# sair-lab/AirSLAM

Hardware: AMD Instinct MI355X
Metric: stereo detect+match pairs/sec (2x PLNet @512x512 internal: points + lines, junctions on the left + LightGlue match) (higher is better)
Workload: dtype fp16

## Files before the change

airslam_amd/_lib.py:

```python
from __future__ import annotations

import ctypes as C
import os

_HERE = os.path.dirname(os.path.abspath(__file__))
LIB_PATH = os.path.join(_HERE, "libairfe.so")


class Tuning(C.Structure):
    _fields_ = [(n, C.c_int) for n in (
        "fuse_lg_block", "gemm_small_max_m", "gemm8_min_m", "gemmr_min_m", "gemmr_wgs", "qkv_pair", "block_min_m", "lgb_tokens", "sg_kenc_gemm",
        "fold_qkv", "overlap_lines", "kf_graph", "kf_spec_rows", "fuse_dec", "assign_fused", "fold_out_proj", "desc_gather_stream", "copy_wgs")] + [("reserved", C.c_int * 5)]


class Cfg(C.Structure):
    _fields_ = [
        ("device", C.c_int), ("precision", C.c_int), ("max_batch", C.c_int), ("enc_chunk", C.c_int),
        ("max_keypoints", C.c_int), ("keypoint_threshold", C.c_float), ("remove_borders", C.c_int),
        ("nms_radius", C.c_int), ("line_threshold", C.c_float), ("line_length_threshold", C.c_float),
        ("matcher", C.c_int), ("image_width", C.c_int), ("image_height", C.c_int), ("sinkhorn_iters", C.c_int),
        ("superpoint_pack", C.c_char_p), ("plnet_s1_pack", C.c_char_p), ("lightglue_pack", C.c_char_p),
        ("superglue_pack", C.c_char_p), ("matcher_precision", C.c_int), ("line_precision", C.c_int), ("check_launches", C.c_int),
        ("tuning", C.POINTER(Tuning)),
    ]


class Stage0(C.Structure):
    _fields_ = [(n, C.c_void_p) for n in (
        "juncs_pred", "lines_pred", "iskeep", "idx_junc_to_end_min", "idx_junc_to_end_max",
        "loi_features", "loi_features_thin", "loi_features_aux")]


class BowdbFilter(C.Structure):
    _fields_ = [("ratio", C.c_float), ("min_words", C.c_int), ("d_max_index", C.c_void_p), ("d_exclude", C.c_void_p), ("exclude_words", C.c_int)]


class RelocCfg(C.Structure):
    _fields_ = [("ratio", C.c_float), ("min_words", C.c_int), ("K", C.c_int), ("outlier_rejection", C.c_int), ("min_inlier", C.c_int),
                ("pose_refinement", C.c_int), ("cam", C.c_double * 5), ("thr", C.c_double * 2)]


class LoopCfg(C.Structure):
    _fields_ = [("ratio", C.c_float), ("min_words", C.c_int), ("K", C.c_int), ("outlier_rejection", C.c_int), ("distance_rate", C.c_double),
                ("min_matches", C.c_int), ("min_points", C.c_int), ("min_inliers", C.c_int), ("cam", C.c_double * 5), ("thr", C.c_double * 2)]


class SeqPolicy(C.Structure):
    _fields_ = [("min_init_stereo_feature", C.c_int), ("min_num_match", C.c_int), ("max_num_match", C.c_int), ("tracking_point_rate", C.c_float),
                ("tracking_parallax_rate", C.c_float), ("min_x_diff", C.c_double), ("max_x_diff", C.c_double), ("max_y_diff", C.c_double),
                ("image_width", C.c_int), ("image_height", C.c_int)]


class SeqFrame(C.Structure):
    _fields_ = ([(n, C.c_int) for n in ("frame_type", "candidate", "promoted", "dropped", "enough_match", "good_stereo_point", "n_left", "n_right", "n_lines_left",
                                        "n_lines_right", "n_junctions", "n_stereo", "n_matches")] + [("_pad", C.c_int)]
                + [(n, C.c_void_p) for n in ("features_left", "features_right", "lines_left", "lines_right", "junctions", "stereo_idx", "stereo_score", "matches_idx",
                                             "matches_score")])


class DebugLinearArgs(C.Structure):
    _fields_ = ([(n, C.c_int) for n in ("prec", "M", "K", "K1", "N")] + [(n, C.c_void_p) for n in ("x1", "x2", "w", "b")]
                + [("epi", C.c_int), ("act", C.c_int), ("rowidx", C.c_void_p), ("src_rows", C.c_int), ("rot_cos", C.c_void_p), ("rot_sin", C.c_void_p),
                   ("Np", C.c_int), ("H", C.c_int), ("x32", C.c_void_p), ("d2s_hc", C.c_int), ("d2s_wc", C.c_int), ("flag", C.c_void_p),
                   ("kernel", C.c_int), ("gr_wgs", C.c_int), ("out", C.c_void_p), ("out2", C.c_void_p)])


class DebugLgBlockArgs(C.Structure):
    _fields_ = ([("prec", C.c_int), ("M", C.c_int)] + [(n, C.c_void_p) for n in ("attn", "x32", "xb", "wo", "bo", "w1", "b1", "gamma", "beta", "w2", "b2")]
                + [(n, C.c_int) for n in ("relu", "tokens_per_wg", "mixed", "nqk_n")]
                + [(n, C.c_void_p) for n in ("nqk_w", "nqk_b", "nv_w", "nv_b", "rot_cos", "rot_sin")]
                + [("Np", C.c_int)] + [(n, C.c_void_p) for n in ("q", "k", "vt")] + [("rows_past", C.c_int * 5)])


class DebugWgPrimsArgs(C.Structure):
    _fields_ = [("v", C.c_void_p), ("keep", C.c_void_p), ("n", C.c_int), ("threads", C.c_int), ("keys", C.c_void_p), ("P", C.c_int), ("key_bytes", C.c_int),
                ("scan", C.c_void_p), ("pos", C.c_void_p), ("totals", C.c_void_p), ("wave", C.c_void_p), ("sorted", C.c_void_p)]


class DebugConvArgs(C.Structure):
    _fields_ = ([(n, C.c_void_p) for n in ("x", "img", "w1a", "b1a", "w", "b")] + [(n, C.c_int) for n in ("cin", "cout", "B", "H", "W", "pool", "out_pad", "relu", "wgs")]
                + [("y_words", C.c_size_t), ("y_raw", C.c_void_p)])


class DebugLgPrepareArgs(C.Structure):
    _fields_ = ([(n, C.c_int) for n in ("prec", "B", "cap", "ld", "kp_off", "normalize")] + [(n, C.c_float) for n in ("cx", "cy", "linv")]
                + [(n, C.c_void_p) for n in ("f0", "f1", "n0", "n1", "wr", "f0x", "f1x")] + [(n, C.c_int) for n in ("n0x", "n1x", "slack_rows", "rows")]
                + [(n, C.c_void_p) for n in ("x32", "xb", "rot_cos", "rot_sin", "lens")] + [("rows_past", C.c_int)])


class DebugLgAssignArgs(C.Structure):
    _fields_ = ([(n, C.c_int) for n in ("prec", "B", "n")] + [(n, C.c_void_p) for n in ("md", "x32", "w")] + [("b", C.c_float), ("lens", C.c_void_p), ("cap", C.c_int),
                ("thr", C.c_float), ("form", C.c_int)]
                + [(n, C.c_void_p) for n in ("pad", "z", "sim", "scores", "rowlse", "collse", "rowval", "rowarg", "colarg", "idx", "score", "nmatch")])


class DebugSgFrontArgs(C.Structure):
    _fields_ = ([(n, C.c_int) for n in ("prec", "split", "B", "cap", "normalize")] + [(n, C.c_void_p) for n in ("f0", "f1", "n0", "n1")] + [("rows", C.c_int)]
                + [(n, C.c_void_p) for n in ("lens", "x32", "xb", "h128", "hb")] + [("rows_past", C.c_int)])


class DebugAttentionArgs(C.Structure):
    _fields_ = ([(n, C.c_int) for n in ("prec", "S", "H", "n", "cross")] + [(n, C.c_void_p) for n in ("q", "k", "v", "lens")]
                + [("canary", C.c_int), ("raw", C.c_int), ("out", C.c_void_p), ("Np", C.c_int), ("rows_past", C.c_int)])


class DebugDetectorTailArgs(C.Structure):
    _fields_ = ([(n, C.c_int) for n in ("B", "Bs", "h", "w", "cap")] + [(n, C.c_void_p) for n in ("heat", "act", "feat", "feat1", "n", "n1", "nms_map", "keep", "cand_cnt")]
                + [("nms_map_written", C.c_int)])


class DebugLinePostArgs(C.Structure):
    _fields_ = ([(n, C.c_int) for n in ("B", "nj", "ld", "h", "w", "capL", "capJ", "from_plane")]
                + [(n, C.c_void_p) for n in ("la", "sc", "m2", "heat", "lines", "nlines", "nfound", "junc", "njunc", "jfound", "jmap")])


class DebugJunctionTailArgs(C.Structure):
    _fields_ = ([(n, C.c_int) for n in ("B", "nj", "ld", "h", "w", "capL", "capJ")]
                + [(n, C.c_void_p) for n in ("la", "sc", "m2", "heat", "act", "lines", "nlines", "nfound", "junc", "njunc", "jfound")] + [("fused", C.c_int)])


class DebugLineMidArgs(C.Structure):
    _fields_ = ([(n, C.c_int) for n in ("B", "j2l", "s1_form", "wgs")]
                + [(n, C.c_void_p) for n in ("juncs_pred", "lines_pred", "thin", "aux", "loi", "iskeep_in", "idx_min_in", "idx_max_in", "iskeep", "idx_min", "idx_max", "counts",
                                             "keep", "pairs", "rep", "head4", "prop4", "ridx", "proj", "lines_adjusted", "scores_line", "table_dirty")])


class DebugS0DecodeArgs(C.Structure):
    _fields_ = ([(n, C.c_int) for n in ("B", "mode", "ld", "off", "want_ta8", "want_loi", "want_jnms", "prec", "wgs")] + [(n, C.c_void_p) for n in ("rows", "x", "w", "b")]
                + [("stage_floats", C.c_size_t)] + [(n, C.c_void_p) for n in ("stage", "jloc", "joff", "jnms", "ta8", "loi", "head_rows")])


SIGNATURES = {
    "airfe_copy_rows_dev": (C.c_int, [C.c_void_p, C.c_int, C.c_void_p, C.c_void_p, C.c_void_p, C.c_void_p, C.c_void_p, C.c_void_p]),
    "airfe_pack_rows_dev": (C.c_int, [C.c_void_p, C.c_int, C.c_void_p, C.c_void_p, C.c_void_p, C.c_void_p, C.c_void_p, C.c_void_p, C.c_void_p]),
    "airfe_seq_default_policy": (None, [C.POINTER(SeqPolicy)]),
    "airfe_seq_add_keyframe_check": (C.c_int, [C.POINTER(SeqPolicy), C.c_void_p, C.c_int, C.c_void_p, C.c_int, C.c_void_p, C.c_int]),
    "airfe_seq_good_stereo_points": (C.c_int, [C.POINTER(SeqPolicy), C.c_void_p, C.c_void_p, C.c_void_p, C.c_int]),
    "airfe_seq_create": (C.c_int, [C.c_void_p, C.c_void_p, C.c_int, C.POINTER(SeqPolicy), C.c_int, C.c_int, C.c_void_p, C.c_void_p, C.c_void_p, C.POINTER(C.c_void_p)]),
    "airfe_seq_destroy": (None, [C.c_void_p]),
    "airfe_seq_last_error": (C.c_char_p, [C.c_void_p]),
    "airfe_seq_begin": (C.c_int, [C.c_void_p, C.c_void_p, C.c_void_p, C.c_int, C.c_int, C.c_int, C.c_size_t]),
    "airfe_seq_end": (C.c_int, [C.c_void_p, C.POINTER(SeqFrame)]),
    "airfe_seq_step": (C.c_int, [C.c_void_p, C.c_void_p, C.c_void_p, C.c_int, C.c_int, C.c_int, C.c_size_t, C.POINTER(SeqFrame)]),
    "airfe_seq_stream": (C.c_void_p, [C.c_void_p]),
    "airfe_seq_set_outlier_rejection": (C.c_int, [C.c_void_p, C.c_int]),
    "airfe_seq_wall_split": (C.c_int, [C.c_void_p, C.POINTER(C.c_double), C.POINTER(C.c_double), C.POINTER(C.c_double), C.POINTER(C.c_int), C.POINTER(C.c_int)]),
    "airfe_default_cfg": (None, [C.POINTER(Cfg)]),
    "airfe_default_tuning": (None, [C.POINTER(Tuning)]),
    "airfe_debug_fail_next_launch": (C.c_int, [C.c_void_p, C.c_int]),
    "airfe_create": (C.c_int, [C.POINTER(Cfg), C.POINTER(C.c_void_p)]),
    "airfe_destroy": (None, [C.c_void_p]),
    "airfe_last_error": (C.c_char_p, [C.c_void_p]),
    "airfe_detect_points": (C.c_int, [C.c_void_p, C.c_void_p, C.c_int, C.c_int, C.c_int, C.c_void_p, C.c_int,
                                      C.POINTER(C.c_int)]),
    "airfe_has_line_branch": (C.c_int, [C.c_void_p]),
    "airfe_detect_plnet": (C.c_int, [C.c_void_p, C.c_void_p, C.c_int, C.c_int, C.c_int, C.POINTER(Stage0), C.c_void_p,
                                     C.c_int, C.POINTER(C.c_int), C.c_void_p, C.c_int, C.POINTER(C.c_int), C.c_void_p,
                                     C.c_int, C.POINTER(C.c_int), C.c_int]),
    "airfe_stereo_keyframe": (C.c_int, [C.c_void_p, C.c_void_p, C.c_void_p, C.c_int, C.c_int, C.c_int, C.c_void_p, C.c_void_p, C.c_int,
                                        C.POINTER(C.c_int), C.POINTER(C.c_int), C.c_void_p, C.c_void_p, C.c_int, C.POINTER(C.c_int),
                                        C.POINTER(C.c_int), C.c_void_p, C.c_int, C.POINTER(C.c_int), C.c_void_p, C.c_void_p, C.c_int,
                                        C.POINTER(C.c_int)]),
    "airfe_stereo_keyframe_tracked": (C.c_int, [C.c_void_p, C.c_void_p, C.c_void_p, C.c_int, C.c_int, C.c_int, C.c_void_p, C.c_void_p, C.c_int,
                                                C.POINTER(C.c_int), C.POINTER(C.c_int), C.c_void_p, C.c_void_p, C.c_int, C.POINTER(C.c_int),
                                                C.POINTER(C.c_int), C.c_void_p, C.c_int, C.POINTER(C.c_int), C.c_void_p, C.c_void_p, C.c_int,
                                                C.POINTER(C.c_int), C.c_void_p, C.c_int, C.c_void_p, C.c_void_p, C.POINTER(C.c_int)]),
    "airfe_track_frame": (C.c_int, [C.c_void_p, C.c_void_p, C.c_int, C.c_int, C.c_int, C.c_void_p, C.c_int, C.c_void_p, C.c_int, C.POINTER(C.c_int),
                                    C.c_void_p, C.c_void_p, C.c_int, C.POINTER(C.c_int)]),
    "airfe_promote_frame": (C.c_int, [C.c_void_p, C.c_void_p, C.c_int, C.c_int, C.c_int, C.c_void_p, C.c_int, C.POINTER(C.c_int), C.c_void_p, C.c_void_p, C.c_int,
                                      C.POINTER(C.c_int)]),
    "airfe_adopt_reference": (C.c_int, [C.c_void_p]),
    "airfe_match_lightglue": (C.c_int, [C.c_void_p, C.c_void_p, C.c_int, C.c_void_p, C.c_int, C.c_void_p, C.c_void_p,
                                        C.c_int, C.POINTER(C.c_int)]),
    "airfe_match_superglue": (C.c_int, [C.c_void_p, C.c_void_p, C.c_int, C.c_void_p, C.c_int, C.c_void_p, C.c_void_p,
                                        C.c_void_p, C.c_void_p]),
    "airfe_assign_points_to_lines": (C.c_int, [C.c_void_p, C.c_void_p, C.c_int, C.c_void_p, C.c_int, C.c_void_p, C.c_void_p,
                                               C.c_void_p, C.c_int, C.c_void_p]),
    "airfe_match_lines": (C.c_int, [C.c_void_p, C.c_void_p, C.c_void_p, C.c_int, C.c_int, C.c_void_p, C.c_void_p, C.c_int, C.c_int,
                                    C.c_void_p, C.c_int, C.c_void_p]),
    "airfe_bow_load": (C.c_int, [C.c_void_p, C.c_void_p, C.c_void_p, C.c_void_p, C.c_void_p, C.c_void_p, C.c_int]),
    "airfe_bow_transform": (C.c_int, [C.c_void_p, C.c_void_p, C.c_int, C.c_void_p, C.c_void_p]),
    "airfe_bow_transform_dev": (C.c_int, [C.c_void_p, C.c_void_p, C.c_int, C.c_void_p, C.c_void_p, C.c_void_p]),
    "airfe_bow_vector": (C.c_int, [C.c_void_p, C.c_void_p, C.c_int, C.c_void_p, C.c_void_p, C.POINTER(C.c_int), C.c_void_p]),
    "airfe_bow_vector_batch_dev": (C.c_int, [C.c_void_p, C.c_void_p, C.c_void_p, C.c_int, C.c_int] + [C.c_void_p] * 5),
    "airfe_bowdb_create": (C.c_int, [C.c_void_p, C.c_int, C.c_int, C.c_int, C.POINTER(C.c_void_p)]),
    "airfe_bowdb_destroy": (C.c_int, [C.c_void_p]),
    "airfe_bowdb_clear": (C.c_int, [C.c_void_p]),
    "airfe_bowdb_size": (C.c_int, [C.c_void_p]),
    "airfe_bowdb_add_batch_dev": (C.c_int, [C.c_void_p] * 6 + [C.c_int, C.c_int, C.c_void_p]),
    "airfe_bowdb_add": (C.c_int, [C.c_void_p] * 6 + [C.c_int, C.c_int]),
    "airfe_bowdb_query_batch_dev": (C.c_int, [C.c_void_p] * 4 + [C.c_int, C.c_int, C.POINTER(BowdbFilter)] + [C.c_void_p] * 3 + [C.c_int] + [C.c_void_p] * 4),
    "airfe_bowdb_topk_dev": (C.c_int, [C.c_void_p] * 4 + [C.c_int, C.c_int, C.c_int, C.c_void_p, C.c_void_p, C.c_void_p]),
    "airfe_bowdb_match_candidates_batch_dev": (C.c_int, [C.c_void_p] * 4 + [C.c_int, C.c_int, C.c_void_p, C.c_int, C.c_int] + [C.c_void_p] * 3 + [C.c_int] + [C.c_void_p] * 3),
    "airfe_bowdb_attach_map": (C.c_int, [C.c_void_p, C.c_int]),
    "airfe_bowdb_set_points_dev": (C.c_int, [C.c_void_p, C.c_int, C.c_int, C.c_void_p, C.c_void_p]),
    "airfe_bowdb_set_points": (C.c_int, [C.c_void_p, C.c_int, C.c_int, C.c_void_p]),
    "airfe_bowdb_get_points": (C.c_int, [C.c_void_p, C.c_int, C.c_int, C.c_void_p]),
    "airfe_bowdb_set_covisibility": (C.c_int, [C.c_void_p, C.c_void_p, C.c_void_p, C.c_void_p, C.c_int]),
    "airfe_bowdb_get_covisibility": (C.c_int, [C.c_void_p, C.c_void_p, C.c_void_p, C.c_void_p, C.c_int, C.POINTER(C.c_int)]),
    "airfe_bowdb_set_positions": (C.c_int, [C.c_void_p, C.c_int, C.c_int, C.c_void_p]),
    "airfe_bowdb_group_dev": (C.c_int, [C.c_void_p, C.c_int] + [C.c_void_p] * 3 + [C.c_int] * 3 + [C.c_void_p] * 8),
    "airfe_relocalize_batch_dev": (C.c_int, [C.c_void_p, C.c_void_p, C.POINTER(RelocCfg), C.c_void_p, C.c_void_p, C.c_int, C.c_int] + [C.c_void_p] * 9 +
                                   [C.c_int] + [C.c_void_p] * 3),
    "airfe_bowdb_set_poses": (C.c_int, [C.c_void_p, C.c_int, C.c_int, C.c_void_p]),
    "airfe_bowdb_get_poses": (C.c_int, [C.c_void_p, C.c_int, C.c_int, C.c_void_p]),
    "airfe_bowdb_set_u_right_dev": (C.c_int, [C.c_void_p, C.c_int, C.c_int, C.c_void_p, C.c_void_p]),
    "airfe_bowdb_set_u_right": (C.c_int, [C.c_void_p, C.c_int, C.c_int, C.c_void_p]),
    "airfe_bowdb_get_u_right": (C.c_int, [C.c_void_p, C.c_int, C.c_int, C.c_void_p]),
    "airfe_bowdb_attach_point_ids": (C.c_int, [C.c_void_p, C.c_int]),
    "airfe_bowdb_set_point_ids_dev": (C.c_int, [C.c_void_p, C.c_int, C.c_int, C.c_void_p, C.c_void_p]),
    "airfe_bowdb_set_point_ids": (C.c_int, [C.c_void_p, C.c_int, C.c_int, C.c_void_p]),
    "airfe_bowdb_get_point_ids": (C.c_int, [C.c_void_p, C.c_int, C.c_int, C.c_void_p]),
    "airfe_bowdb_build_covisibility_dev": (C.c_int, [C.c_void_p, C.c_void_p, C.c_void_p]),
    "airfe_bowdb_build_covisibility": (C.c_int, [C.c_void_p, C.POINTER(C.c_int)]),
    "airfe_bowdb_attach_triangulation": (C.c_int, [C.c_void_p]),
    "airfe_bowdb_triangulate_points_dev": (C.c_int, [C.c_void_p, C.c_void_p, C.c_int] + [C.c_void_p] * 5),
    "airfe_bowdb_triangulate_points": (C.c_int, [C.c_void_p, C.c_void_p, C.c_int, C.c_void_p, C.c_void_p, C.c_void_p, C.POINTER(C.c_int)]),
    "airfe_bowdb_fill_points_dev": (C.c_int, [C.c_void_p, C.c_void_p, C.c_void_p, C.c_int, C.c_void_p, C.c_void_p]),
    "airfe_triangulate_point": (C.c_int, [C.c_void_p, C.c_void_p, C.c_void_p, C.c_int, C.c_void_p, C.POINTER(C.c_int)]),
    "airfe_bowdb_attach_merge": (C.c_int, [C.c_void_p]),
    "airfe_bowdb_merge_points_dev": (C.c_int, [C.c_void_p, C.c_void_p, C.c_int, C.c_void_p, C.c_void_p, C.c_void_p]),
    "airfe_bowdb_merge_points": (C.c_int, [C.c_void_p, C.c_void_p, C.c_int, C.c_void_p, C.c_void_p]),
    "airfe_bowdb_loop_merge_batch_dev": (C.c_int, [C.c_void_p, C.c_void_p, C.c_void_p, C.c_int] + [C.c_void_p] * 6 + [C.c_int] + [C.c_void_p] * 4),
    "airfe_junction_connections_batch_dev": (C.c_int, [C.c_void_p, C.c_void_p, C.c_void_p, C.c_int, C.c_void_p, C.c_void_p] + [C.c_int] * 4 + [C.c_void_p, C.c_int] +
                                             [C.c_void_p] * 4),
    "airfe_junction_connections": (C.c_int, [C.c_void_p, C.c_void_p, C.c_int, C.c_void_p, C.c_int, C.c_int, C.c_int, C.c_void_p, C.c_int, C.POINTER(C.c_int),
                                             C.c_void_p]),
    "airfe_bowdb_attach_junctions": (C.c_int, [C.c_void_p, C.c_int, C.c_int]),
    "airfe_bowdb_set_junctions_dev": (C.c_int, [C.c_void_p, C.c_int, C.c_int] + [C.c_void_p] * 6),
    "airfe_bowdb_set_junctions": (C.c_int, [C.c_void_p, C.c_int, C.c_int] + [C.c_void_p] * 5),
    "airfe_bowdb_get_junctions": (C.c_int, [C.c_void_p, C.c_int, C.c_int] + [C.c_void_p] * 10),
    "airfe_bowdb_junction_term_batch_dev": (C.c_int, [C.c_void_p] * 9 + [C.c_int] + [C.c_void_p] * 4),
    "airfe_bowdb_junction_extra_batch_dev": (C.c_int, [C.c_void_p, C.c_void_p, C.c_void_p, C.c_int, C.c_void_p, C.c_void_p] + [C.c_int] * 4 + [C.c_void_p] * 4),
    "airfe_bowdb_add_junction_frames_batch_dev": (C.c_int, [C.c_void_p, C.c_void_p, C.c_void_p, C.c_int, C.c_void_p, C.c_void_p] + [C.c_int] * 4 + [C.c_void_p]),
    "airfe_bowdb_query_stored_batch_dev": (C.c_int, [C.c_void_p, C.c_void_p, C.c_int, C.c_float, C.c_int, C.c_int] + [C.c_void_p] * 3 + [C.c_int] +
                                           [C.c_void_p] * 4),
    "airfe_loop_detect_batch_dev": (C.c_int, [C.c_void_p, C.c_void_p, C.POINTER(LoopCfg), C.c_void_p, C.c_int] + [C.c_void_p] * 10 + [C.c_int] +
                                    [C.c_void_p] * 3),
    "airfe_set_rectify_maps": (C.c_int, [C.c_void_p, C.c_int, C.c_void_p, C.c_void_p, C.c_int, C.c_int]),
    "airfe_rectify_detect_points": (C.c_int, [C.c_void_p, C.c_int, C.c_void_p, C.c_int, C.c_int, C.c_int, C.c_void_p, C.c_void_p, C.c_int,
                                              C.POINTER(C.c_int)]),
    "airfe_rectify_batch_dev": (C.c_int, [C.c_void_p, C.c_int, C.c_void_p, C.c_int, C.c_int, C.c_int, C.c_int, C.c_size_t, C.c_void_p,
                                          C.c_int, C.c_size_t, C.c_void_p]),
    "airfe_detect_points_batch_dev": (C.c_int, [C.c_void_p, C.c_void_p, C.c_int, C.c_int, C.c_int, C.c_int, C.c_size_t,
                                                C.c_void_p, C.c_int, C.c_void_p, C.c_void_p]),
    "airfe_match_lightglue_batch_dev": (C.c_int, [C.c_void_p, C.c_void_p, C.c_void_p, C.c_void_p, C.c_void_p, C.c_int,
                                                  C.c_int, C.c_void_p, C.c_void_p, C.c_int, C.c_void_p, C.c_void_p]),
    "airfe_match_superglue_batch_dev": (C.c_int, [C.c_void_p, C.c_void_p, C.c_void_p, C.c_void_p, C.c_void_p, C.c_int, C.c_int,
                                                  C.c_void_p, C.c_void_p, C.c_void_p, C.c_void_p, C.c_void_p]),
    "airfe_stereo_batch_dev": (C.c_int, [C.c_void_p, C.c_void_p, C.c_void_p, C.c_int, C.c_int, C.c_int, C.c_int,
                                         C.c_size_t, C.c_void_p, C.c_void_p, C.c_int, C.c_void_p, C.c_void_p, C.c_void_p,
                                         C.c_void_p, C.c_int, C.c_void_p, C.c_void_p]),
    "airfe_detect_plnet_batch_dev": (C.c_int, [C.c_void_p, C.c_void_p, C.c_int, C.c_int, C.c_int, C.c_int, C.c_size_t, C.c_void_p,
                                               C.c_int, C.c_void_p, C.c_void_p, C.c_int, C.c_void_p, C.c_void_p, C.c_int, C.c_void_p,
                                               C.c_int, C.c_void_p, C.c_void_p]),
    "airfe_stereo_plnet_batch_dev": (C.c_int, [C.c_void_p, C.c_void_p, C.c_void_p, C.c_int, C.c_int, C.c_int, C.c_int, C.c_size_t,
                                               C.c_void_p, C.c_void_p, C.c_int, C.c_void_p, C.c_void_p, C.c_void_p, C.c_int, C.c_void_p,
                                               C.c_void_p, C.c_int, C.c_void_p, C.c_void_p, C.c_void_p, C.c_void_p, C.c_int, C.c_void_p,
                                               C.c_void_p]),
    "airfe_debug_plnet_j2l": (C.c_int, [C.c_void_p, C.c_int, C.c_void_p, C.c_void_p, C.c_void_p]),
    "airfe_assign_points_to_lines_batch_dev": (C.c_int, [C.c_void_p, C.c_void_p, C.c_void_p, C.c_int, C.c_void_p, C.c_void_p, C.c_int, C.c_int,
                                                         C.c_void_p, C.c_void_p, C.c_void_p, C.c_int, C.c_void_p, C.c_void_p]),
    "airfe_match_lines_batch_dev": (C.c_int, [C.c_void_p] + [C.c_void_p] * 8 + [C.c_int, C.c_int, C.c_void_p, C.c_void_p, C.c_int, C.c_int,
                                              C.c_void_p, C.c_void_p, C.c_void_p, C.c_int, C.c_void_p, C.c_void_p]),
    "airfe_fundamental_ransac": (C.c_int, [C.c_void_p, C.c_void_p, C.c_int, C.c_void_p, C.c_int, C.c_void_p, C.c_void_p, C.c_int, C.POINTER(C.c_int)]),
    "airfe_fundamental_ransac_batch_dev": (C.c_int, [C.c_void_p, C.c_void_p, C.c_void_p, C.c_void_p, C.c_void_p, C.c_int, C.c_int, C.c_void_p, C.c_void_p,
                                                     C.c_int, C.c_void_p, C.c_void_p, C.c_void_p]),
    "airfe_set_outlier_rejection": (C.c_int, [C.c_void_p, C.c_int]),
    "airfe_pnp_ransac": (C.c_int, [C.c_void_p, C.c_void_p, C.c_void_p, C.c_int, C.c_void_p, C.c_void_p, C.c_void_p, C.c_void_p, C.POINTER(C.c_int)]),
    "airfe_pnp_ransac_batch_dev": (C.c_int, [C.c_void_p, C.c_void_p, C.c_void_p, C.c_void_p, C.c_int, C.c_int, C.c_void_p, C.c_void_p, C.c_void_p,
                                             C.c_void_p, C.c_void_p, C.c_void_p]),
    "airfe_stereo_points": (C.c_int, [C.c_void_p, C.c_void_p, C.c_void_p, C.c_int, C.c_void_p, C.c_int, C.c_void_p, C.c_int, C.c_void_p, C.c_void_p,
                                      C.c_void_p, C.POINTER(C.c_int)]),
    "airfe_stereo_points_batch_dev": (C.c_int, [C.c_void_p] * 6 + [C.c_int, C.c_int, C.c_void_p, C.c_void_p, C.c_int] + [C.c_void_p] * 5),
    "airfe_stereo_lines": (C.c_int, [C.c_void_p, C.c_void_p, C.c_void_p, C.c_int, C.c_void_p, C.c_int] + [C.c_void_p] * 8),
    "airfe_stereo_lines_batch_dev": (C.c_int, [C.c_void_p] * 6 + [C.c_int, C.c_void_p, C.c_void_p, C.c_int] + [C.c_void_p] * 7),
    "airfe_stereo_line_landmarks_batch_dev": (C.c_int, [C.c_void_p] * 6 + [C.c_int] + [C.c_void_p] * 4 + [C.c_int, C.c_void_p, C.c_void_p, C.c_int,
                                                        C.c_void_p, C.c_int] + [C.c_void_p] * 8 + [C.c_int] + [C.c_void_p] * 8),
    "airfe_track_pose_batch_dev": (C.c_int, [C.c_void_p, C.c_void_p, C.c_void_p, C.c_int, C.c_void_p, C.c_int, C.c_void_p, C.c_void_p, C.c_int, C.c_int,
                                             C.c_void_p, C.c_void_p, C.c_void_p, C.c_void_p, C.c_void_p]),
    "airfe_frame_optimize": (C.c_int, [C.c_void_p, C.c_void_p, C.c_void_p, C.c_int] + [C.c_void_p] * 7 + [C.POINTER(C.c_int)]),
    "airfe_frame_optimize_batch_dev": (C.c_int, [C.c_void_p, C.c_void_p, C.c_void_p, C.c_void_p, C.c_int, C.c_int] + [C.c_void_p] * 9),
    "airfe_track_pose_opt_batch_dev": (C.c_int, [C.c_void_p, C.c_void_p, C.c_void_p, C.c_int, C.c_void_p, C.c_int, C.c_void_p, C.c_int, C.c_void_p,
                                                 C.c_void_p, C.c_int, C.c_int] + [C.c_void_p] * 9),
    "airfe_sync": (C.c_int, [C.c_void_p]),
    "airfe_superglue_status": (C.c_int, [C.c_void_p, C.c_void_p]),
    "airfe_profile_enable": (C.c_int, [C.c_void_p, C.c_int]),
    "airfe_profile_stages": (C.c_int, []),
    "airfe_profile_stage_name": (C.c_char_p, [C.c_int]),
    "airfe_profile_read": (C.c_int, [C.c_void_p, C.c_void_p, C.c_void_p, C.c_void_p, C.c_void_p]),
    "airfe_debug_detector_maps": (C.c_int, [C.c_void_p, C.c_int, C.c_void_p, C.c_void_p, C.c_void_p]),
    "airfe_debug_lightglue_scores": (C.c_int, [C.c_void_p, C.c_void_p, C.c_int, C.c_void_p, C.c_int, C.c_void_p]),
    "airfe_debug_superglue_scores": (C.c_int, [C.c_void_p, C.c_void_p, C.c_int, C.c_void_p, C.c_int, C.c_void_p]),
    "airfe_debug_lg_filter": (C.c_int, [C.c_void_p, C.c_void_p, C.c_int, C.c_int, C.c_void_p, C.c_void_p, C.c_int, C.POINTER(C.c_int)]),
    "airfe_debug_sg_decode": (C.c_int, [C.c_void_p, C.c_void_p, C.c_int, C.c_int, C.c_void_p, C.c_void_p, C.c_void_p, C.c_void_p]),
    "airfe_debug_sg_sinkhorn": (C.c_int, [C.c_void_p, C.c_void_p, C.c_void_p, C.c_int, C.c_int, C.c_float, C.c_int, C.c_int, C.c_void_p, C.POINTER(C.c_int)]),
    "airfe_debug_detector_tail": (C.c_int, [C.c_void_p, C.POINTER(DebugDetectorTailArgs)]),
    "airfe_debug_line_post": (C.c_int, [C.c_void_p, C.POINTER(DebugLinePostArgs)]),
    "airfe_debug_junction_tail": (C.c_int, [C.c_void_p, C.POINTER(DebugJunctionTailArgs)]),
    "airfe_debug_junctions_topk": (C.c_int, [C.c_void_p, C.c_void_p, C.c_void_p, C.c_int, C.c_void_p]),
    "airfe_debug_line_mid": (C.c_int, [C.c_void_p, C.POINTER(DebugLineMidArgs)]),
    "airfe_debug_s0_decode": (C.c_int, [C.c_void_p, C.POINTER(DebugS0DecodeArgs)]),
    "airfe_debug_lg_prepare": (C.c_int, [C.c_void_p, C.POINTER(DebugLgPrepareArgs)]),
    "airfe_debug_lg_assign": (C.c_int, [C.c_void_p, C.POINTER(DebugLgAssignArgs)]),
    "airfe_debug_sg_front": (C.c_int, [C.c_void_p, C.POINTER(DebugSgFrontArgs)]),
    "airfe_debug_plnet_stage0": (C.c_int, [C.c_void_p] + [C.c_void_p] * 10),
    "airfe_debug_plnet_s1": (C.c_int, [C.c_void_p, C.POINTER(Stage0), C.c_void_p, C.c_void_p, C.c_int, C.POINTER(C.c_int)]),
    "airfe_debug_plnet_s1_last": (C.c_int, [C.c_void_p, C.c_void_p, C.c_void_p, C.c_int, C.POINTER(C.c_int)]),
    "airfe_debug_preprocess": (C.c_int, [C.c_void_p, C.c_void_p, C.c_int, C.c_int, C.c_int, C.c_void_p]),
    "airfe_debug_conv3x3": (C.c_int, [C.c_void_p, C.c_void_p, C.c_int, C.c_int, C.c_int, C.c_int, C.c_void_p, C.c_void_p,
                                      C.c_int, C.c_int, C.c_void_p]),
    "airfe_debug_conv": (C.c_int, [C.c_void_p, C.POINTER(DebugConvArgs)]),
    "airfe_debug_trace": (C.c_int, [C.c_void_p, C.c_int]),
    "airfe_debug_trace_stop": (C.c_int, [C.c_void_p, C.c_int]),
    "airfe_debug_trace_buffer": (C.c_int, [C.c_void_p, C.c_int, C.c_void_p, C.c_size_t]),
    "airfe_debug_trace_slots": (C.c_int, [C.c_void_p]),
    "airfe_debug_conv_order": (C.c_int, [C.c_int, C.POINTER(C.c_int)]),
    "airfe_debug_wg_prims": (C.c_int, [C.c_void_p, C.POINTER(DebugWgPrimsArgs)]),
    "airfe_debug_trace_slot": (C.c_int, [C.c_void_p, C.c_int, C.c_char_p, C.c_int, C.POINTER(C.c_uint), C.POINTER(C.c_uint), C.POINTER(C.c_uint)]),
    "airfe_debug_trace_read": (C.c_int, [C.c_void_p, C.c_void_p, C.c_void_p, C.c_void_p]),
    "airfe_debug_gemm": (C.c_int, [C.c_void_p, C.c_void_p, C.c_int, C.c_int, C.c_void_p, C.c_void_p, C.c_int, C.c_int,
                                   C.c_void_p]),
    "airfe_debug_linear": (C.c_int, [C.c_void_p, C.POINTER(DebugLinearArgs)]),
    "airfe_debug_qkv": (C.c_int, [C.c_void_p] + [C.c_int] * 3 + [C.c_void_p] * 3 + [C.c_int] + [C.c_void_p] * 4 + [C.c_int] * 2 + [C.c_void_p] * 3),
    "airfe_debug_lg_block": (C.c_int, [C.c_void_p, C.POINTER(DebugLgBlockArgs)]),
    "airfe_debug_ln_gelu": (C.c_int, [C.c_void_p, C.c_int, C.c_void_p, C.c_void_p, C.c_void_p, C.c_int]),
    "airfe_debug_attention_args": (C.c_int, [C.c_void_p, C.POINTER(DebugAttentionArgs)]),
    "airfe_debug_attention": (C.c_int, [C.c_void_p, C.c_void_p, C.c_void_p, C.c_void_p, C.c_void_p, C.c_int, C.c_int, C.c_int, C.c_int, C.c_void_p]),
}

_lib = None


def lib() -> C.CDLL:
    global _lib
    if _lib is None:
        if not os.path.exists(LIB_PATH):
            raise RuntimeError(
                f"{LIB_PATH} is missing: build it with `python -m airslam_amd.build` "
                "(hipcc, gfx950).  airslam_amd has no CPU fallback.")
        try:
            import torch
        except Exception:
            pass
        l = C.CDLL(LIB_PATH)
        for name, (res, args) in SIGNATURES.items():
            fn = getattr(l, name)
            fn.restype = res
            fn.argtypes = args
        _lib = l
    return _lib
```

airslam_amd/api.py:

```python
from __future__ import annotations

import ctypes as C
import os
import tempfile
from typing import Dict, Optional

import numpy as np

from . import _lib, weights as W

FEAT = 259


def _pack_arg(x, tmpfiles) -> Optional[bytes]:
    if x is None:
        return None
    if isinstance(x, (str, bytes, os.PathLike)):
        return os.fsencode(x)
    f = tempfile.NamedTemporaryFile(suffix=".airfe", delete=False)
    f.close()
    W.save_pack(f.name, x)
    tmpfiles.append(f.name)
    return f.name.encode()


class AirfeError(RuntimeError):
    pass


def conv_tile_order(order: int) -> int:
    prev = C.c_int()
    if _lib.lib().airfe_debug_conv_order(int(order), C.byref(prev)) != 0:
        raise AirfeError((_lib.lib().airfe_last_error(None) or b"airfe_debug_conv_order failed").decode())
    return prev.value


class Context:

    def __init__(self, superpoint=None, lightglue=None, superglue=None, plnet_s1=None, tuning=None, **cfg):
        self._l = _lib.lib()
        c = _lib.Cfg()
        self._l.airfe_default_cfg(C.byref(c))
        t = None
        if tuning and "conv_order" in tuning:
            tuning = dict(tuning)
            conv_tile_order(int(tuning.pop("conv_order")))
        if tuning:
            t = _lib.Tuning()
            self._l.airfe_default_tuning(C.byref(t))
            for k, v in tuning.items():
                if k == "reserved" or not hasattr(t, k):
                    raise TypeError(f"unknown airfe_tuning field {k!r}")
                setattr(t, k, int(v))
            c.tuning = C.pointer(t)
        for k, v in cfg.items():
            if not hasattr(c, k):
                raise TypeError(f"unknown airfe_cfg field {k!r}")
            setattr(c, k, v)
        tmp = []
        try:
            c.superpoint_pack = _pack_arg(superpoint, tmp)
            c.lightglue_pack = _pack_arg(lightglue, tmp)
            c.superglue_pack = _pack_arg(superglue, tmp)
            c.plnet_s1_pack = _pack_arg(plnet_s1, tmp)
            h = C.c_void_p()
            rc = self._l.airfe_create(C.byref(c), C.byref(h))
            if rc != 0:
                raise AirfeError((self._l.airfe_last_error(None) or b"airfe_create failed").decode())
        finally:
            for t in tmp:
                os.unlink(t)
        self._h = h
        c.tuning = None
        self.cfg = c
        self.max_keypoints = c.max_keypoints
        self.np_rows = (c.max_keypoints + 15) // 16 * 16

    def close(self):
        if getattr(self, "_h", None):
            self._l.airfe_destroy(self._h)
            self._h = None

    def __del__(self):
        try:
            self.close()
        except Exception:
            pass

    def _chk(self, rc, what):
        if rc != 0:
            raise AirfeError(f"{what}: {(self._l.airfe_last_error(self._h) or b'').decode()}")

    @staticmethod
    def _image(img, wrong_type=None):
        img = np.asarray(img)
        if img.ndim != 2 or img.dtype != np.uint8:
            raise wrong_type if wrong_type is not None else AirfeError("empty image")
        if img.size == 0:
            raise AirfeError("empty image")
        if img.strides[1] != 1 or img.strides[0] < img.shape[1]:
            img = np.ascontiguousarray(img)
        return img

    def detect_points(self, gray: np.ndarray) -> np.ndarray:
        gray = self._image(gray, TypeError("expected a 2-D uint8 image"))
        cap = self.np_rows
        feat = np.empty((cap, FEAT), dtype=np.float32)
        n = C.c_int(0)
        self._chk(self._l.airfe_detect_points(self._h, gray.ctypes.data, gray.shape[0], gray.shape[1], gray.strides[0],
                                              feat.ctypes.data, cap, C.byref(n)), "airfe_detect_points")
        return feat[:n.value].copy()

    def bow_load(self, voc: dict):
        d = np.ascontiguousarray(voc["desc"], np.float32); fc = np.ascontiguousarray(voc["first_child"], np.int32)
        nc = np.ascontiguousarray(voc["n_children"], np.int32); wi = np.ascontiguousarray(voc["word_id"], np.int32)
        w = np.ascontiguousarray(voc["weight"], np.float64)
        self._chk(self._l.airfe_bow_load(self._h, d.ctypes.data, fc.ctypes.data, nc.ctypes.data, wi.ctypes.data, w.ctypes.data, d.shape[0]),
                  "airfe_bow_load")

    def bow_transform(self, feat_rows: np.ndarray):
        f = np.ascontiguousarray(feat_rows, np.float32).reshape(-1, FEAT)
        wid = np.empty((f.shape[0],), np.uint32); w = np.empty((f.shape[0],), np.float64)
        self._chk(self._l.airfe_bow_transform(self._h, f.ctypes.data, f.shape[0], wid.ctypes.data, w.ctypes.data), "airfe_bow_transform")
        return wid, w

    def set_rectify_maps(self, side: int, mapx: np.ndarray, mapy: np.ndarray):
        mx = np.ascontiguousarray(mapx, np.float32); my = np.ascontiguousarray(mapy, np.float32)
        if mx.shape != my.shape or mx.ndim != 2:
            raise TypeError("maps must be two 2-D arrays of one shape")
        self._chk(self._l.airfe_set_rectify_maps(self._h, side, mx.ctypes.data, my.ctypes.data, mx.shape[0], mx.shape[1]), "airfe_set_rectify_maps")

    def rectify_detect(self, side: int, raw: np.ndarray, detect: bool = True):
        raw = self._image(raw)
        rect = np.empty(raw.shape, np.uint8)
        cap = self.np_rows
        feat = np.empty((cap, FEAT), np.float32) if detect else None
        n = C.c_int(0)
        self._chk(self._l.airfe_rectify_detect_points(self._h, side, raw.ctypes.data, raw.shape[0], raw.shape[1], raw.strides[0],
                                                      rect.ctypes.data, feat.ctypes.data if detect else None, cap, C.byref(n)),
                  "airfe_rectify_detect_points")
        return rect, (feat[:n.value].copy() if detect else None)

    def match_lightglue(self, f0: np.ndarray, f1: np.ndarray):
        f0 = np.ascontiguousarray(f0, dtype=np.float32)
        f1 = np.ascontiguousarray(f1, dtype=np.float32)
        cap = self.np_rows
        idx = np.empty((cap, 2), dtype=np.int32)
        sc = np.empty((cap,), dtype=np.float32)
        n = C.c_int(0)
        self._chk(self._l.airfe_match_lightglue(self._h, f0.ctypes.data, f0.shape[0], f1.ctypes.data, f1.shape[0],
                                                idx.ctypes.data, sc.ctypes.data, cap, C.byref(n)), "airfe_match_lightglue")
        return idx[:n.value].copy(), sc[:n.value].copy()

    def lightglue_scores(self, f0: np.ndarray, f1: np.ndarray) -> np.ndarray:
        f0 = np.ascontiguousarray(f0, dtype=np.float32)
        f1 = np.ascontiguousarray(f1, dtype=np.float32)
        out = np.empty((f0.shape[0], f1.shape[0]), dtype=np.float32)
        self._chk(self._l.airfe_debug_lightglue_scores(self._h, f0.ctypes.data, f0.shape[0], f1.ctypes.data, f1.shape[0],
                                                       out.ctypes.data), "airfe_debug_lightglue_scores")
        return out

    @staticmethod
    def _stage0(s0):
        st = _lib.Stage0()
        keep = []
        for name, _ in _lib.Stage0._fields_:
            a = np.ascontiguousarray(s0[name], dtype=np.float32)
            keep.append(a)
            setattr(st, name, a.ctypes.data)
        return st, keep

    def detect_plnet(self, gray: np.ndarray, stage0=None, want_junctions: bool = False, cap_lines: int = 45056,
                     cap_junc: int = 2048):
        gray = self._image(gray)
        cap = self.np_rows
        feat = np.empty((cap, FEAT), np.float32)
        lines = np.empty((cap_lines, 4), np.float64)
        junc = np.empty((cap_junc, FEAT), np.float32)
        n, nl, nj = C.c_int(0), C.c_int(0), C.c_int(0)
        st, keep = (self._stage0(stage0) if stage0 is not None else (None, None))
        self._chk(self._l.airfe_detect_plnet(self._h, gray.ctypes.data, gray.shape[0], gray.shape[1], gray.strides[0],
                                             C.byref(st) if st is not None else None, feat.ctypes.data, cap, C.byref(n),
                                             lines.ctypes.data, cap_lines, C.byref(nl), junc.ctypes.data, cap_junc,
                                             C.byref(nj), int(want_junctions)), "airfe_detect_plnet")
        return feat[:n.value].copy(), lines[:nl.value].copy(), junc[:nj.value].copy()

    def stereo_keyframe(self, left: np.ndarray, right: np.ndarray, match: bool = True, want_junctions: bool = True, cap_lines: int = 4096,
                        cap_junc: int = 2048, track: bool = False, ref_feat=None, outlier_rejection: bool = False):
        if outlier_rejection and not track:
            raise AirfeError("stereo_keyframe: outlier_rejection applies to the temporal match: pass track=True")
        if ref_feat is not None and not track:
            raise AirfeError("stereo_keyframe: ref_feat is the temporal match's reference: pass track=True")
        if track and not match:
            raise AirfeError("stereo_keyframe: track=True needs match=True (the temporal pair rides in the stereo match's forward)")
        imgs = [self._image(g) for g in (left, right)]
        if imgs[0].shape != imgs[1].shape:
            raise AirfeError("stereo_keyframe: left and right images differ in size")
        if imgs[0].strides[0] != imgs[1].strides[0]:
            imgs = [np.ascontiguousarray(g) for g in imgs]
# ... 312 lines not shown
                                  thin=thin.ctypes.data, aux=aux.ctypes.data, loi=loi.ctypes.data, **{k: v.ctypes.data for k, v in out.items()})
        ins = [None if x is None else f(x) for x in (iskeep, idx_min, idx_max)]
        for name, x in zip(("iskeep_in", "idx_min_in", "idx_max_in"), ins):
            if x is not None:
                assert x.shape == (b, n)
                setattr(a, name, x.ctypes.data)
        self._chk(self._l.airfe_debug_line_mid(self._h, C.byref(a)), "airfe_debug_line_mid")
        return out

    S0_STAGE = {"lines_pred": (600, 3 * 16384 * 4), "thin": (600 + 7 * 3 * 16384, 4 * 16384), "aux": (600 + 7 * 3 * 16384 + 4 * 16384, 4 * 16384)}
    S0_STAGE_FLOATS = (600 + 7 * 3 * 16384 + 8 * 16384 + 63) // 64 * 64

    def debug_s0_decode(self, rows=None, ld=160, off=128, ta8=True, loi=False, jnms=True, x=None, w=None, b=None, prec=1, wgs=0, two_pass=False):
        f = lambda t: np.ascontiguousarray(t, np.float32)
        npx, sf = 128 * 128, self.S0_STAGE_FLOATS
        a = _lib.DebugS0DecodeArgs(want_ta8=int(bool(ta8)), want_loi=int(bool(loi)), want_jnms=int(bool(jnms)), prec=int(prec), wgs=int(wgs), stage_floats=sf)
        if rows is not None:
            assert x is None and not two_pass
            rows = f(rows)
            bb = rows.shape[0]
            assert rows.shape == (bb, npx, ld)
            a.mode, a.ld, a.off, a.rows = 0, int(ld), int(off), rows.ctypes.data
        else:
            x, w, b = f(x), f(w), f(b)
            bb = x.shape[0] // npx
            assert x.shape == (bb * npx, 128) and w.shape == (17, 128) and b.shape == (17,)
            a.mode, a.x, a.w, a.b = (2 if two_pass else 1), x.ctypes.data, w.ctypes.data, b.ctypes.data
        poison = lambda *shape: np.full(shape, -1, np.int32).view(np.float32)
        out = {"stage": poison(bb, sf), "jloc": poison(bb, 128, 128), "joff": poison(bb, 2, 128, 128), "jnms": poison(bb, 128, 128), "ta8": poison(bb, npx, 8),
               "loi": poison(128, 128, 128)}
        if two_pass:
            out["head_rows"] = poison(bb, npx, 32)
        a.B = bb
        for k, v in out.items():
            setattr(a, k, v.ctypes.data)
        self._chk(self._l.airfe_debug_s0_decode(self._h, C.byref(a)), "airfe_debug_s0_decode")
        for k, (o, n) in self.S0_STAGE.items():
            v = out["stage"][:, o:o + n]
            out[k] = v.reshape(bb, 3 * npx, 4) if k == "lines_pred" else v.reshape(bb, 4, 128, 128)
        return out

    def debug_junctions_topk(self, jloc, joff):
        jloc, joff = np.ascontiguousarray(jloc, np.float32), np.ascontiguousarray(joff, np.float32)
        b = jloc.shape[0]
        assert jloc.shape == (b, 128, 128) and joff.shape == (b, 2, 128, 128)
        out = np.full((b, 300, 2), np.nan, np.float32)
        self._chk(self._l.airfe_debug_junctions_topk(self._h, jloc.ctypes.data, joff.ctypes.data, b, out.ctypes.data), "airfe_debug_junctions_topk")
        return out

    def debug_preprocess(self, gray):
        gray = np.ascontiguousarray(gray, np.uint8)
        out = np.empty((512, 512), np.float32)
        self._chk(self._l.airfe_debug_preprocess(self._h, gray.ctypes.data, gray.shape[0], gray.shape[1], gray.strides[0],
                                                 out.ctypes.data), "airfe_debug_preprocess")
        return out

    def debug_conv3x3(self, x, w, b, pool=False):
        x = np.ascontiguousarray(x, np.float32); w = np.ascontiguousarray(w, np.float32); b = np.ascontiguousarray(b, np.float32)
        bb, cin, hh, ww = x.shape
        cout = w.shape[0]
        ho, wo = (hh // 2, ww // 2) if pool else (hh, ww)
        y = np.empty((bb, cout, ho, wo), np.float32)
        self._chk(self._l.airfe_debug_conv3x3(self._h, x.ctypes.data, bb, cin, hh, ww, w.ctypes.data, b.ctypes.data, cout,
                                              int(pool), y.ctypes.data), "airfe_debug_conv3x3")
        return y

    def debug_conv(self, w, b, prec, x=None, img=None, w1a=None, b1a=None, pool=False, out_pad=1, relu=True, wgs=256):
        f32 = lambda t: None if t is None else np.ascontiguousarray(t, np.float32)
        x, img, w1a, b1a, w, b = map(f32, (x, img, w1a, b1a, w, b))
        src = x if x is not None else img
        bb, hh, ww = src.shape[0], src.shape[-2], src.shape[-1]
        cout, cin = w.shape[0], w.shape[1]
        p = int(out_pad)
        ho, wo = (hh // 2, ww // 2) if pool else (hh, ww)
        guard = (wo + 2 * p) * cout
        words = bb * (ho + 2 * p) * guard
        raw = np.zeros(words + 2 * guard, np.uint16)
        ptr = lambda t: None if t is None else t.ctypes.data
        a = _lib.DebugConvArgs(x=ptr(x), img=ptr(img), w1a=ptr(w1a), b1a=ptr(b1a), w=ptr(w), b=ptr(b), cin=cin, cout=cout, B=bb, H=hh, W=ww, pool=int(pool), out_pad=p,
                               relu=int(relu), wgs=int(wgs), y_words=raw.size, y_raw=ptr(raw))
        self._chk(self._l.airfe_debug_conv(self._h, C.byref(a)), "airfe_debug_conv")
        buf = raw[guard:guard + words].reshape(bb, ho + 2 * p, wo + 2 * p, cout)
        inner = np.ascontiguousarray(buf[:, p:p + ho, p:p + wo, :])
        y = inner.view(np.float16).astype(np.float32) if prec == 1 else (inner.astype(np.uint32) << 16).view(np.float32)
        return {"raw": buf, "guard_lo": raw[:guard], "guard_hi": raw[guard + words:], "y": np.ascontiguousarray(y.transpose(0, 3, 1, 2))}

    def debug_gemm(self, x, w, b, relu=False):
        x = np.ascontiguousarray(x, np.float32); w = np.ascontiguousarray(w, np.float32); b = np.ascontiguousarray(b, np.float32)
        m, k = x.shape
        n = w.shape[0]
        y = np.empty((m, n), np.float32)
        self._chk(self._l.airfe_debug_gemm(self._h, x.ctypes.data, m, k, w.ctypes.data, b.ctypes.data, n, int(relu),
                                           y.ctypes.data), "airfe_debug_gemm")
        return y

    DEBUG_KERNELS = {"dispatch": 0, "small": 1, "tiled": 2, "gemm8": 3, "gemmr": 4, "gemmr_gather": 5, "gemmr_gather128": 6}

    def debug_linear(self, x1, w, b, prec, epi=0, act=0, x2=None, rowidx=None, rot=None, Np=0, x32=None, d2s=None, kernel="dispatch", gr_wgs=0):
        f32 = lambda t: None if t is None else np.ascontiguousarray(t, np.float32)
        x1, w, b, x2, x32 = f32(x1), f32(w), f32(b), f32(x2), (None if x32 is None else np.array(x32, np.float32, copy=True))
        n, k = w.shape
        m = len(rowidx) if rowidx is not None else x1.shape[0]
        a = _lib.DebugLinearArgs(prec=prec, M=m, K=k, K1=x1.shape[1], N=n, x1=x1.ctypes.data, w=w.ctypes.data, b=b.ctypes.data, epi=epi, act=act, Np=Np, H=4,
                                 kernel=self.DEBUG_KERNELS[kernel], gr_wgs=gr_wgs)
        keep = []
        if x2 is not None:
            a.x2 = x2.ctypes.data
        if rowidx is not None:
            ri = np.ascontiguousarray(rowidx, np.int32)
            keep.append(ri)
            a.rowidx, a.src_rows = ri.ctypes.data, x1.shape[0]
        if rot is not None:
            rc, rs = f32(rot[0]), f32(rot[1])
            keep += [rc, rs]
            a.rot_cos, a.rot_sin = rc.ctypes.data, rs.ctypes.data
        if x32 is not None:
            a.x32 = x32.ctypes.data
        flag = np.zeros(1, np.int32)
        out2 = None
        if epi == 5:
            hc, wc = d2s
            a.d2s_hc, a.d2s_wc, a.flag = hc, wc, flag.ctypes.data
            out = np.empty((m // (hc * wc), 8 * hc, 8 * wc), np.float32)
        elif epi in (3, 4):
            s = m // Np
            out = np.empty((s, 4, Np, 64) if epi == 3 else (s, 4, 64, Np), np.float32)
            if epi == 3 and n == 512:
                out2 = np.empty_like(out)
                a.out2 = out2.ctypes.data
        else:
            out = np.empty((m, n), np.float32)
        a.out = out.ctypes.data
        self._chk(self._l.airfe_debug_linear(self._h, C.byref(a)), "airfe_debug_linear")
        if epi == 5:
            return out, int(flag[0])
        if epi == 2:
            return out, x32
        return (out, out2) if out2 is not None else out

    def debug_qkv(self, x, wqk, bqk, wv, bv, prec, Np, rot=None, pair=True, gr_wgs=0):
        f32 = lambda t: np.ascontiguousarray(t, np.float32)
        x, wqk, bqk, wv, bv = f32(x), f32(wqk), f32(bqk), f32(wv), f32(bv)
        m, nqk, s = x.shape[0], wqk.shape[0], x.shape[0] // Np
        q = np.empty((s, 4, Np, 64), np.float32)
        k = np.empty_like(q) if nqk == 512 else None
        vt = np.empty((s, 4, 64, Np), np.float32)
        rc, rs = (f32(rot[0]), f32(rot[1])) if rot is not None else (None, None)
        ptr = lambda t: None if t is None else t.ctypes.data
        self._chk(self._l.airfe_debug_qkv(self._h, prec, m, Np, ptr(x), ptr(wqk), ptr(bqk), nqk, ptr(wv), ptr(bv), ptr(rc), ptr(rs), int(pair), gr_wgs, ptr(q),
                                          ptr(k), ptr(vt)), "airfe_debug_qkv")
        return q, k, vt

    def debug_lg_block(self, attn, x32, w1, b1, w2, b2, prec, gamma=None, beta=None, wo=None, bo=None, relu=False, tokens_per_wg=128, mixed=False,
                       nqk=None, nv=None, rot=None, Np=0):
        f32 = lambda t: None if t is None else np.ascontiguousarray(t, np.float32)
        m = attn.shape[0]
        attn, w1, b1, w2, b2, gamma, beta, wo, bo = map(f32, (attn, w1, b1, w2, b2, gamma, beta, wo, bo))
        x32 = np.array(x32, np.float32, copy=True)
        xb = np.empty_like(x32)
        ptr = lambda t: None if t is None else t.ctypes.data
        a = _lib.DebugLgBlockArgs(prec=prec, M=m, attn=ptr(attn), x32=ptr(x32), xb=ptr(xb), wo=ptr(wo), bo=ptr(bo), w1=ptr(w1), b1=ptr(b1), gamma=ptr(gamma),
                                  beta=ptr(beta), w2=ptr(w2), b2=ptr(b2), relu=int(relu), tokens_per_wg=tokens_per_wg, mixed=int(mixed), Np=Np)
        q = k = vt = None
        keep = []
        if nqk is not None:
            (qw, qb), (vw, vb) = map(lambda p: (f32(p[0]), f32(p[1])), (nqk, nv))
            keep += [qw, qb, vw, vb]
            s = m // Np
            q, vt = np.empty((s, 4, Np, 64), np.float32), np.empty((s, 4, 64, Np), np.float32)
            a.nqk_n, a.nqk_w, a.nqk_b, a.nv_w, a.nv_b, a.q, a.vt = qw.shape[0], ptr(qw), ptr(qb), ptr(vw), ptr(vb), ptr(q), ptr(vt)
            if qw.shape[0] == 512:
                k = np.empty_like(q)
                a.k = ptr(k)
        if rot is not None:
            rc, rs = f32(rot[0]), f32(rot[1])
            keep += [rc, rs]
            a.rot_cos, a.rot_sin = ptr(rc), ptr(rs)
        self._chk(self._l.airfe_debug_lg_block(self._h, C.byref(a)), "airfe_debug_lg_block")
        return {"x32": x32, "xb": xb, "q": q, "k": k, "vt": vt, "rows_past": list(a.rows_past)}

    def debug_ln_gelu(self, h, gamma, beta, prec):
        h = np.array(h, np.float32, copy=True)
        gamma, beta = np.ascontiguousarray(gamma, np.float32), np.ascontiguousarray(beta, np.float32)
        self._chk(self._l.airfe_debug_ln_gelu(self._h, prec, h.ctypes.data, gamma.ctypes.data, beta.ctypes.data, h.shape[0]), "airfe_debug_ln_gelu")
        return h

    def debug_attention(self, q, k, v, lens, cross=False, prec=None, raw=False):
        q = np.ascontiguousarray(q, np.float32); k = np.ascontiguousarray(k, np.float32); v = np.ascontiguousarray(v, np.float32)
        lens = np.ascontiguousarray(lens, np.int32)
        s, h, n, d = q.shape
        assert d == 64 and k.shape == q.shape and v.shape == q.shape and lens.shape == (s,)
        if prec is None:
            assert not raw, "raw rows come from airfe_debug_attention_args: give prec"
            out = np.empty((s, n, h * 64), np.float32)
            self._chk(self._l.airfe_debug_attention(self._h, q.ctypes.data, k.ctypes.data, v.ctypes.data, lens.ctypes.data, s, h, n, int(cross), out.ctypes.data),
                      "airfe_debug_attention")
            return out
        out = np.empty((s, (n + 15) // 16 * 16 if raw else n, h * 64), np.float32)
        a = _lib.DebugAttentionArgs(prec=int(prec), S=s, H=h, n=n, cross=int(cross), q=q.ctypes.data, k=k.ctypes.data, v=v.ctypes.data, lens=lens.ctypes.data,
                                    canary=1, raw=int(raw), out=out.ctypes.data)
        self._chk(self._l.airfe_debug_attention_args(self._h, C.byref(a)), "airfe_debug_attention_args")
        return (out, a.rows_past) if raw else out

    def detect_batch_dev(self, gray_t, feat_t, n_t, stream=None):
        b, h, w = gray_t.shape
        self._chk(self._l.airfe_detect_points_batch_dev(self._h, gray_t.data_ptr(), b, h, w, gray_t.stride(1),
                                                        gray_t.stride(0), feat_t.data_ptr(), feat_t.shape[1],
                                                        n_t.data_ptr(), self._stream(stream)), "airfe_detect_points_batch_dev")

    def fundamental_ransac(self, f0: np.ndarray, f1: np.ndarray, idx: np.ndarray, score: np.ndarray):
        f0 = np.ascontiguousarray(f0, dtype=np.float32).reshape(-1, FEAT)
        f1 = np.ascontiguousarray(f1, dtype=np.float32).reshape(-1, FEAT)
        idx = np.array(idx, dtype=np.int32, copy=True).reshape(-1, 2)
        score = np.array(score, dtype=np.float32, copy=True).reshape(-1)
        if len(score) != len(idx):
            raise AirfeError("fundamental_ransac: idx and score differ in length")
        k = C.c_int(0)
        self._chk(self._l.airfe_fundamental_ransac(self._h, f0.ctypes.data, len(f0), f1.ctypes.data, len(f1), idx.ctypes.data, score.ctypes.data, len(idx),
                                                   C.byref(k)), "airfe_fundamental_ransac")
        return idx[:k.value], score[:k.value]

    def fundamental_ransac_batch_dev(self, f0_t, f1_t, idx_t, score_t, nm_t, F_t=None, stream=None):
        self._chk(self._l.airfe_fundamental_ransac_batch_dev(self._h, f0_t.data_ptr(), None, f1_t.data_ptr(), None, f0_t.shape[0], f0_t.shape[1],
                                                             idx_t.data_ptr(), score_t.data_ptr(), idx_t.shape[1], nm_t.data_ptr(),
                                                             None if F_t is None else F_t.data_ptr(), self._stream(stream)),
                  "airfe_fundamental_ransac_batch_dev")

    def pnp_ransac(self, obj: np.ndarray, img: np.ndarray, K):
        obj = np.ascontiguousarray(obj, np.float64).reshape(-1, 3)
        img = np.ascontiguousarray(img, np.float64).reshape(-1, 2)
        if len(obj) != len(img):
            raise AirfeError("pnp_ransac: obj and img differ in length")
        k = np.ascontiguousarray(K, np.float64).reshape(4)
        Twc, Rt = np.zeros(16), np.zeros(12)
        mask = np.zeros(max(len(obj), 1), np.uint8)
        cnt = C.c_int(0)
        self._chk(self._l.airfe_pnp_ransac(self._h, obj.ctypes.data, img.ctypes.data, len(obj), k.ctypes.data, Twc.ctypes.data, Rt.ctypes.data,
                                           mask.ctypes.data, C.byref(cnt)), "airfe_pnp_ransac")
        return dict(Twc=Twc.reshape(4, 4), Rt=Rt, inlier=mask[:len(obj)], count=cnt.value)

    def pnp_ransac_batch_dev(self, obj_t, img_t, n_t, K, Twc_t, inlier_t, count_t, Rt_t=None, stream=None):
        k = np.ascontiguousarray(K, np.float64).reshape(4)
        self._chk(self._l.airfe_pnp_ransac_batch_dev(self._h, obj_t.data_ptr(), img_t.data_ptr(), n_t.data_ptr(), obj_t.shape[0], obj_t.shape[1],
                                                     k.ctypes.data, Twc_t.data_ptr(), None if Rt_t is None else Rt_t.data_ptr(), inlier_t.data_ptr(),
                                                     count_t.data_ptr(), self._stream(stream)), "airfe_pnp_ransac_batch_dev")

    def stereo_points(self, cam, featL: np.ndarray, featR: np.ndarray, idx: np.ndarray):
        cam = np.ascontiguousarray(cam, np.float64).reshape(8)
        featL = np.ascontiguousarray(featL, np.float32).reshape(-1, FEAT)
        featR = np.ascontiguousarray(featR, np.float32).reshape(-1, FEAT)
        idx = np.ascontiguousarray(idx, np.int32).reshape(-1, 2)
        nL = len(featL)
        u, d, xyz = np.empty(max(nL, 1)), np.empty(max(nL, 1)), np.empty((max(nL, 1), 3))
        good = C.c_int(0)
        self._chk(self._l.airfe_stereo_points(self._h, cam.ctypes.data, featL.ctypes.data, nL, featR.ctypes.data, len(featR), idx.ctypes.data, len(idx),
                                              u.ctypes.data, d.ctypes.data, xyz.ctypes.data, C.byref(good)), "airfe_stereo_points")
        return dict(u_right=u[:nL], depth=d[:nL], xyz=xyz[:nL], good=good.value)

    def stereo_points_batch_dev(self, cam, featL_t, nL_t, featR_t, nR_t, idx_t, nm_t, u_right_t, depth_t, xyz_t, good_t, stream=None):
        cam = np.ascontiguousarray(cam, np.float64).reshape(8)
        self._chk(self._l.airfe_stereo_points_batch_dev(self._h, cam.ctypes.data, featL_t.data_ptr(), nL_t.data_ptr(), featR_t.data_ptr(), nR_t.data_ptr(),
                                                        featL_t.shape[0], featL_t.shape[1], idx_t.data_ptr(), nm_t.data_ptr(), idx_t.shape[1],
                                                        u_right_t.data_ptr(), depth_t.data_ptr(), xyz_t.data_ptr(), good_t.data_ptr(), self._stream(stream)),
                  "airfe_stereo_points_batch_dev")

    def stereo_lines(self, cam, lines_left: np.ndarray, lines_right: np.ndarray, line_matches: np.ndarray, Twc=None):
        cam = np.ascontiguousarray(cam, np.float64).reshape(8)
        ll = np.ascontiguousarray(lines_left, np.float64).reshape(-1, 4)
        lr = np.ascontiguousarray(lines_right, np.float64).reshape(-1, 4)
        lm = np.ascontiguousarray(line_matches, np.int32).reshape(-1)
        if len(lm) != len(ll):
            raise ValueError("stereo_lines: one match per left line")
        twc = None if Twc is None else np.ascontiguousarray(Twc, np.float64).reshape(16)
        n = len(ll)
        m = max(n, 1)
        sel, valid, status = np.empty((m, 4)), np.empty(m, np.uint8), np.empty(m, np.int32)
        ends, plk, count = np.empty((m, 6)), np.empty((m, 6)), np.empty(3, np.int32)
        self._chk(self._l.airfe_stereo_lines(self._h, cam.ctypes.data, ll.ctypes.data, n, lr.ctypes.data if len(lr) else None, len(lr), lm.ctypes.data,
                                             None if twc is None else twc.ctypes.data, sel.ctypes.data, valid.ctypes.data, status.ctypes.data,
                                             ends.ctypes.data, plk.ctypes.data, count.ctypes.data), "airfe_stereo_lines")
        return dict(lines_right_sel=sel[:n], right_valid=valid[:n], status=status[:n], endpoints=ends[:n], plucker=plk[:n], count=count)

    def stereo_lines_batch_dev(self, cam, lines_left_t, nlines_left_t, lines_right_t, nlines_right_t, line_matches_t, Twc_t, lines_right_sel_t,
                               right_valid_t, status_t, endpoints_t, plucker_t, count_t, stream=None):
        cam = np.ascontiguousarray(cam, np.float64).reshape(8)
        self._chk(self._l.airfe_stereo_lines_batch_dev(
            self._h, cam.ctypes.data, lines_left_t.data_ptr(), nlines_left_t.data_ptr(), lines_right_t.data_ptr(), nlines_right_t.data_ptr(),
            lines_left_t.shape[1], line_matches_t.data_ptr(), None if Twc_t is None else Twc_t.data_ptr(), lines_left_t.shape[0],
            lines_right_sel_t.data_ptr(), right_valid_t.data_ptr(), status_t.data_ptr(), endpoints_t.data_ptr(), plucker_t.data_ptr(), count_t.data_ptr(),
            self._stream(stream)), "airfe_stereo_lines_batch_dev")

    def stereo_line_landmarks_batch_dev(self, cam, lines_left_t, nlines_left_t, lines_right_t, nlines_right_t, featL_t, nL_t, featR_t, nR_t, idx_t, nm_t,
                                        Twc_t, relL, relR, line_matches_t, lines_right_sel_t, right_valid_t, status_t, endpoints_t, plucker_t, count_t,
                                        stream=None):
        cam = np.ascontiguousarray(cam, np.float64).reshape(8)
        tot = [None if r[3] is None else r[3].data_ptr() for r in (relL, relR)]
        self._chk(self._l.airfe_stereo_line_landmarks_batch_dev(
            self._h, cam.ctypes.data, lines_left_t.data_ptr(), nlines_left_t.data_ptr(), lines_right_t.data_ptr(), nlines_right_t.data_ptr(),
            lines_left_t.shape[1], featL_t.data_ptr(), nL_t.data_ptr(), featR_t.data_ptr(), nR_t.data_ptr(), featL_t.shape[1], idx_t.data_ptr(),
            nm_t.data_ptr(), idx_t.shape[1], None if Twc_t is None else Twc_t.data_ptr(), lines_left_t.shape[0], relL[0].data_ptr(), relL[1].data_ptr(),
            relL[2].data_ptr(), tot[0], relR[0].data_ptr(), relR[1].data_ptr(), relR[2].data_ptr(), tot[1], relL[1].shape[1],
            line_matches_t.data_ptr(), lines_right_sel_t.data_ptr(), right_valid_t.data_ptr(), status_t.data_ptr(), endpoints_t.data_ptr(),
            plucker_t.data_ptr(), count_t.data_ptr(), self._stream(stream)), "airfe_stereo_line_landmarks_batch_dev")

    def track_pose_batch_dev(self, K, xyz_t, feat_t, tidx_t, ntrack_t, Twc_t, mask_t, count_t, Rt_t=None, stream=None):
        k = np.ascontiguousarray(K, np.float64).reshape(4)
        self._chk(self._l.airfe_track_pose_batch_dev(self._h, k.ctypes.data, xyz_t.data_ptr(), xyz_t.shape[1], feat_t.data_ptr(), feat_t.shape[1],
                                                     tidx_t.data_ptr(), ntrack_t.data_ptr(), tidx_t.shape[1], tidx_t.shape[0], Twc_t.data_ptr(),
                                                     None if Rt_t is None else Rt_t.data_ptr(), mask_t.data_ptr(), count_t.data_ptr(),
                                                     self._stream(stream)), "airfe_track_pose_batch_dev")

    @staticmethod
    def _tcb(Tcb):
        if Tcb is None:
            return None, None
        t = np.ascontiguousarray(Tcb, np.float64)
        if t.size == 16:
            t = np.ascontiguousarray(np.concatenate([t.reshape(4, 4)[:3, :3].reshape(9), t.reshape(4, 4)[:3, 3]]))
        t = t.reshape(12)
        return t, t.ctypes.data

    def frame_optimize(self, X: np.ndarray, obs: np.ndarray, cam, thr, Twc0, Tcb=None):
        X = np.ascontiguousarray(X, np.float64).reshape(-1, 3)
        obs = np.ascontiguousarray(obs, np.float64).reshape(-1, 3)
        if len(X) != len(obs):
            raise AirfeError("frame_optimize: X and obs differ in length")
        cam = np.ascontiguousarray(cam, np.float64).reshape(5)
        thr = np.ascontiguousarray(thr, np.float64).reshape(2)
        T0 = np.ascontiguousarray(Twc0, np.float64).reshape(16)
        keep, tcb = self._tcb(Tcb)
        Twc, Rt = np.zeros(16), np.zeros(12)
        mask = np.zeros(max(len(X), 1), np.uint8)
# ... 573 lines not shown
```

airslam_amd/csrc/airfe_debug.hip:

```cpp
#include "airfe_host.h"
#include "wg_prims.h"

#include <limits.h>
#include <memory>

struct HookStage {
  enum { OWN_TEXT = 1, SATURATION = 2, DEVICE_WIDE = 4 };
  HookStage(airfe_ctx* c_, const std::string& who_, int pack_prec = 0) : c(c_), who(who_), st(c_->stream) { mem.pack_prec = pack_prec; }
  HookStage(const HookStage&) = delete;
  ~HookStage() {
    if (queued) (void)hipStreamSynchronize(st);
    for (void* p : mem.allocs) (void)hipFree(p);
  }
  int status() const { return rc; }
  hipStream_t stream() { queued = true; return st; }
  int refuse(const std::string& m) { return rc ? rc : rc = fail(c, who + ": " + m); }
  void step(int r) { queued = true; if (r) rc = 1; }
  template <class T> T* fresh(size_t n, int byte) {
    T* p = raw<T>(n);
    fill(p, byte, std::max<size_t>(n, 1) * sizeof(T));
    return p;
  }
  template <class T> T* up(std::vector<T> v) { T* p = raw<T>(v.size()); put(p, std::move(v)); return p; }
  template <class T> T* up(const T* src, size_t n) { return up(std::vector<T>(src, src + n)); }
// ... 84 lines not shown
  __shared__ int wsum[THREADS / 64];
  __shared__ K key[32768 / sizeof(K)];
  const int t = threadIdx.x;
  const int x0 = t < n ? v[t] : 0;
  const int ws = wave_sum(x0), wx = wave_max(x0), wn = wave_min(x0);
  if ((t & 63) == 0) { wave[3 * (t >> 6)] = ws; wave[3 * (t >> 6) + 1] = wx; wave[3 * (t >> 6) + 2] = wn; }
  int sbase = 0, cbase = 0, s = 0, mx = INT_MIN, mn = INT_MAX;
  for (int i0 = 0; i0 < n; i0 += THREADS) {
    const int i = i0 + t;
    const int x = i < n ? v[i] : 0;
    int stot, ctot;
    const int ex = sbase + block_excl_scan<THREADS>(x, wsum, &stot);
    const int p = cbase + block_compact<THREADS>(i < n && keep[i], wsum, &ctot);
    if (i < n) { scan[i] = ex; pos[i] = p; s += x; mx = max(mx, x); mn = min(mn, x); }
    sbase += stot;
    cbase += ctot;
  }
  s = block_sum<THREADS>(s, wsum);
  mx = block_max<THREADS>(mx, wsum);
  mn = block_min<THREADS>(mn, wsum);
  if (t == 0) { totals[0] = sbase; totals[1] = cbase; totals[2] = s; totals[3] = mx; totals[4] = mn; }
  for (int i = t; i < P; i += THREADS) key[i] = keys[i];
  block_sort_asc<THREADS>(key, P);
  for (int i = t; i < P; i += THREADS) sorted[i] = key[i];
}
template <int THREADS>
static void launch_wg_prims(const airfe_debug_wg_prims_args* a, const int* v, const uint8_t* keep, const void* keys, int* out, void* sorted, hipStream_t st) {
  int *scan = out, *pos = out + a->n, *totals = out + 2 * a->n, *wave = totals + 5;
  if (a->key_bytes == 4)
    hipLaunchKernelGGL((wg_prims_kernel<THREADS, unsigned>), dim3(1), dim3(THREADS), 0, st, v, keep, a->n, static_cast<const unsigned*>(keys), a->P, scan, pos, totals,
                       wave, static_cast<unsigned*>(sorted));
  else
    hipLaunchKernelGGL((wg_prims_kernel<THREADS, unsigned long long>), dim3(1), dim3(THREADS), 0, st, v, keep, a->n, static_cast<const unsigned long long*>(keys), a->P,
                       scan, pos, totals, wave, static_cast<unsigned long long*>(sorted));
}

extern "C" {

int airfe_debug_preprocess(airfe_ctx* c, const uint8_t* gray, int h, int w, int stride, float* out) try {
  if (c && enter_device(c)) return 1;
  if (!c || !c->has_sp) return fail(c, "debug_preprocess: detector not loaded");
  const size_t bytes = (size_t)h * stride;
  const int R = AIRFE_INTERNAL_SIZE;
  HookStage s(c, "debug_preprocess");
  s.step(upload_image(c, gray, h, w, stride) || ensure_tables(c, h, w));
  if (s.status()) return 1;
  launch_preprocess(c->st_img.p, 1, h, w, stride, bytes, c->xtab, c->ytab, c->lut, c->img32, R, R, s.stream());
  s.wait();
  s.get2d(out, (size_t)R * 4, c->img32 + (R + 2) + 1, (size_t)(R + 2) * 4, (size_t)R * 4, R);
  return s.status();
} AIRFE_CATCH(c)

int airfe_debug_conv3x3(airfe_ctx* c, const float* x, int B, int cin, int H, int W, const float* w, const float* b, int cout,
                        int pool, float* y) try {
  AIRFE_ENTER(c);
  if ((cin != 64 && cin != 128) || cout % 64 || W % 16 || H % 16) return fail(c, "debug_conv3x3: unsupported shape");
  const int prec = c->prec;
  const int Ho = pool ? H / 2 : H, Wo = pool ? W / 2 : W;
  const size_t ywords = (size_t)B * (Ho + 2) * (Wo + 2) * cout;
  HookStage s(c, "debug_conv3x3");
  ConvArgs a;
  a.X = s.up(dbg_conv_x(x, B, cin, H, W, prec)); a.Wp = s.up(dbg_conv_slabs(w, cin, cout, prec));
  a.bias = s.up(b, (size_t)cout); a.Y = s.fresh<uint16_t>(ywords, 0);
  a.B = B; a.H = H; a.W = W; a.CIN = cin; a.COUT = cout;
  a.pool = pool; a.out_pad = 1; a.relu = 1;
  if (s.status()) return 1;
  launch_conv3x3(prec, a, s.stream());
  s.wait();
  const std::vector<uint16_t> yo = s.get<uint16_t>(a.Y, ywords);
  for (int bb = 0; bb < B; ++bb)
    for (int co = 0; co < cout; ++co)
      for (int yy = 0; yy < Ho; ++yy)
        for (int xx = 0; xx < Wo; ++xx)
          y[(((size_t)bb * cout + co) * Ho + yy) * Wo + xx] = back2(yo[(((size_t)bb * (Ho + 2) + yy + 1) * (Wo + 2) + xx + 1) * cout + co], prec);
  return s.status();
} AIRFE_CATCH(c)

int airfe_debug_fail_next_launch(airfe_ctx* c, int stage) try {
  AIRFE_ENTER(c);
  if (stage < -1 || stage >= ST_COUNT) return fail(c, "debug_fail_next_launch: no such stage");
  c->fail_stage = stage;
  return 0;
} AIRFE_CATCH(c)

int airfe_debug_gemm(airfe_ctx* c, const float* x, int M, int K, const float* w, const float* b, int N, int relu, float* y) try {
  AIRFE_ENTER(c);
  if (K != 128 && K != 256 && K != 512) return fail(c, "debug_gemm: K must be 128, 256 or 512");
  const int prec = c->prec, Mp = (M + 127) / 128 * 128, Np8 = (N + 7) / 8 * 8;
  HookStage s(c, "debug_gemm", prec);
  LinW lw;
  s.linear(w, b, K, N, lw);
  GemmArgs g;
  g.X1 = s.up(dbg_rows2(x, M, K, Mp, prec)); g.ld1 = K; g.K1 = K; g.Wp = lw.w; g.bias = lw.b; g.M = Mp; g.N = N; g.cb_total = lw.cbt;
  g.epi = EPI_STORE_F32; g.act = relu ? ACT_RELU : ACT_NONE; g.out = s.fresh<float>((size_t)Mp * Np8, 0); g.ldo = Np8;
  dbg_gemm_dispatch(c, g, 0);
  if (s.status()) return 1;
  launch_gemm(prec, K, false, g, s.stream());
  s.wait(HookStage::OWN_TEXT);
  const std::vector<float> yo = s.get<float>(g.out, (size_t)Mp * Np8);
  for (int m = 0; m < M; ++m)
    for (int n = 0; n < N; ++n) y[(size_t)m * N + n] = yo[(size_t)m * Np8 + n];
  return s.status();
} AIRFE_CATCH(c)

int airfe_debug_conv(airfe_ctx* c, airfe_debug_conv_args* a) try {
  AIRFE_ENTER(c);
  if (!a || !a->w || !a->b || !a->y_raw) return fail(c, "debug_conv: null argument");
  const bool fused = a->img != nullptr;
  if (fused == (a->x != nullptr)) return fail(c, "debug_conv: exactly one of x (plain form) and img (fused conv1a -> conv1b) must be given");
  const int cin = a->cin, cout = a->cout, B = a->B, H = a->H, W = a->W, pool = a->pool, opad = a->out_pad, prec = c->prec;
  if (prec != 0 && prec != 1) return fail(c, "debug_conv: the context's precision must be fp16 or bf16");
  if (a->wgs < 1 || a->wgs > 256) return fail(c, "debug_conv: wgs must lie in 1 .. 256");
  if (cin != 64 && cin != 128) return fail(c, "debug_conv: cin must be 64 or 128");
  if (cout < 64 || cout % 64 || (cin == 128 && cout % 128)) return fail(c, "debug_conv: cout must be a multiple of 64 (of 128 when cin is 128)");
  if (B < 1 || H < 16 || W < 16 || H % 16 || W % 16) return fail(c, "debug_conv: B >= 1, H and W multiples of 16");
  if ((pool != 0 && pool != 1) || (opad != 0 && opad != 1) || (a->relu != 0 && a->relu != 1)) return fail(c, "debug_conv: pool, out_pad and relu are 0 or 1");
  if (pool && !opad) return fail(c, "debug_conv: a pooled layer always feeds another conv (out_pad = 1); pool with out_pad = 0 is no form of the arena");
  if (fused && (cin != 64 || cout != 64 || !pool || !opad || !a->relu || !a->w1a || !a->b1a))
    return fail(c, "debug_conv: the fused form is conv1a -> conv1b: cin = cout = 64, pool = 1, out_pad = 1, relu = 1, w1a and b1a given");
  const int Ho = pool ? H / 2 : H, Wo = pool ? W / 2 : W;
  const size_t guard = (size_t)(Wo + 2 * opad) * cout, words = (size_t)B * (Ho + 2 * opad) * guard, total = words + 2 * guard;
  if (a->y_words != total) return fail(c, "debug_conv: y_words must be (B (Ho + 2 out_pad) + 2) (Wo + 2 out_pad) cout");
  HookStage s(c, "debug_conv");
  ConvArgs g;
  if (fused) {
    std::vector<float> im((size_t)B * (H + 2) * (W + 2), 0.f);
    for (int bb = 0; bb < B; ++bb)
      for (int yy = 0; yy < H; ++yy) memcpy(&im[((size_t)bb * (H + 2) + yy + 1) * (W + 2) + 1], a->img + ((size_t)bb * H + yy) * W, (size_t)W * sizeof(float));
    g.img = s.up(std::move(im));
    g.w1a = s.up(a->w1a, (size_t)64 * 9);
    g.b1a = s.up(a->b1a, (size_t)64);
  } else {
    g.X = s.up(dbg_conv_x(a->x, B, cin, H, W, prec));
  }
  g.Wp = s.up(dbg_conv_slabs(a->w, cin, cout, prec));
  g.bias = s.up(a->b, (size_t)cout);
  uint16_t* dy = s.fresh<uint16_t>(total, 0xFF);
  if (s.status()) return 1;
  g.Y = dy + guard;
  g.B = B; g.H = H; g.W = W; g.CIN = cin; g.COUT = cout; g.pool = pool; g.out_pad = opad; g.relu = a->relu; g.wgs = a->wgs;
  if (fused) launch_conv64r(prec, g, s.stream());
  else launch_conv3x3(prec, g, s.stream());
  s.wait(HookStage::OWN_TEXT);
  s.get(a->y_raw, dy, total * 2);
  return s.status();
} AIRFE_CATCH(c)

int airfe_debug_conv_order(int order, int* previous) try {
  if (order < -1 || order > CONV_ORDER_DEFAULT) return fail(nullptr, "debug_conv_order: order must lie in -1 .. 3");
  const int before = conv_tile_order_switch(order);
  if (previous) *previous = before;
  return 0;
} AIRFE_CATCH(nullptr)

int airfe_debug_linear(airfe_ctx* c, const airfe_debug_linear_args* a) try {
  AIRFE_ENTER(c);
  if (!a || !a->x1 || !a->w || !a->b || !a->out) return fail(c, "debug_linear: null argument");
  const int prec = a->prec, M = a->M, K = a->K, N = a->N, epi = a->epi, kern = a->kernel, K1 = a->x2 ? a->K1 : K;
  if ((prec != 0 && prec != 1) || M < 1 || N < 1 || (K != 128 && K != 256 && K != 512) || K1 < 32 || K1 % 32 || K1 > K || (a->x2 && K1 == K) ||
      epi < EPI_STORE || epi > EPI_SOFTMAX_D2S || kern < AIRFE_DEBUG_KERNEL_DISPATCH || kern > AIRFE_DEBUG_KERNEL_GEMMR_GATHER128 || (a->act != ACT_NONE && a->act != ACT_RELU))
    return fail(c, "debug_linear: bad argument");
  const bool trans = epi == EPI_HEADS_T, heads = epi == EPI_HEADS || trans, d2s = epi == EPI_SOFTMAX_D2S;
  if (heads && ((a->H != 4 && a->H != 0) || a->Np < 16 || a->Np % 16 || M % a->Np || (epi == EPI_HEADS ? (N != 256 && N != 512) || (N == 512 && !a->out2) : N != 256)))
    return fail(c, "debug_linear: head layouts need H = 4, M = S * Np with Np a multiple of 16, N = 256 (or 512 with out2 for EPI_HEADS)");
  if ((a->rot_cos || a->rot_sin) && (epi != EPI_HEADS || !a->rot_cos || !a->rot_sin)) return fail(c, "debug_linear: rotary is an EPI_HEADS form");
  if (epi == EPI_RESID && (!a->x32 || N % 64)) return fail(c, "debug_linear: EPI_RESID needs x32 and N a multiple of 64");
  if (d2s && (K != 256 || N != 65 || a->x2 || a->rowidx || a->act || a->d2s_hc < 1 || a->d2s_wc < 1 || M % (a->d2s_hc * a->d2s_wc) || M % 16 ||
              (kern != AIRFE_DEBUG_KERNEL_DISPATCH && kern != AIRFE_DEBUG_KERNEL_GEMM8)))
    return fail(c, "debug_linear: EPI_SOFTMAX_D2S is launch_gemm8's head kernel: K = 256, N = 65, dense rows, M = B * hc * wc, M % 16 == 0");
  if (a->rowidx) {
    if (kern != AIRFE_DEBUG_KERNEL_GEMM8 && kern != AIRFE_DEBUG_KERNEL_GEMMR_GATHER && kern != AIRFE_DEBUG_KERNEL_GEMMR_GATHER128)
      return fail(c, "debug_linear: a row gather runs in gemm8, gemmr_gather or gemmr_gather128 only");
    if (a->src_rows < 1) return fail(c, "debug_linear: rowidx needs src_rows");
    for (int r = 0; r < M; ++r)
      if (a->rowidx[r] < 0 || a->rowidx[r] >= a->src_rows) return fail(c, "debug_linear: rowidx entry outside 0 .. src_rows - 1");
  }
  static const int row_tile[7] = {128, 32, 128, 256, 32, 32, 64};
  const int Mp = d2s ? M : (M + row_tile[kern] - 1) / row_tile[kern] * row_tile[kern];
  const int xrows = a->rowidx ? a->src_rows : Mp;
  const int ldo = (epi == EPI_STORE || epi == EPI_STORE_F32) ? (N + 7) / 8 * 8 : N;
  const int Sg = heads ? (Mp + a->Np - 1) / a->Np : 0, S = heads ? M / a->Np : 0;
  const bool f32 = epi == EPI_STORE_F32 || d2s, two = epi == EPI_HEADS && N == 512;
  const size_t out_elems = d2s ? (size_t)M * 64 : heads ? (size_t)Sg * 4 * a->Np * 64 : (size_t)Mp * ldo, out_bytes = out_elems * (f32 ? 4 : 2);
  HookStage s(c, "debug_linear", prec);
  LinW lw;
  s.linear(a->w, a->b, K, N, lw);
  GemmArgs g;
  g.X1 = s.up(dbg_rows2(a->x1, a->rowidx ? a->src_rows : M, K1, xrows, prec)); g.ld1 = K1; g.K1 = K1;
  if (a->x2) { g.X2 = s.up(dbg_rows2(a->x2, M, K - K1, Mp, prec)); g.ld2 = K - K1; }
  g.Wp = lw.w; g.bias = lw.b; g.M = Mp; g.N = N; g.cb_total = lw.cbt; g.epi = epi; g.act = a->act; g.ldo = ldo; g.Np = a->Np; g.H = 4;
  dbg_gemm_dispatch(c, g, a->gr_wgs);
  if (a->rot_cos) { g.rot_cos = s.up(dbg_rows4(a->rot_cos, M, 32, Mp)); g.rot_sin = s.up(dbg_rows4(a->rot_sin, M, 32, Mp)); }
  if (a->rowidx) { std::vector<int> ri(Mp, 0); memcpy(ri.data(), a->rowidx, (size_t)M * sizeof(int)); g.rowidx = s.up(std::move(ri)); }
  g.out = s.fresh<uint8_t>(out_bytes, 0xFF);
  if (two) g.out2 = s.fresh<uint8_t>(out_bytes, 0xFF);
  if (epi == EPI_RESID) g.x32 = s.up(dbg_rows4(a->x32, M, N, Mp));
  if (d2s) { g.d2s_hc = a->d2s_hc; g.d2s_wc = a->d2s_wc; g.flag = s.fresh<int>(1, 0); }
  if (s.status()) return 1;
  const char* refused = nullptr;
  hipStream_t st = s.stream();
  switch (kern) {
    case AIRFE_DEBUG_KERNEL_DISPATCH:
      if (d2s) launch_gemm8(prec, K, false, g, st);
      else launch_gemm(prec, K, trans, g, st);
      break;
    case AIRFE_DEBUG_KERNEL_SMALL:
      if (d2s || a->rowidx) refused = "gemm_small";
      else { g.small_max = 1 << 30; g.g8_min = 1 << 30; g.gr_min = 1 << 30; launch_gemm(prec, K, trans, g, st); }
      break;
    case AIRFE_DEBUG_KERNEL_TILED:
      if (d2s || a->rowidx || K1 % 64) refused = "gemm_kernel";
      else { g.small_max = -1; g.g8_min = 1 << 30; g.gr_min = 1 << 30; launch_gemm(prec, K, trans, g, st); }
      break;
    case AIRFE_DEBUG_KERNEL_GEMM8:
      if (K1 % 64) refused = "gemm8";
      else launch_gemm8(prec, K, trans, g, st);
      break;
    case AIRFE_DEBUG_KERNEL_GEMMR:
      if (a->rowidx || !gemmr_applicable(K, trans, g)) refused = "gemmr";
      else launch_gemmr(prec, trans, g, st);
      break;
    case AIRFE_DEBUG_KERNEL_GEMMR_GATHER:
      if (!gemmr_gather_applicable(K, g)) refused = "gemmr_gather";
      else launch_gemmr_gather(prec, g, st);
      break;
    default:
      if (!gemmr_gather128_applicable(g)) refused = "gemmr_gather128";
      else launch_gemmr_gather128(prec, g, st);
      break;
  }
  if (refused) return s.refuse(std::string(refused) + " does not apply to this form");
  s.wait(HookStage::OWN_TEXT);
  if (f32) {
    const std::vector<float> ho = s.get<float>(g.out, out_elems);
    for (int m = 0; m < (d2s ? 1 : M); ++m) memcpy(a->out + (size_t)m * N, ho.data() + (size_t)m * ldo, (d2s ? out_elems : (size_t)N) * 4);
    if (d2s && a->flag) s.get(a->flag, g.flag, sizeof(int));
  } else if (heads) {
    const size_t n = (size_t)S * 4 * a->Np * 64;
    dbg_back2(s.get<uint16_t>(g.out, out_elems), n, prec, a->out);
    if (two) dbg_back2(s.get<uint16_t>(g.out2, out_elems), n, prec, a->out2);
  } else {
    const std::vector<uint16_t> ho = s.get<uint16_t>(g.out, out_elems);
    for (int m = 0; m < M; ++m)
      for (int n = 0; n < N; ++n) a->out[(size_t)m * N + n] = back2(ho[(size_t)m * ldo + n], prec);
    if (epi == EPI_RESID) s.get(a->x32, g.x32, (size_t)M * N * 4);
  }
  return s.status();
} AIRFE_CATCH(c)

int airfe_debug_qkv(airfe_ctx* c, int prec, int M, int Np, const float* x, const float* wqk, const float* bqk, int nqk, const float* wv, const float* bv,
                    const float* rot_cos, const float* rot_sin, int pair, int gr_wgs, float* q, float* k, float* vt) try {
  AIRFE_ENTER(c);
  if ((prec != 0 && prec != 1) || M < 1 || Np < 16 || Np % 16 || M % Np || (nqk != 256 && nqk != 512) || !x || !wqk || !bqk || !wv || !bv || !q || !vt ||
      (nqk == 512 && !k) || (!rot_cos) != (!rot_sin))
    return fail(c, "debug_qkv: bad argument");
  const int Mp = (M + 127) / 128 * 128, Sg = (Mp + Np - 1) / Np, S = M / Np;
  const size_t elems = (size_t)Sg * 4 * Np * 64, n = (size_t)S * 4 * Np * 64;
  HookStage s(c, "debug_qkv", prec);
  LinW lqk, lv;
  s.linear(wqk, bqk, 256, nqk, lqk);
  s.linear(wv, bv, 256, 256, lv);
  GemmArgs ga, gb;
  ga.X1 = gb.X1 = s.up(dbg_rows2(x, M, 256, Mp, prec));
  ga.ld1 = gb.ld1 = 256; ga.K1 = gb.K1 = 256; ga.M = gb.M = Mp; ga.Np = gb.Np = Np; ga.H = gb.H = 4;
  ga.Wp = lqk.w; ga.bias = lqk.b; ga.N = nqk; ga.cb_total = lqk.cbt; ga.epi = EPI_HEADS; ga.ldo = nqk;
  gb.Wp = lv.w; gb.bias = lv.b; gb.N = 256; gb.cb_total = lv.cbt; gb.epi = EPI_HEADS_T; gb.ldo = 256;
  ga.out = s.fresh<uint16_t>(elems, 0xFF);
  if (nqk == 512) ga.out2 = s.fresh<uint16_t>(elems, 0xFF);
  gb.out = s.fresh<uint16_t>(elems, 0xFF);
  if (rot_cos) { ga.rot_cos = s.up(dbg_rows4(rot_cos, M, 32, Mp)); ga.rot_sin = s.up(dbg_rows4(rot_sin, M, 32, Mp)); }
  dbg_gemm_dispatch(c, ga, gr_wgs);
  dbg_gemm_dispatch(c, gb, gr_wgs);
  if (s.status()) return 1;
  if (pair) {
    if (!gemmr_pair_applicable(ga, gb)) return s.refuse("gemmr_pair does not apply to this form");
    launch_gemmr_pair(prec, ga, gb, s.stream());
  } else {
    launch_gemm(prec, 256, false, ga, s.stream());
    launch_gemm(prec, 256, true, gb, s.stream());
  }
  s.wait(HookStage::OWN_TEXT);
  dbg_back2(s.get<uint16_t>(ga.out, elems), n, prec, q);
  if (nqk == 512) dbg_back2(s.get<uint16_t>(ga.out2, elems), n, prec, k);
  dbg_back2(s.get<uint16_t>(gb.out, elems), n, prec, vt);
  return s.status();
} AIRFE_CATCH(c)

int airfe_debug_lg_block(airfe_ctx* c, airfe_debug_lg_block_args* a) try {
  AIRFE_ENTER(c);
  if (!a || !a->attn || !a->x32 || !a->xb || !a->w1 || !a->b1 || !a->w2 || !a->b2 || (!a->relu && (!a->gamma || !a->beta)) || (!a->wo) != (!a->bo))
    return fail(c, "debug_lg_block: null argument");
  const int prec = a->prec, M = a->M, T = a->tokens_per_wg, nq = a->nqk_n, Np = a->Np;
  if ((prec != 0 && prec != 1) || M < 1 || (T != 32 && T != 64 && T != 112 && T != 128) || (nq != 0 && nq != 256 && nq != 512) || (a->relu && nq))
    return fail(c, "debug_lg_block: bad argument");
  if (a->mixed) {
    const int tiles = (M + 15) / 16, W = c->n_cu;
    if (a->wo || T != 112 || W <= 0 || tiles <= 7 * W || tiles > 13 * W) return fail(c, "debug_lg_block: the mixed split does not apply to this form");
  }
  if (nq && (!a->nqk_w || !a->nqk_b || !a->nv_w || !a->nv_b || !a->q || !a->vt || (nq == 512) != (a->rot_cos && a->rot_sin) || (nq == 512 && !a->k) || Np < 16 ||
             Np % 16 || M % Np))
    return fail(c, "debug_lg_block: the next projection needs its weights and outputs, rotary exactly when nqk_n = 512, and M = S * Np (Np a multiple of 16)");
  const int cap = M + 256;
  const int Sg = nq ? (cap + Np - 1) / Np : 0, S = nq ? M / Np : 0;
  const size_t helems = (size_t)Sg * 4 * Np * 64;
  HookStage s(c, "debug_lg_block", prec);
  LinW lo, l1, l2, lq, lv;
  if (a->wo) s.linear(a->wo, a->bo, 256, 256, lo);
  s.linear(a->w1, a->b1, 512, 512, l1);
  s.linear(a->w2, a->b2, 512, 256, l2);
  if (nq) { s.linear(a->nqk_w, a->nqk_b, 256, nq, lq); s.linear(a->nv_w, a->nv_b, 256, 256, lv); }
  const bool fr = lg_blockf_frag_weights();
  const std::vector<float> x32h = dbg_rows4(a->x32, M, 256, cap);
  std::vector<uint16_t> xbh((size_t)cap * 256);
  for (size_t i = 0; i < xbh.size(); ++i) xbh[i] = cvt2(x32h[i], prec);
  std::vector<float> gb(1024, 0.f);
  if (!a->relu) { memcpy(gb.data(), a->gamma, 512 * 4); memcpy(gb.data() + 512, a->beta, 512 * 4); }
  LgBlockFArgs g;
  g.attn = s.up(dbg_rows2(a->attn, M, 256, cap, prec));
  g.xb = s.up(xbh);
  g.x32 = s.up(x32h);
  const float* dgb = s.up(std::move(gb));
  g.gamma = dgb; g.beta = dgb ? dgb + 512 : nullptr;
  g.wo = a->wo ? (fr ? lo.wf : lo.w) : nullptr; g.bo = a->wo ? lo.b : nullptr;
  g.w1 = fr ? l1.wf : l1.w; g.b1 = l1.b; g.w2 = fr ? l2.wf : l2.w; g.b2 = l2.b;
  g.M = M; g.tokens_per_wg = T; g.mixed = a->mixed; g.n_cu = c->n_cu; g.relu = a->relu;
  if (nq) {
    g.nqk_w = fr ? lq.wf : lq.w; g.nqk_b = lq.b; g.nqk_n = nq; g.nv_w = fr ? lv.wf : lv.w; g.nv_b = lv.b; g.Np = Np; g.H = 4;
    if (nq == 512) { g.rot_cos = s.up(dbg_rows4(a->rot_cos, M, 32, cap)); g.rot_sin = s.up(dbg_rows4(a->rot_sin, M, 32, cap)); }
    g.q_out = s.fresh<uint16_t>(helems, 0xFF);
    if (nq == 512) g.k_out = s.fresh<uint16_t>(helems, 0xFF);
    g.vt_out = s.fresh<uint16_t>(helems, 0xFF);
  }
  if (s.status()) return 1;
  launch_lg_blockf(prec, g, s.stream());
  s.wait(HookStage::OWN_TEXT);
  const std::vector<float> x32o = s.get<float>(g.x32, (size_t)cap * 256);
  const std::vector<uint16_t> xbo = s.get<uint16_t>(g.xb, (size_t)cap * 256);
  memcpy(a->x32, x32o.data(), (size_t)M * 256 * 4);
  dbg_back2(xbo, (size_t)M * 256, prec, a->xb);
  for (int i = 0; i < 5; ++i) a->rows_past[i] = 0;
  for (int r = M; r < cap; ++r)
    for (int f = 0; f < 256; ++f) {
      const size_t e = (size_t)r * 256 + f;
      if (memcmp(&x32o[e], &x32h[e], 4)) a->rows_past[0] = r - M + 1;
      if (xbo[e] != xbh[e]) a->rows_past[1] = r - M + 1;
    }
  uint16_t* dev[3] = {g.q_out, g.k_out, g.vt_out};
  float* host[3] = {a->q, a->k, a->vt};
  for (int j = 0; j < 3 && nq; ++j) {
    if (!dev[j]) continue;
    const std::vector<uint16_t> ho = s.get<uint16_t>(dev[j], helems);
    dbg_back2(ho, (size_t)S * 4 * Np * 64, prec, host[j]);
    for (size_t e = (size_t)S * 4 * Np * 64; e < helems; ++e) {
      if (ho[e] == 0xFFFF) continue;
      const size_t sq = e / ((size_t)4 * Np * 64), w = e % ((size_t)Np * 64);
      const int row = (int)(sq * Np + (j == 2 ? w % Np : w / 64));
      a->rows_past[2 + j] = std::max(a->rows_past[2 + j], row - M + 1);
    }
  }
  return s.status();
} AIRFE_CATCH(c)

int airfe_debug_ln_gelu(airfe_ctx* c, int prec, float* h, const float* gamma, const float* beta, int M) try {
  AIRFE_ENTER(c);
  if ((prec != 0 && prec != 1) || M < 1 || !h || !gamma || !beta) return fail(c, "debug_ln_gelu: bad argument");
  HookStage s(c, "debug_ln_gelu");
  std::vector<float> gb(1024);
  memcpy(gb.data(), gamma, 512 * 4);
  memcpy(gb.data() + 512, beta, 512 * 4);
  uint16_t* dh = s.up(dbg_rows2(h, M, 512, M, prec));
  const float* dgb = s.up(std::move(gb));
  if (s.status()) return 1;
  launch_ln_gelu(prec, dh, dgb, dgb + 512, M, s.stream());
  s.wait(HookStage::OWN_TEXT);
  dbg_back2(s.get<uint16_t>(dh, (size_t)M * 512), (size_t)M * 512, prec, h);
  return s.status();
} AIRFE_CATCH(c)
}

static int dbg_attention_run(airfe_ctx* c, airfe_debug_attn_args* a, const char* who) {
  const std::string w = std::string(who) + ": ";
  const int S = a->S, H = a->H, n = a->n, cross = a->cross, prec = a->prec;
  if (prec != 0 && prec != 1) return fail(c, w + "prec must be 0 (bf16) or 1 (fp16)");
  if (S < 1 || H < 1 || n < 1 || (S * H) % 8 != 0 || (cross && (S & 1))) return fail(c, w + "S * H must be a multiple of 8 (cross: S even)");
  if (!a->q || !a->k || !a->v || !a->lens || !a->out) return fail(c, w + "null argument");
  for (int s = 0; s < S; ++s)
    if (a->lens[s] < 0 || a->lens[s] > n) return fail(c, w + "lens[s] must lie in 0 .. n");
  const int Np = (n + 15) / 16 * 16;
  a->Np = Np; a->rows_past = 0;
  const size_t rows = (size_t)S * H * Np + 128;
  std::vector<uint16_t> hq(rows * 64, 0), hk(rows * 64, 0), hvt(rows * 64, 0);
  for (int s = 0; s < S; ++s)
    for (int h = 0; h < H; ++h)
      for (int i = 0; i < n; ++i)
        for (int d = 0; d < 64; ++d) {
          const size_t src = (((size_t)s * H + h) * n + i) * 64 + d;
          hq[(((size_t)s * H + h) * Np + i) * 64 + d] = cvt2(a->q[src], prec);
          hk[(((size_t)s * H + h) * Np + i) * 64 + d] = cvt2(a->k[src], prec);
          hvt[(((size_t)s * H + h) * 64 + d) * Np + i] = cvt2(a->v[src], prec);
        }
  HookStage s(c, who);
  const uint16_t *dq = s.up(std::move(hq)), *dk = s.up(std::move(hk)), *dv = s.up(std::move(hvt));
  const size_t out_n = (size_t)S * Np * H * 64, slack_n = (size_t)128 * H * 64;
  uint16_t* dout = s.fresh<uint16_t>(out_n + slack_n, a->canary ? 0xFF : 0);
  const int* dl = s.up(a->lens, (size_t)S);
  if (s.status()) return 1;
  launch_attention32(prec, dq, dk, dv, dout, dl, S, H, Np, cross, s.stream());
  s.wait(HookStage::OWN_TEXT);
  const std::vector<uint16_t> ho = s.get<uint16_t>(dout, out_n + slack_n);
  const int rows_out = a->raw ? Np : n;
  for (int q = 0; q < S; ++q)
    for (int i = 0; i < rows_out; ++i)
      for (int f = 0; f < H * 64; ++f) a->out[((size_t)q * rows_out + i) * H * 64 + f] = back2(ho[((size_t)q * Np + i) * H * 64 + f], prec);
  for (int r = 0; r < 128 && a->canary; ++r) {
    bool changed = false;
    for (int f = 0; f < H * 64 && !changed; ++f) changed = ho[out_n + (size_t)r * H * 64 + f] != 0xFFFFu;
    a->rows_past += changed;
  }
  return s.status();
}

extern "C" {
int airfe_debug_attention(airfe_ctx* c, const float* q, const float* k, const float* v, const int* lens, int S, int H, int n, int cross, float* out) try {
  AIRFE_ENTER(c);
  if (c->mprec == 2) return fail(c, "debug_attention drives the 2-byte kernel (matcher_precision fp16 / bf16)");
  airfe_debug_attn_args a = {};
  a.prec = c->mprec; a.S = S; a.H = H; a.n = n; a.cross = cross;
  a.q = q; a.k = k; a.v = v; a.lens = lens; a.out = out;
  return dbg_attention_run(c, &a, "debug_attention");
} AIRFE_CATCH(c)

int airfe_debug_attention_args(airfe_ctx* c, airfe_debug_attn_args* a) try {
  AIRFE_ENTER(c);
  if (!a) return fail(c, "debug_attention_args: null argument");
  return dbg_attention_run(c, a, "debug_attention_args");
} AIRFE_CATCH(c)

int airfe_debug_lg_prepare(airfe_ctx* c, airfe_debug_lg_prepare_args* a) try {
  AIRFE_ENTER(c);
  if (!c->has_arena) return fail(c, "debug_lg_prepare: no matcher loaded");
  if (!a || !a->f0 || !a->f1 || !a->n0 || !a->n1 || !a->wr || !a->x32 || !a->xb || !a->rot_cos || !a->rot_sin || !a->lens || (!a->f0x) != (!a->f1x))
    return fail(c, "debug_lg_prepare: null argument");
  const int Np = c->Np, B = a->B, Bt = a->f0x ? 2 : B;
  if ((a->prec != 0 && a->prec != 1) || B < 1 || B > c->Pmax || (a->f0x && (B != 1 || c->Pmax < 2)) || a->cap < 1 || a->cap > Np || a->kp_off < 0 ||
      a->ld < a->kp_off + 258 || a->slack_rows < 0)
    return fail(c, "debug_lg_prepare: bad argument (prec 0 / 1, 1 <= B <= max_batch, a second pair with B = 1 only, 1 <= cap <= Np, ld >= kp_off + 258)");
  for (int b = 0; b < B; ++b)
    if (a->n0[b] < 0 || a->n0[b] > a->cap || a->n1[b] < 0 || a->n1[b] > a->cap) return fail(c, "debug_lg_prepare: every n0, n1 must lie in 0 .. cap");
  if (a->f0x && (a->n0x < 0 || a->n0x > Np || a->n1x < 0 || a->n1x > Np)) return fail(c, "debug_lg_prepare: the second pair's lengths must lie in 0 .. Np");
  const size_t rows = (size_t)2 * Bt * Np + (size_t)a->slack_rows, R = c->arena_rows;
  if (rows > R || (size_t)a->rows != rows) return fail(c, "debug_lg_prepare: rows must be 2 Bt Np + slack_rows and fit the arena");
  HookStage s(c, "debug_lg_prepare");
  const size_t fl = (size_t)B * a->cap * a->ld;
  std::vector<int> hn(2 * B + 2);
  for (int b = 0; b < B; ++b) { hn[b] = a->n0[b]; hn[B + b] = a->n1[b]; }
  hn[2 * B] = a->n0x; hn[2 * B + 1] = a->n1x;
  const int* dn = s.up(std::move(hn));
  LgPrepArgs pa;
  pa.f0 = s.up(a->f0, fl); pa.f1 = s.up(a->f1, fl); pa.wr = s.up(a->wr, (size_t)64);
  if (a->f0x) {
    std::vector<float> x0(a->f0x, a->f0x + (size_t)a->n0x * a->ld), x1(a->f1x, a->f1x + (size_t)a->n1x * a->ld);
    x0.resize(x0.size() + a->ld, 0.f); x1.resize(x1.size() + a->ld, 0.f);
    pa.f0x = s.up(std::move(x0)); pa.f1x = s.up(std::move(x1));
  }
  const DevSpan arena[4] = {{c->x32, R * 256 * 4}, {c->xb, R * 256 * 2}, {c->rot_cos, R * 32 * 4}, {c->rot_sin, R * 32 * 4}};
  for (const DevSpan& e : arena) s.fill(e.p, 0xFF, e.bytes);
  s.fill(c->lens, 0xFF, (size_t)2 * c->Pmax * 4);
  if (s.status()) return 1;
  pa.n0 = dn; pa.n1 = dn + B; pa.ld = a->ld; pa.kp_off = a->kp_off; pa.normalize = a->normalize;
  pa.cx = a->cx; pa.cy = a->cy; pa.linv = a->linv; pa.B = B; pa.cap = a->cap; pa.Np = Np;
  pa.x32 = c->x32; pa.xb = c->xb; pa.rot_cos = c->rot_cos; pa.rot_sin = c->rot_sin; pa.lens = c->lens;
  if (a->f0x) { pa.n0x = dn + 2 * B; pa.n1x = dn + 2 * B + 1; }
  pa.slack_rows = a->slack_rows;
  launch_lg_prepare(a->prec, pa, s.stream());
  s.wait();
  const std::vector<float> hx = s.get<float>(c->x32, R * 256);
  const std::vector<uint16_t> hb = s.get<uint16_t>(c->xb, R * 256);
  s.get(a->rot_cos, c->rot_cos, rows * 32 * 4);
  s.get(a->rot_sin, c->rot_sin, rows * 32 * 4);
  s.get(a->lens, c->lens, (size_t)2 * Bt * 4);
  if (s.status()) return 1;
  memcpy(a->x32, hx.data(), rows * 256 * 4);
  dbg_back2(hb, rows * 256, a->prec, a->xb);
  int past = 0;
  for (size_t r = rows; r < R; ++r) {
    bool touched = false;
    for (int k = 0; k < 256 && !touched; ++k) {
      uint32_t u;
      memcpy(&u, &hx[r * 256 + k], 4);
      touched = u != 0xFFFFFFFFu || hb[r * 256 + k] != 0xFFFFu;
    }
    past += touched;
  }
  a->rows_past = past;
  for (const DevSpan& e : arena) s.fill(e.p, 0, e.bytes);
  return s.wait();
} AIRFE_CATCH(c)

int airfe_debug_lg_assign(airfe_ctx* c, airfe_debug_lg_assign_args* a) try {
  AIRFE_ENTER(c);
  if (!c->has_arena) return fail(c, "debug_lg_assign: no matcher loaded");
  if (!a || !a->md || !a->x32 || !a->w || !a->lens || !a->z || !a->sim || !a->scores || !a->rowlse || !a->collse || !a->rowval || !a->rowarg || !a->colarg ||
      !a->idx || !a->score || !a->nmatch)
    return fail(c, "debug_lg_assign: null argument");
  const int Np = c->Np, B = a->B, n = a->n, S = 2 * B, cap = a->cap, prec = a->prec;
// ... 624 lines not shown
```

airslam_amd/csrc/kernels.h:

```cpp
#pragma once
#include <hip/hip_runtime.h>
#include <stdint.h>

struct MergeTables;
struct MergeLoop;

namespace airfe {

enum Epi {
  EPI_STORE = 0,
  EPI_STORE_F32 = 1,
  EPI_RESID = 2,
  EPI_HEADS = 3,
  EPI_HEADS_T = 4,
  EPI_SOFTMAX_D2S = 5
};
enum Act { ACT_NONE = 0, ACT_RELU = 1 };

struct GemmArgs {
  const uint16_t* X1 = nullptr;
  const uint16_t* X2 = nullptr;
  int ld1 = 0, ld2 = 0, K1 = 0;
  const uint16_t* Wp = nullptr;
  const float* bias = nullptr;
  int M = 0;
  int N = 0;
  int cb_total = 0;
  int epi = EPI_STORE;
  int act = ACT_NONE;
  void* out = nullptr;
  void* out2 = nullptr;
  int ldo = 0;
  float* x32 = nullptr;
  const float* rot_cos = nullptr;
  const float* rot_sin = nullptr;
  int Np = 0, H = 4;
  int small_max = 4096, g8_min = 16000;
  int gr_min = 8192;
  int gr_wgs = 256;
  const int* rowidx = nullptr;
  int d2s_hc = 0, d2s_wc = 0;
  int* flag = nullptr;
};

void launch_gemm(int prec, int K, bool trans, const GemmArgs& a, hipStream_t st);
void launch_gemm8(int prec, int K, bool trans, const GemmArgs& a, hipStream_t st);
bool gemmr_applicable(int K, bool trans, const GemmArgs& a);
void launch_gemmr(int prec, bool trans, const GemmArgs& a, hipStream_t st);
bool gemmr_gather_applicable(int K, const GemmArgs& a);
void launch_gemmr_gather(int prec, const GemmArgs& a, hipStream_t st);
bool gemmr_gather128_applicable(const GemmArgs& a);
void launch_gemmr_gather128(int prec, const GemmArgs& a, hipStream_t st);
bool gemmr_pair_applicable(const GemmArgs& a, const GemmArgs& b);
void launch_gemmr_pair(int prec, const GemmArgs& a, const GemmArgs& b, hipStream_t st);

struct LgBlockFArgs {
  const uint16_t* attn;
  uint16_t* xb;
  float* x32;
  const uint16_t *wo, *w1, *w2;
  const float *bo, *b1, *gamma, *beta, *b2;
  int M;
  int tokens_per_wg = 128;
  int mixed = 0, n_cu = 0;
  int relu = 0;
  const uint16_t *nqk_w = nullptr, *nv_w = nullptr;
  const float *nqk_b = nullptr, *nv_b = nullptr, *rot_cos = nullptr, *rot_sin = nullptr;
  int nqk_n = 0, Np = 0, H = 4;
  uint16_t *q_out = nullptr, *k_out = nullptr, *vt_out = nullptr;
};
void launch_lg_blockf(int prec, const LgBlockFArgs& a, hipStream_t st);
bool lg_blockf_frag_weights();

struct ConvArgs {
  const uint16_t* X = nullptr;
  const uint16_t* Wp = nullptr;
  const float* bias = nullptr;
  uint16_t* Y = nullptr;
  int B = 0, H = 0, W = 0, CIN = 0, COUT = 0;
  int pool = 0;
  int out_pad = 1;
  int relu = 1;
  int wgs = 256;
  const float* img = nullptr;
  const float* w1a = nullptr;
  const float* b1a = nullptr;
};
void launch_conv3x3(int prec, const ConvArgs& a, hipStream_t st);
void launch_conv64r(int prec, const ConvArgs& a, hipStream_t st);
void launch_conv128r(int prec, const ConvArgs& a, hipStream_t st);
constexpr int CONV_ORDER_64R = 1, CONV_ORDER_128R = 2, CONV_ORDER_DEFAULT = CONV_ORDER_64R | CONV_ORDER_128R;
int conv_tile_order_switch();
int conv_tile_order_switch(int v);

void launch_preprocess(const uint8_t* src, int B, int h, int w, int stride, size_t img_stride,
                       const int* xtab , const int* ytab , const float* lut ,
                       float* out, int RH, int RW, hipStream_t st, const uint8_t* src1 = nullptr, int n0 = 0);

void launch_remap_linear(const uint8_t* src, int B, int h, int w, int stride, size_t img_stride, const float* mapx, const float* mapy,
                         uint8_t* dst, int dstride, size_t dimg_stride, hipStream_t st);

void launch_softmax_d2s(const float* logits, int ldl, float* heat, int B, int HC, int WC, hipStream_t st);
void launch_l2norm256(float* d, int rows, hipStream_t st);
void launch_simple_nms(const float* heat, float* out, float* tmp, int B, int H, int W, int radius, hipStream_t st);
void launch_nms512_candidates(const float* heat, float* out, void* planes, int B, float thr, int border, unsigned long long* cand,
                              int* cand_cnt, int cand_cap, hipStream_t st);
void launch_candidates(const float* heat, int B, int H, int W, float thr, int border, unsigned long long* cand,
                       int* cand_cnt, int cand_cap, hipStream_t st);
void launch_candidates_nms3(const float* heat, int B, int H, int W, float thr, unsigned long long* cand, int* cand_cnt, int cand_cap, hipStream_t st);
struct SelectExtra {
  float* feat1 = nullptr; int* n_out1 = nullptr; int Bs = 0;
  int* desc_idx = nullptr; int HC = 0, WC = 0;
  int sort_all = 0;
};
void launch_select_list(const unsigned long long* cand, const int* cand_cnt, int cand_cap, int B, int W, int topk, int cap,
                        float* feat, int* n_out, hipStream_t st, const SelectExtra* ex = nullptr);
void launch_sample_desc(const float* desc, int B, int HC, int WC, float* feat, const int* n, int cap,
                        float w_scale, float h_scale, int normalise, hipStream_t st, int compact = 0, int* flag = nullptr,
                        float* feat1 = nullptr, const int* n1 = nullptr, int Bs = 0);
struct DescSample {
  float* feat = nullptr; float* feat1 = nullptr;
  const int* n = nullptr; const int* n1 = nullptr;
  int Bs = 0, B = 0, cap = 0, HC = 0, WC = 0;
  float w_scale = 1.f, h_scale = 1.f;
  int* flag = nullptr;
  float sx = 0.f, bx = 0.f, sy = 0.f, by = 0.f;
  int junc = 0;
};
bool gemmr_gather_sample_applicable(const GemmArgs& a);
void launch_gemmr_gather_sample(int prec, const GemmArgs& a, const DescSample& ds, hipStream_t st);
bool gemmr_gather_sample_junc_applicable(const GemmArgs& a, const DescSample& ds);
void launch_gemmr_gather_sample_junc(int prec, const GemmArgs& a, const DescSample& ds, hipStream_t st);

struct LgPrepArgs {
  const float* f0; const float* f1;
  const int* n0; const int* n1;
  int ld, kp_off;
  int normalize;
  float cx, cy, linv;
  const float* wr;
  int B, cap, Np;
  float* x32; uint16_t* xb;
  float* rot_cos; float* rot_sin;
  int* lens;
  const float *f0x = nullptr, *f1x = nullptr; const int *n0x = nullptr, *n1x = nullptr;
  int slack_rows = 0;
};
void launch_lg_prepare(int prec, const LgPrepArgs& a, hipStream_t st);
void launch_attention32(int prec, const uint16_t* Q, const uint16_t* K, const uint16_t* Vt, uint16_t* O, const int* lens,
                        int S, int H, int Np, int cross, hipStream_t st);
void launch_ln_gelu(int prec, uint16_t* h, const float* gamma, const float* beta, int M, hipStream_t st);
void launch_rowdot256(const float* x32, const float* w, float b, float* z, int M, hipStream_t st);
void launch_sim(int prec, const uint16_t* md, float* sim, int B, int Np, hipStream_t st);
void launch_lg_assign(const float* sim, const float* z, const int* lens, int B, int Np, int cap, float thr,
                      float* rowlse, float* collse, float* scores_out, int* rowarg, float* rowval, int* colarg,
                      int32_t* idx, float* score, int* nmatch, hipStream_t st);

void launch_trace_hash(const void* p, unsigned unit_words, unsigned units, unsigned long long* out, hipStream_t st);
void launch_trace_digest(const unsigned long long* tab, const unsigned* off, int slots, unsigned long long* dig, hipStream_t st);
size_t lg_assign_part_floats(int B, int Np);
void launch_lg_assign_fused(int prec, const uint16_t* md, const float* z, const int* lens, int B, int Np, int cap, float thr, float* part, float* argpart,
                            float* rowlse, float* collse, float* sim_out, float* scores_out, int* rowarg, float* rowval, int* colarg, int32_t* idx,
                            float* score, int* nmatch, hipStream_t st);
void launch_lg_filter_scores(const float* scores, const int* lens, int B, int Np, int cap, float thr, int* rowarg, float* rowval,
                             int* colarg, int32_t* idx, float* score, int* nmatch, hipStream_t st);

constexpr int LINE_CNT_LD = 64;
constexpr int WF_WGS = 48;
void launch_wireframe(const float* iskeep, const float* imin, const float* imax, int n, int jn, int* table, int* keep,
                      int* pairs, int* rep, int cap, int line_cap, int* counts, bool counted, const float* juncs, const float* lines_pred, float* head4,
                      float* prop4, int B, size_t stage_stride, hipStream_t st);
constexpr int S1_WPAD = 128;
void launch_s1_junc_rows(const float* juncs, int jn, int* ridx, int B, size_t stage_stride, hipStream_t st);
void launch_s1_junc_proj(const float* juncs, const float* head, size_t head_img, int ps, const float* lrows, int jn, const float* w0t,
                         float* proj, int B, size_t stage_stride, hipStream_t st);
void launch_plnet_s1(const float* juncs, const float* lines_pred, const int* keep, const int* pairs, const int* rep,
                     const int* counts, const float* loi, size_t loi_img, const float* proj, const float* ta8, const float* thin,
                     const float* aux, const float* const* w, float* lines_adjusted, float* scores_line, int keep_cap, int line_cap, int B,
                     size_t stage_stride, hipStream_t st, int wgs = 0);
void launch_plnet_s1h(const int* pairs, const int* counts, const float* proj, const float* ta8, const uint16_t* const* wsplit, const float* const* w,
                      const float* lines_adjusted, const float* prop4, float* scores_line, int line_cap, int B, hipStream_t st, int wgs = 0);
void launch_s1h_junc_proj(const float* juncs, const float* lrows, int jn, const uint16_t* wa, const uint16_t* wb, float* proj, int B, size_t stage_stride,
                          hipStream_t st);
void launch_line_filter(const float* la, const float* sc, const int* counts, int border, float line_thr, float len_thr,
                        float w_scale, float h_scale, int R, unsigned char* jmap, int nj, double* lines_out, int capL, int* nlines, int* nfound,
                        int line_cap, int B, hipStream_t st);
void launch_zero16(void* p, size_t bytes, hipStream_t st);
void launch_junction_scan(const unsigned char* jmap, const float* heat, int R, int border, float* feat, int cap, int* n_kept, int* n_found,
                          int* wg_counts, int B, hipStream_t st, const unsigned long long* mask = nullptr);
void launch_line_filter_junc(const float* la, const float* sc, const int* counts, int border, float line_thr, float len_thr, float w_scale, float h_scale,
                             double* lines_out, int capL, int* nlines, int* nfound, int line_cap, int B, int nj, const float* heat, const unsigned long long* mask,
                             float* feat, int capJ, int* n_kept, int* n_jfound, hipStream_t st);

struct GemmF32Args {
  const float* X1 = nullptr; int ld1 = 0, K1 = 0;
  const float* X2 = nullptr; int ld2 = 0;
  const float* W = nullptr;
  const float* bias = nullptr;
  float* Y = nullptr; int ldy = 0;
  int M = 0, N = 0, K = 0;
  float scale = 1.f;
  int relu = 0, accumulate = 0;
};
void launch_conv1a_f32(const float* img, const float* w, const float* bias, float* out, int B, int H, int W, hipStream_t st);
void launch_conv3x3_f32(const float* X, const float* Wt, const float* bias, float* Y, int B, int H, int W, int CIN, int COUT, int opad,
                        hipStream_t st);
void launch_maxpool2_f32(const float* X, float* Y, int B, int H, int W, int C, hipStream_t st);
void launch_gemm_f32(const GemmF32Args& a, hipStream_t st);
void launch_rotary_f32(float* qk, int ld, const float* rc, const float* rs, int M, hipStream_t st);
void launch_attention_f32(const float* Q, int ldq, const float* K, int ldk, const float* V, int ldv, float* O, const int* lens, int S, int H,
                          int Np, int cross, float scale, hipStream_t st);
void launch_ln_gelu_f32(float* h, const float* gamma, const float* beta, int M, hipStream_t st);

void launch_s0_decode(const float* head, int ld, int off, float* lines_pred, float* jloc, float* jnms, float* joff, float* thin, float* aux,
                      float* loi, float* ta8, int B, size_t stage_stride, hipStream_t st);
void launch_s0_head_decode(int prec, const uint16_t* X, const uint16_t* Wp, const float* bias, float* lines_pred, float* jloc, float* jnms,
                           float* joff, float* ta8, int B, size_t stage_stride, hipStream_t st, int wgs = 0);
void launch_s0_juncs(const float* sel, const int* n_sel, const float* joff, float* juncs, int jn, int sel_cap, int B, size_t stage_stride,
                     hipStream_t st);
bool launch_s0_j2l(const float* lines_pred, const float* juncs, int jn, int n, float thr, float* iskeep, float* imin, float* imax, int* counts,
                   int B, size_t stage_stride, int exact_all, hipStream_t st);

void launch_sg_prepare(int prec, const float* f0, const float* f1, const int* n0, const int* n1, int ld, int normalize,
                       float cx, float cy, float linv, const float* const* w, int B, int cap, int Np, float* x32,
// ... 311 lines not shown
```

airslam_amd/csrc/kernels_lgblockf.hip:

```cpp
#include "common.h"
#include "kernels.h"
#ifdef LF_TIMING
__device__ unsigned long long lf_dbg[32];
#define LF_T(i) { const long long now_ = wall_clock64(); if (L.wave == 0 && L.lane == 0) atomicAdd(&lf_dbg[L.tb + i], (unsigned long long)(now_ - tp_)); tp_ = now_; }
extern "C" void airfe_dbg_lf(unsigned long long* out, int reset) {
  if (reset) { unsigned long long z[32] = {}; (void)hipMemcpyToSymbol(HIP_SYMBOL(lf_dbg), z, sizeof(z)); }
  else (void)hipMemcpyFromSymbol(out, HIP_SYMBOL(lf_dbg), 32 * sizeof(unsigned long long));
}
#else
#define LF_T(i)
#endif
#ifdef LF_TIMING2
__device__ unsigned long long lf2_dbg[16];
extern "C" void airfe_dbg_lf2(unsigned long long* out, int reset) {
  if (reset) { unsigned long long z[16] = {}; (void)hipMemcpyToSymbol(HIP_SYMBOL(lf2_dbg), z, sizeof(z)); }
  else (void)hipMemcpyFromSymbol(out, HIP_SYMBOL(lf2_dbg), 16 * sizeof(unsigned long long));
}
#define LF2_NOW(v) { __builtin_amdgcn_sched_barrier(0); v = __builtin_readcyclecounter(); __builtin_amdgcn_sched_barrier(0); }
#endif

namespace airfe {

constexpr int LF_R0 = 0, LF_R1 = 65536, LF_ST = 131072;
constexpr int LF_LDS = LF_ST + 8 * 128 * 8;
// ... 118 lines not shown
      }
    };
    constexpr int AHEAD = (NT == 4 ? 4 : 8) / (NMT > 2 ? 2 : 1);
#pragma unroll
    for (int d = 1; d <= AHEAD; ++d)
      if (d <= nslab) fetch(d, ring[d - 1]);
    __builtin_amdgcn_sched_barrier(0);
#pragma unroll
    for (int s = 0; s < 8; ++s) {
      if (s < nslab) {
        hook(s);
        __builtin_amdgcn_sched_barrier(0);
#pragma unroll
        for (int h = 0; h < 2; ++h) {
          const int boff = (((s * 8 + h * 4 + g) ^ l15) << 4);
          typename P::vec8 bf[NMT];
#pragma unroll
          for (int j = 0; j < NMT; ++j) bf[j] = lds_frag<P>(brow, boff + j * 16 * pitch);
#pragma unroll
          for (int t = 0; t < NT; ++t)
#pragma unroll
            for (int j = 0; j < NMT; ++j) {
              if constexpr (SWAP) acc[t][j] = P::mfma(bf[j], cur[t][h], acc[t][j]);
              else acc[t][j] = P::mfma(cur[t][h], bf[j], acc[t][j]);
            }
        }
#pragma unroll
        for (int t = 0; t < NT; ++t) {
          cur[t][0] = ring[s % AHEAD][t][0];
          cur[t][1] = ring[s % AHEAD][t][1];
        }
        if (s + 1 + AHEAD <= nslab) fetch(s + 1 + AHEAD, ring[s % AHEAD]);
        __builtin_amdgcn_sched_barrier(0);
      }
    }
    return;
  }
  typename P::vec8 nxt[NT][2];
#ifdef LF_NOLDS
  typename P::vec8 bf0[4];
#pragma unroll
  for (int j = 0; j < 4; ++j) bf0[j] = lds_frag<P>(brow, ((g ^ l15) << 4) + j * 16 * pitch);
#endif
#ifdef LF_TIMING2
  [[maybe_unused]] unsigned long long q0 = 0, q1 = 0, q2 = 0, q3 = 0, q4 = 0, q5 = 0, q6 = 0;
  [[maybe_unused]] unsigned long long a_pref = 0, a_vm = 0, a_rd = 0, a_lgkm = 0, a_mma = 0, a_mov = 0, a_trips = 0;
#endif
#pragma unroll 1
  for (int s = 0; s < nslab; ++s) {
#ifdef LF_TIMING2
    if constexpr (TIMED) LF2_NOW(q0)
#endif
    const bool last = s + 1 == nslab;
    const char* p0 = last ? n0 : w0 + (s + 1) * LF_SS;
    const char* p1 = last ? n1 : w1 + (s + 1) * LF_SS;
#ifdef LF_NOWEIGHTS
    if (true) {
      (void)p0; (void)p1;
#pragma unroll
      for (int t = 0; t < NT; ++t) {
        nxt[t][0] = cur[t][0];
        nxt[t][1] = cur[t][1];
      }
    } else
#endif
    if constexpr (TS == TSN) {
#pragma unroll
      for (int t = 0; t < NT; ++t) {
        nxt[t][0] = lf_ldg<P>(p0 + t * TS);
        nxt[t][1] = lf_ldg<P>(p1 + t * TS);
      }
    } else {
      const int ts = last ? TSN : TS;
#pragma unroll
      for (int t = 0; t < NT; ++t) {
        nxt[t][0] = lf_ldg<P>(p0 + t * ts);
        nxt[t][1] = lf_ldg<P>(p1 + t * ts);
      }
    }
    hook(s);
    __builtin_amdgcn_sched_barrier(0);
#ifdef LF_TIMING2
    if constexpr (TIMED) {
      LF2_NOW(q1)
      asm volatile("s_waitcnt vmcnt(%0)" ::"n"(2 * NT) : "memory");
      LF2_NOW(q2)
      a_pref += q1 - q0; a_vm += q2 - q1;
    }
#endif
#pragma unroll
    for (int h = 0; h < 2; ++h) {
      const int boff = (((s * 8 + h * 4 + g) ^ l15) << 4);
#pragma unroll
      for (int mb = 0; mb < NMT; mb += 4) {
#ifdef LF_TIMING2
        if constexpr (TIMED) LF2_NOW(q3)
#endif
        typename P::vec8 bf[4];
#ifdef LF_NOLDS
        (void)boff;
#pragma unroll
        for (int j = 0; j < 4; ++j) bf[j] = bf0[j];
#else
#pragma unroll
        for (int j = 0; j < 4; ++j)
          if (mb + j < NMT) bf[j] = lds_frag<P>(brow, boff + (mb + j) * 16 * pitch);
#endif
#ifdef LF_TIMING2
        if constexpr (TIMED) {
          LF2_NOW(q4)
          asm volatile("s_waitcnt lgkmcnt(0)" ::: "memory");
          LF2_NOW(q5)
        }
#endif
#pragma unroll
        for (int t = 0; t < NT; ++t)
#pragma unroll
          for (int j = 0; j < 4; ++j)
            if (mb + j < NMT) {
              if constexpr (SWAP) acc[t][mb + j] = P::mfma(bf[j], cur[t][h], acc[t][mb + j]);
              else acc[t][mb + j] = P::mfma(cur[t][h], bf[j], acc[t][mb + j]);
            }
#ifdef LF_TIMING2
        if constexpr (TIMED) {
          LF2_NOW(q6)
          a_rd += q4 - q3; a_lgkm += q5 - q4; a_mma += q6 - q5;
        }
#endif
      }
    }
#pragma unroll
    for (int t = 0; t < NT; ++t) {
      cur[t][0] = nxt[t][0];
      cur[t][1] = nxt[t][1];
    }
#ifdef LF_TIMING2
    if constexpr (TIMED) {
      LF2_NOW(q1)
      a_mov += q1 - q6; a_trips += 1;
    }
#endif
  }
#ifdef LF_TIMING2
  if constexpr (TIMED) {
    if ((threadIdx.x & 63) == 0) {
      atomicAdd(&lf2_dbg[0], a_pref); atomicAdd(&lf2_dbg[1], a_vm); atomicAdd(&lf2_dbg[2], a_rd); atomicAdd(&lf2_dbg[3], a_lgkm); atomicAdd(&lf2_dbg[4], a_mma);
      atomicAdd(&lf2_dbg[5], a_mov); atomicAdd(&lf2_dbg[6], a_trips); atomicAdd(&lf2_dbg[7], (unsigned long long)(2 * ((NMT + 3) / 4)) * a_trips);
      atomicAdd(&lf2_dbg[8], (unsigned long long)(2 * NT * NMT) * a_trips);
    }
  }
#endif
}

struct LfLane {
  int lane, wave, l15, g, wf, cb, tp, fo0, fo1;
#ifdef LF_TIMING
  int tb;
#endif
  const char *wob, *w1b, *w2b;
};

template <class P, int NMT, bool RELU, int FOLD, bool FOLDO>
__device__ __forceinline__ void lf_pass(const LgBlockFArgs& a, char* smem, const LfLane& L, int row0) {
  const int lane = L.lane, wave = L.wave, l15 = L.l15, g = L.g, wf = L.wf, cb = L.cb, tp = L.tp, fo0 = L.fo0, fo1 = L.fo1;
#ifdef LF_TIMING
  long long tp_ = wall_clock64();
  if (wave == 0 && lane == 0) atomicAdd(&lf_dbg[L.tb + 15], 1ull);
#endif
  typename P::vec8 c2[2][2], c4[4][2];
  [[maybe_unused]] f32x4 bo2[2];
  f32x4 b14[4];
  if constexpr (FOLDO) {
    lf_first<P, 4, LF_TS512>(c4, L.w1b + 4 * LF_SS + fo0, L.w1b + 4 * LF_SS + fo1);
  } else {
    lf_first<P, 2, LF_TS256>(c2, L.wob + fo0, L.wob + fo1);
#pragma unroll
    for (int u = 0; u < 2; ++u) bo2[u] = *reinterpret_cast<const f32x4*>(a.bo + cb * 64 + tp * 32 + g * 8 + u * 4);
  }
#pragma unroll
  for (int t = 0; t < 4; ++t) b14[t] = *reinterpret_cast<const f32x4*>(a.b1 + wf * 64 + (t >> 1) * 32 + g * 8 + (t & 1) * 4);
  asm volatile("s_waitcnt vmcnt(0)" ::: "memory");
  __syncthreads();
  LF_T(0)

  if constexpr (!FOLDO) {
    {
    f32x4 acc[2][NMT];
#pragma unroll
    for (int u = 0; u < 2; ++u)
#pragma unroll
      for (int m = 0; m < NMT; ++m) acc[u][m] = bo2[u];
    lf_mma<P, 2, NMT, LF_TS256, LF_TS256>(acc, c2, L.wob + fo0, L.wob + fo1, 4, L.wob + fo0, L.wob + fo1, smem + LF_R0, 512, l15, g);
    lf_first<P, 4, LF_TS512>(c4, L.w1b + 4 * LF_SS + fo0, L.w1b + 4 * LF_SS + fo1);
    const int piece = cb * 8 + tp * 4 + g;
#pragma unroll
    for (int m = 0; m < NMT; ++m) {
      float v[8];
#pragma unroll
      for (int e = 0; e < 4; ++e) {
        v[e] = acc[0][m][e];
        v[4 + e] = acc[1][m][e];
      }
      *reinterpret_cast<uint4*>(smem + LF_R1 + (m * 16 + l15) * 512 + ((piece ^ l15) << 4)) = pack8<P>(v);
    }
    }
    __syncthreads();
  }
  LF_T(1)

  f32x4 h[4][NMT];
#pragma unroll
  for (int t = 0; t < 4; ++t)
#pragma unroll
    for (int m = 0; m < NMT; ++m) h[t][m] = b14[t];
  if constexpr (FOLDO) {
    lf_mma<P, 4, NMT, LF_TS512, LF_TS512>(h, c4, L.w1b + 4 * LF_SS + fo0, L.w1b + 4 * LF_SS + fo1, 4, L.w1b + fo0, L.w1b + fo1, smem + LF_R1, 512, l15, g);
    LF_T(2)
    LF_T(3)
  } else {
    auto xhook = [&](int s) { if (s == 3) lf_stage_rows(a.xb, row0, NMT, LF_R0, wave, lane); };
    lf_mma<P, 4, NMT, LF_TS512, LF_TS512, decltype(xhook)>(h, c4, L.w1b + 4 * LF_SS + fo0, L.w1b + 4 * LF_SS + fo1, 4, L.w1b + fo0, L.w1b + fo1, smem + LF_R1, 512, l15, g,
                                                             xhook);
    LF_T(2)
    asm volatile("s_waitcnt vmcnt(0)" ::: "memory");
    __syncthreads();
    LF_T(3)
  }
#ifdef LF_TIMING2
  lf_mma<P, 4, NMT, LF_TS512, LF_TS512, LfNoHook, false, true>(h, c4, L.w1b + fo0, L.w1b + fo1, 4, L.w1b + fo0, L.w1b + fo1, smem + LF_R0, 512, l15, g);
#else
  lf_mma<P, 4, NMT, LF_TS512, LF_TS512>(h, c4, L.w1b + fo0, L.w1b + fo1, 4, L.w1b + fo0, L.w1b + fo1, smem + LF_R0, 512, l15, g);
#endif

  [[maybe_unused]] f32x4 gam[2][2], bet[2][2];
  if constexpr (!RELU) {
#pragma unroll
    for (int q = 0; q < 2; ++q)
#pragma unroll
      for (int u = 0; u < 2; ++u) {
        gam[q][u] = *reinterpret_cast<const f32x4*>(a.gamma + wf * 64 + q * 32 + g * 8 + u * 4);
        bet[q][u] = *reinterpret_cast<const f32x4*>(a.beta + wf * 64 + q * 32 + g * 8 + u * 4);
      }
  }
  if constexpr (!RELU) {
    float2* st = reinterpret_cast<float2*>(smem + LF_ST);
#pragma unroll
    for (int m = 0; m < NMT; ++m) {
      float s1 = 0.f, s2 = 0.f;
#pragma unroll
      for (int t = 0; t < 4; ++t)
#pragma unroll
        for (int e = 0; e < 4; ++e) s1 += h[t][m][e];
      s1 = rows_sum(s1);
      const float mw = s1 * (1.0f / 64.0f);
#pragma unroll
      for (int t = 0; t < 4; ++t)
#pragma unroll
        for (int e = 0; e < 4; ++e) {
          const float d = h[t][m][e] - mw;
          s2 = fmaf(d, d, s2);
        }
      s2 = rows_sum(s2);
      if (g == 0) st[wf * 128 + m * 16 + l15] = make_float2(s1, s2);
    }
  }
  LF_T(4)
  __syncthreads();
  LF_T(5)
  const int co = cb * 64 + tp * 32 + g * 8;
  float* xr0 = a.x32 + (size_t)(row0 + l15) * 256 + co;
  float4 r0[NMT], r1[NMT];
  constexpr bool EARLY_W2 = NMT < 8;
  if constexpr (EARLY_W2) lf_first<P, 2, LF_TS512>(c2, L.w2b + fo0, L.w2b + fo1);
  f32x4 b22[2];
#pragma unroll
  for (int u = 0; u < 2; ++u) b22[u] = *reinterpret_cast<const f32x4*>(a.b2 + co + u * 4);
  __builtin_amdgcn_sched_barrier(0);
  {
    const float2* st = reinterpret_cast<const float2*>(smem + LF_ST);
    [[maybe_unused]] float nmr[NMT], rstd[NMT];
#pragma unroll
    for (int m = 0; m < (RELU ? 0 : NMT); ++m) {
      float s1 = 0.f, s2 = 0.f;
#pragma unroll
      for (int w = 0; w < 8; ++w) s1 += st[w * 128 + m * 16 + l15].x;
      const float mean = s1 * (1.0f / 512.0f);
#pragma unroll
      for (int w = 0; w < 8; ++w) {
        const float2 p = st[w * 128 + m * 16 + l15];
        const float dm = p.x * (1.0f / 64.0f) - mean;
        s2 += fmaf(64.0f * dm, dm, p.y);
      }
      const float var = s2 * (1.0f / 512.0f);
      rstd[m] = 1.0f / sqrtf(var + 1e-5f);
      nmr[m] = -mean * rstd[m];
    }
#pragma unroll
    for (int q = 0; q < 2; ++q) {
      const int piece = wf * 8 + q * 4 + g;
      if constexpr (RELU) {
#pragma unroll
        for (int m = 0; m < NMT; ++m) {
          float v[8];
#pragma unroll
          for (int e = 0; e < 4; ++e) {
            v[e] = fmaxf(h[2 * q][m][e], 0.f);
            v[4 + e] = fmaxf(h[2 * q + 1][m][e], 0.f);
          }
          *reinterpret_cast<uint4*>(smem + (m * 16 + l15) * 1024 + ((piece ^ l15) << 4)) = pack8<P>(v);
        }
      } else {
      const f32x4 g0 = gam[q][0], g1 = gam[q][1], be0 = bet[q][0], be1 = bet[q][1];
#pragma unroll
      for (int m = 0; m < NMT; ++m) {
        const f32x2 rs = {rstd[m], rstd[m]}, nm = {nmr[m], nmr[m]};
        float v[8];
#if LF_GELU_X4
        f32x2 y[4];
#pragma unroll
        for (int e = 0; e < 4; e += 2) {
          y[e >> 1] = (f32x2{h[2 * q][m][e], h[2 * q][m][e + 1]} * rs + nm) * f32x2{g0[e], g0[e + 1]} + f32x2{be0[e], be0[e + 1]};
          y[2 + (e >> 1)] = (f32x2{h[2 * q + 1][m][e], h[2 * q + 1][m][e + 1]} * rs + nm) * f32x2{g1[e], g1[e + 1]} + f32x2{be1[e], be1[e + 1]};
        }
        lf_gelu2x4(y);
#pragma unroll
        for (int e = 0; e < 4; e += 2) {
          v[e] = y[e >> 1].x; v[e + 1] = y[e >> 1].y;
          v[4 + e] = y[2 + (e >> 1)].x; v[5 + e] = y[2 + (e >> 1)].y;
        }
#else
#pragma unroll
        for (int e = 0; e < 4; e += 2) {
          const f32x2 y0 = (f32x2{h[2 * q][m][e], h[2 * q][m][e + 1]} * rs + nm) * f32x2{g0[e], g0[e + 1]} + f32x2{be0[e], be0[e + 1]};
          const f32x2 y1 = (f32x2{h[2 * q + 1][m][e], h[2 * q + 1][m][e + 1]} * rs + nm) * f32x2{g1[e], g1[e + 1]} + f32x2{be1[e], be1[e + 1]};
          const f32x2 o0 = lf_gelu2(y0), o1 = lf_gelu2(y1);
          v[e] = o0.x; v[e + 1] = o0.y;
          v[4 + e] = o1.x; v[5 + e] = o1.y;
        }
#endif
        *reinterpret_cast<uint4*>(smem + (m * 16 + l15) * 1024 + ((piece ^ l15) << 4)) = pack8<P>(v);
      }
      }
      if (q == 0) {
#pragma unroll
        for (int m = 0; m < NMT; ++m) {
          r0[m] = *reinterpret_cast<const float4*>(xr0 + (size_t)m * 16 * 256);
          r1[m] = *reinterpret_cast<const float4*>(xr0 + (size_t)m * 16 * 256 + 4);
        }
        __builtin_amdgcn_sched_barrier(0);
      }
    }
  }
  if constexpr (!EARLY_W2) lf_first<P, 2, LF_TS512>(c2, L.w2b + fo0, L.w2b + fo1);
  LF_T(6)
  __syncthreads();
  LF_T(7)

  constexpr bool KEEP_X = FOLD != 0 && NMT < 8;
  [[maybe_unused]] uint4 xpk[KEEP_X ? NMT : 1];
  {
    f32x4 acc[2][NMT];
#pragma unroll
    for (int u = 0; u < 2; ++u)
#pragma unroll
      for (int m = 0; m < NMT; ++m) acc[u][m] = b22[u];
    const char* nq = FOLD ? reinterpret_cast<const char*>(a.nqk_w) + lf_woff(256, cb, 2 * tp) : L.w2b;
    lf_mma<P, 2, NMT, LF_TS512, (FOLD ? LF_TS256 : LF_TS512)>(acc, c2, L.w2b + fo0, L.w2b + fo1, 8, nq + fo0, nq + fo1, smem, 1024, l15, g);
#pragma unroll
    for (int m = 0; m < NMT; ++m) {
      const size_t row = (size_t)(row0 + m * 16 + l15);
      float* xr = xr0 + (size_t)m * 16 * 256;
      float v[8] = {acc[0][m][0] + r0[m].x, acc[0][m][1] + r0[m].y, acc[0][m][2] + r0[m].z, acc[0][m][3] + r0[m].w,
                    acc[1][m][0] + r1[m].x, acc[1][m][1] + r1[m].y, acc[1][m][2] + r1[m].z, acc[1][m][3] + r1[m].w};
      *reinterpret_cast<float4*>(xr) = make_float4(v[0], v[1], v[2], v[3]);
      *reinterpret_cast<float4*>(xr + 4) = make_float4(v[4], v[5], v[6], v[7]);
      const uint4 xp = pack8<P>(v);
      if constexpr (KEEP_X) xpk[m] = xp;
      *reinterpret_cast<uint4*>(a.xb + row * 256 + co) = xp;
    }
  }
  LF_T(8)
  if constexpr (FOLD != 0) {
    __syncthreads();
    {
      const int piece = cb * 8 + tp * 4 + g;
#pragma unroll
      for (int m = 0; m < NMT; ++m) {
        uint4 xp;
        if constexpr (KEEP_X) xp = xpk[m];
        else xp = *reinterpret_cast<const uint4*>(a.xb + (size_t)(row0 + m * 16 + l15) * 256 + co);
        *reinterpret_cast<uint4*>(smem + LF_R0 + (m * 16 + l15) * 512 + ((piece ^ l15) << 4)) = xp;
      }
    }
    __syncthreads();
    LF_T(9)
    const int H = a.H, Np = a.Np;
    constexpr int NQ = FOLD == 2 ? 2 : 1;
    const char* vbase = reinterpret_cast<const char*>(a.nv_w) + lf_woff(256, cb, 2 * tp);
#pragma unroll
    for (int qu = 0; qu < NQ; ++qu) {
      const int cbq = cb + 4 * qu;
      const char* wq = reinterpret_cast<const char*>(a.nqk_w) + lf_woff(256, cbq, 2 * tp);
      const char* nx = (qu + 1 < NQ) ? reinterpret_cast<const char*>(a.nqk_w) + lf_woff(256, cbq + 4, 2 * tp) : vbase;
      const int cq = cbq * 64 + tp * 32 + g * 8;
      f32x4 bq[2];
#pragma unroll
      for (int u = 0; u < 2; ++u) bq[u] = *reinterpret_cast<const f32x4*>(a.nqk_b + cq + u * 4);
      f32x4 acc[2][NMT];
#pragma unroll
      for (int u = 0; u < 2; ++u)
#pragma unroll
        for (int m = 0; m < NMT; ++m) acc[u][m] = f32x4{0.f, 0.f, 0.f, 0.f};
      lf_mma<P, 2, NMT, LF_TS256, LF_TS256>(acc, c2, wq + fo0, wq + fo1, 4, nx + fo0, nx + fo1, smem + LF_R0, 512, l15, g);
      const int sel = cq >> 8, hh = (cq & 255) >> 6, d = cq & 63;
      uint16_t* ob = sel ? a.k_out : a.q_out;
#pragma unroll
      for (int m = 0; m < NMT; ++m) {
        const int row = row0 + m * 16 + l15;
        float v[8];
#pragma unroll
        for (int e = 0; e < 4; ++e) {
          v[e] = acc[0][m][e] + bq[0][e];
          v[4 + e] = acc[1][m][e] + bq[1][e];
        }
        if constexpr (FOLD == 2) {
          const f32x4 cs = *reinterpret_cast<const f32x4*>(a.rot_cos + (size_t)row * 32 + tp * 16 + g * 4);
          const f32x4 sn = *reinterpret_cast<const f32x4*>(a.rot_sin + (size_t)row * 32 + tp * 16 + g * 4);
          rotate_pairs(v, cs, sn);
        }
        const int sq = row / Np, nn = row - sq * Np;
        *reinterpret_cast<uint4*>(ob + (((size_t)sq * H + hh) * Np + nn) * 64 + d) = pack8<P>(v);
      }
    }
    LF_T(10)
    {
      float bt[2];
#pragma unroll
      for (int u = 0; u < 2; ++u) bt[u] = a.nv_b[cb * 64 + slab_row_to_feature((2 * tp + u) * 16 + l15)];
      f32x4 acc[2][NMT];
#pragma unroll
      for (int u = 0; u < 2; ++u)
#pragma unroll
        for (int m = 0; m < NMT; ++m) acc[u][m] = f32x4{0.f, 0.f, 0.f, 0.f};
      lf_mma<P, 2, NMT, LF_TS256, LF_TS256, LfNoHook, true>(acc, c2, vbase + fo0, vbase + fo1, 4, vbase + fo0, vbase + fo1, smem + LF_R0, 512, l15, g);
#pragma unroll
      for (int u = 0; u < 2; ++u) {
        const int cv = cb * 64 + slab_row_to_feature((2 * tp + u) * 16 + l15);
        const int hh = cv >> 6, d = cv & 63;
#pragma unroll
        for (int m = 0; m < NMT; ++m) {
          const int rw = row0 + m * 16 + g * 4;
          const int sq = rw / Np, nn = rw - sq * Np;
          *reinterpret_cast<uint2*>(a.vt_out + (((size_t)sq * H + hh) * 64 + d) * Np + nn) =
                pack4<P>(acc[u][m][0] + bt[u], acc[u][m][1] + bt[u], acc[u][m][2] + bt[u], acc[u][m][3] + bt[u]);
        }
      }
    }
    LF_T(11)
  }
}

__device__ __forceinline__ void lf_lane_init(const LgBlockFArgs& a, LfLane& L) {
  const int tid = threadIdx.x;
  L.lane = tid & 63;
  L.wave = __builtin_amdgcn_readfirstlane(tid >> 6);
  L.l15 = L.lane & 15;
  L.g = L.lane >> 4;
  if (LF_FRAG) {
    L.fo0 = L.lane * 16;
    L.fo1 = L.lane * 16 + 1024;
  } else {
    const int sw = (L.l15 >> 1) & 7;
    L.fo0 = L.l15 * 128 + ((L.g ^ sw) << 4);
    L.fo1 = L.l15 * 128 + (((4 + L.g) ^ sw) << 4);
  }
  L.wf = (L.wave + (blockIdx.x >> 3)) & 7;
  L.cb = L.wf >> 1;
  L.tp = L.wf & 1;
  L.wob = reinterpret_cast<const char*>(a.wo) + lf_woff(256, L.cb, 2 * L.tp);
  L.w1b = reinterpret_cast<const char*>(a.w1) + lf_woff(512, L.wf, 0);
  L.w2b = reinterpret_cast<const char*>(a.w2) + lf_woff(512, L.cb, 2 * L.tp);
}

template <class P, int NMT, bool RELU, int FOLD, bool FOLDO>
__global__ __launch_bounds__(512, 1) void lg_blockf_kernel(LgBlockFArgs a) {
  extern __shared__ __attribute__((aligned(16))) char smem[];
  LfLane L;
  lf_lane_init(a, L);
  const int row0 = blockIdx.x * (16 * NMT);
  lf_stage_rows(a.attn, row0, NMT, FOLDO ? LF_R1 : LF_R0, L.wave, L.lane);
  if constexpr (FOLDO) lf_stage_rows(a.xb, row0, NMT, LF_R0, L.wave, L.lane);
#ifdef LF_TIMING
  L.tb = 0;
#endif
  lf_pass<P, NMT, RELU, FOLD, FOLDO>(a, smem, L, row0);
#ifdef LF_TWICE
  __syncthreads();
  L.tb = 16;
  lf_stage_rows(a.attn, row0, NMT, FOLDO ? LF_R1 : LF_R0, L.wave, L.lane);
  if constexpr (FOLDO) lf_stage_rows(a.xb, row0, NMT, LF_R0, L.wave, L.lane);
  lf_pass<P, NMT, RELU, FOLD, FOLDO>(a, smem, L, row0);
#endif
}

template <class P, bool RELU, int FOLD>
__global__ __launch_bounds__(512, 1) void lg_blockf_mixed_kernel(LgBlockFArgs a, int n7) {
  extern __shared__ __attribute__((aligned(16))) char smem[];
  LfLane L;
  lf_lane_init(a, L);
#ifdef LF_TIMING
  L.tb = 0;
#endif
  if ((int)blockIdx.x < n7) {
    const int row0 = blockIdx.x * 112;
    lf_stage_rows(a.attn, row0, 7, LF_R1, L.wave, L.lane);
    lf_stage_rows(a.xb, row0, 7, LF_R0, L.wave, L.lane);
    lf_pass<P, 7, RELU, FOLD, true>(a, smem, L, row0);
  } else {
    const int row0 = n7 * 112 + ((int)blockIdx.x - n7) * 96;
    lf_stage_rows(a.attn, row0, 6, LF_R1, L.wave, L.lane);
    lf_stage_rows(a.xb, row0, 6, LF_R0, L.wave, L.lane);
    lf_pass<P, 6, RELU, FOLD, true>(a, smem, L, row0);
  }
}

template <class P, bool RELU, int FOLD>
static bool launch_mixed(const LgBlockFArgs& a, hipStream_t st) {
  const int tiles = (a.M + 15) / 16, W = a.n_cu;
  if (!a.mixed || a.wo || W <= 0 || tiles <= 7 * W || tiles > 13 * W) return false;
  const int n7 = W, n6 = (tiles - 7 * W + 5) / 6;
  static PerDeviceOnce attr_once;
  auto kfn = lg_blockf_mixed_kernel<P, RELU, FOLD>;
  if (auto once_token = attr_once.first()) {
    (void)hipFuncSetAttribute(reinterpret_cast<const void*>(kfn), hipFuncAttributeMaxDynamicSharedMemorySize, LF_LDS);
  }
  hipLaunchKernelGGL(kfn, dim3((unsigned)(n7 + n6)), dim3(512), LF_LDS, st, a, n7);
  return true;
}

template <class P, int NMT, bool RELU, int FOLD, bool FOLDO>
static void launch_fo(const LgBlockFArgs& a, hipStream_t st) {
  static PerDeviceOnce attr_once;
  auto kfn = lg_blockf_kernel<P, NMT, RELU, FOLD, FOLDO>;
  if (auto once_token = attr_once.first()) {
    (void)hipFuncSetAttribute(reinterpret_cast<const void*>(kfn), hipFuncAttributeMaxDynamicSharedMemorySize, LF_LDS);
  }
  hipLaunchKernelGGL(kfn, dim3((unsigned)((a.M + 16 * NMT - 1) / (16 * NMT))), dim3(512), LF_LDS, st, a);
}

template <class P, int NMT, bool RELU, int FOLD = 0>
static void launch_f(const LgBlockFArgs& a, hipStream_t st) {
  if (a.wo) launch_fo<P, NMT, RELU, FOLD, false>(a, st);
  else launch_fo<P, NMT, RELU, FOLD, true>(a, st);
}

template <class P, bool RELU, int FOLD>
static void launch_nmt(const LgBlockFArgs& a, hipStream_t st) {
  switch (a.tokens_per_wg) {
    case 32: launch_f<P, 2, RELU, FOLD>(a, st); break;
    case 64: launch_f<P, 4, RELU, FOLD>(a, st); break;
    case 112: if (!launch_mixed<P, RELU, FOLD>(a, st)) launch_f<P, 7, RELU, FOLD>(a, st); break;
    default: launch_f<P, 8, RELU, FOLD>(a, st); break;
  }
}

bool lg_blockf_frag_weights() { return LF_FRAG != 0; }

void launch_lg_blockf(int prec, const LgBlockFArgs& a, hipStream_t st) {
  if (a.relu) {
    if (prec == 1) launch_nmt<PF16, true, 0>(a, st); else launch_nmt<PBF16, true, 0>(a, st);
    return;
  }
  if (a.nqk_w) {
    if (a.nqk_n == 512) {
      if (prec == 1) launch_nmt<PF16, false, 2>(a, st); else launch_nmt<PBF16, false, 2>(a, st);
    } else {
      if (prec == 1) launch_nmt<PF16, false, 1>(a, st); else launch_nmt<PBF16, false, 1>(a, st);
    }
    return;
  }
  if (prec == 1) launch_nmt<PF16, false, 0>(a, st); else launch_nmt<PBF16, false, 0>(a, st);
}

}
```

include/airfe_debug.h:

```cpp
#ifndef AIRFE_DEBUG_H_
#define AIRFE_DEBUG_H_
#include "airfe.h"
#ifdef __cplusplus
extern "C" {
#endif

int airfe_debug_detector_maps(airfe_ctx* ctx, int B, float* heat_raw, float* heat_nms, float* desc);
int airfe_debug_lightglue_scores(airfe_ctx* ctx, const float* f0, int n0, const float* f1, int n1, float* scores);
int airfe_debug_lg_filter(airfe_ctx* ctx, const float* scores, int n0, int n1, int32_t* idx, float* score, int cap, int* nmatch);
int airfe_debug_sg_decode(airfe_ctx* ctx, const float* Z, int n0, int n1, int32_t* idx0, int32_t* idx1, double* ms0, double* ms1);
int airfe_debug_sg_sinkhorn(airfe_ctx* ctx, const float* sim, const int* lens , int B, int ld ,
                            float alpha, int iters, int form , float* Z , int* form_ran);
int airfe_debug_superglue_scores(airfe_ctx* ctx, const float* f0, int n0, const float* f1, int n1, float* scores);
int airfe_debug_plnet_stage0(airfe_ctx* ctx, float* juncs_pred, float* lines_pred, float* iskeep, float* idx_min, float* idx_max,
                             float* loi, float* thin, float* aux, float* jloc, float* joff);
int airfe_debug_plnet_j2l(airfe_ctx* ctx, int fast, float* iskeep, float* idx_min, float* idx_max);
int airfe_debug_plnet_s1(airfe_ctx* ctx, const airfe_plnet_stage0* stage0, float* lines_adjusted, float* scores_line,
                         int cap, int* m2);
int airfe_debug_plnet_s1_last(airfe_ctx* ctx, float* lines_adjusted, float* scores_line, int cap, int* m2);
int airfe_debug_preprocess(airfe_ctx* ctx, const uint8_t* gray, int h, int w, int stride, float* out);
int airfe_debug_conv3x3(airfe_ctx* ctx, const float* x, int B, int cin, int H, int W, const float* w, const float* b,
                        int cout, int pool, float* y);
int airfe_debug_gemm(airfe_ctx* ctx, const float* x, int M, int K, const float* w, const float* b, int N, int relu, float* y);
typedef struct airfe_debug_conv_args {
  const float* x;
  const float* img;
  const float *w1a, *b1a;
  const float *w, *b;
  int cin, cout, B, H, W;
  int pool, out_pad, relu, wgs;
  size_t y_words;
  uint16_t* y_raw;
} airfe_debug_conv_args;
int airfe_debug_conv(airfe_ctx* ctx, airfe_debug_conv_args* a);
int airfe_debug_conv_order(int order, int* previous);
enum {
  AIRFE_DEBUG_KERNEL_DISPATCH = 0,
  AIRFE_DEBUG_KERNEL_SMALL = 1,
  AIRFE_DEBUG_KERNEL_TILED = 2,
  AIRFE_DEBUG_KERNEL_GEMM8 = 3,
  AIRFE_DEBUG_KERNEL_GEMMR = 4,
  AIRFE_DEBUG_KERNEL_GEMMR_GATHER = 5,
  AIRFE_DEBUG_KERNEL_GEMMR_GATHER128 = 6
};
typedef struct airfe_debug_linear_args {
  int prec, M, K, K1, N;
  const float* x1;
  const float* x2;
  const float* w;
  const float* b;
  int epi, act;
  const int* rowidx;
  int src_rows;
  const float* rot_cos;
  const float* rot_sin;
  int Np, H;
  float* x32;
  int d2s_hc, d2s_wc;
  int* flag;
  int kernel;
  int gr_wgs;
  float* out;
  float* out2;
} airfe_debug_linear_args;
int airfe_debug_linear(airfe_ctx* ctx, const airfe_debug_linear_args* a);
int airfe_debug_qkv(airfe_ctx* ctx, int prec, int M, int Np, const float* x, const float* wqk, const float* bqk, int nqk, const float* wv, const float* bv,
                    const float* rot_cos, const float* rot_sin, int pair, int gr_wgs, float* q, float* k, float* vt);
typedef struct airfe_debug_lg_block_args {
  int prec, M;
  const float* attn;
  float* x32;
  float* xb;
  const float *wo, *bo;
  const float *w1, *b1;
  const float *gamma, *beta;
  const float *w2, *b2;
  int relu;
  int tokens_per_wg, mixed;
  int nqk_n;
  const float *nqk_w, *nqk_b;
  const float *nv_w, *nv_b;
  const float *rot_cos, *rot_sin;
  int Np;
  float *q, *k, *vt;
  int rows_past[5];
} airfe_debug_lg_block_args;
int airfe_debug_lg_block(airfe_ctx* ctx, airfe_debug_lg_block_args* a);
int airfe_debug_ln_gelu(airfe_ctx* ctx, int prec, float* h, const float* gamma, const float* beta, int M);
int airfe_debug_attention(airfe_ctx* ctx, const float* q, const float* k, const float* v, const int* lens, int S, int H, int n, int cross, float* out);
typedef struct airfe_debug_attn_args {
  int prec;
  int S, H, n, cross;
  const float *q, *k, *v;
  const int* lens;
  int canary, raw;
  float* out;
  int Np, rows_past;
} airfe_debug_attn_args;
int airfe_debug_attention_args(airfe_ctx* ctx, airfe_debug_attn_args* a);
typedef struct airfe_debug_lg_prepare_args {
  int prec;
  int B, cap, ld, kp_off;
  int normalize;
  float cx, cy, linv;
  const float *f0, *f1;
  const int *n0, *n1;
  const float* wr;
  const float *f0x, *f1x;
  int n0x, n1x;
  int slack_rows;
  int rows;
  float *x32, *xb;
  float *rot_cos, *rot_sin;
  int* lens;
  int rows_past;
} airfe_debug_lg_prepare_args;
int airfe_debug_lg_prepare(airfe_ctx* ctx, airfe_debug_lg_prepare_args* a);
typedef struct airfe_debug_lg_assign_args {
  int prec, B, n;
  const float* md;
  const float* x32;
  const float* w;
  float b;
  const int* lens;
  int cap;
  float thr;
  int form;
  const float* pad;
  float* z;
  float *sim, *scores;
  float *rowlse, *collse, *rowval;
  int32_t *rowarg, *colarg;
  int32_t* idx;
  float* score;
  int32_t* nmatch;
} airfe_debug_lg_assign_args;
int airfe_debug_lg_assign(airfe_ctx* ctx, airfe_debug_lg_assign_args* a);
typedef struct airfe_debug_sg_front_args {
  int prec, split;
  int B, cap, normalize;
  const float *f0, *f1;
  const int *n0, *n1;
  int rows;
  int* lens;
  float *x32, *xb;
  float *h128, *hb;
  int rows_past;
} airfe_debug_sg_front_args;
int airfe_debug_sg_front(airfe_ctx* ctx, airfe_debug_sg_front_args* a);
typedef struct airfe_debug_detector_tail_args {
  int B, Bs, h, w, cap;
  const float* heat;
  const float* act;
  float *feat, *feat1;
  int *n, *n1;
  float* nms_map;
  unsigned long long* keep;
  int* cand_cnt;
  int nms_map_written;
} airfe_debug_detector_tail_args;
int airfe_debug_detector_tail(airfe_ctx* ctx, airfe_debug_detector_tail_args* a);
typedef struct airfe_debug_line_post_args {
  int B, nj, ld, h, w, capL, capJ, from_plane;
  const float *la, *sc;
  const int* m2;
  const float* heat;
  double* lines;
  int *nlines, *nfound;
  float* junc;
  int *njunc, *jfound;
  const unsigned char* jmap;
} airfe_debug_line_post_args;
int airfe_debug_line_post(airfe_ctx* ctx, airfe_debug_line_post_args* a);
typedef struct airfe_debug_junction_tail_args {
  int B, nj, ld, h, w, capL, capJ;
  const float *la, *sc;
  const int* m2;
  const float* heat;
  const float* act;
  double* lines;
  int *nlines, *nfound;
  float* junc;
  int *njunc, *jfound;
  int fused;
} airfe_debug_junction_tail_args;
int airfe_debug_junction_tail(airfe_ctx* ctx, airfe_debug_junction_tail_args* a);
int airfe_debug_junctions_topk(airfe_ctx* ctx, const float* jloc, const float* joff, int B, float* juncs_pred);
typedef struct airfe_debug_line_mid_args {
  int B, j2l, s1_form, wgs;
  const float* juncs_pred;
  const float* lines_pred;
  const float *thin, *aux;
  const float* loi;
  const float *iskeep_in, *idx_min_in, *idx_max_in;
  float *iskeep, *idx_min, *idx_max;
  int32_t* counts;
  int32_t* keep;
  int32_t *pairs, *rep;
  float *head4, *prop4;
  int32_t* ridx;
  float* proj;
  float *lines_adjusted, *scores_line;
  int32_t* table_dirty;
} airfe_debug_line_mid_args;
int airfe_debug_line_mid(airfe_ctx* ctx, airfe_debug_line_mid_args* a);
typedef struct airfe_debug_s0_decode_args {
  int B, mode;
  int ld, off;
  int want_ta8, want_loi, want_jnms;
  int prec, wgs;
  const float* rows;
  const float* x;
  const float *w, *b;
  size_t stage_floats;
  float* stage;
  float *jloc, *joff, *jnms;
  float* ta8;
  float* loi;
  float* head_rows;
} airfe_debug_s0_decode_args;
int airfe_debug_s0_decode(airfe_ctx* ctx, airfe_debug_s0_decode_args* a);
int airfe_debug_fail_next_launch(airfe_ctx* ctx, int stage);
int airfe_debug_trace(airfe_ctx* ctx, int on);
int airfe_debug_trace_stop(airfe_ctx* ctx, int slot);
int airfe_debug_trace_buffer(airfe_ctx* ctx, int slot, void* host, size_t bytes);
int airfe_debug_trace_slots(airfe_ctx* ctx);
int airfe_debug_trace_slot(airfe_ctx* ctx, int i, char* name, int name_cap, unsigned* off, unsigned* units, unsigned* unit_words);
int airfe_debug_trace_read(airfe_ctx* ctx, void* stream, unsigned long long* digests, unsigned long long* table);
typedef struct airfe_debug_wg_prims_args {
  const int32_t* v; const uint8_t* keep; int n, threads;
  const void* keys; int P, key_bytes;
  int32_t *scan, *pos, *totals, *wave;
  void* sorted;
} airfe_debug_wg_prims_args;
int airfe_debug_wg_prims(airfe_ctx* ctx, airfe_debug_wg_prims_args* a);

#ifdef __cplusplus
}
#endif
#endif
// ... 1 lines not shown
```

Baseline: 7982.

## Add software-pipelined fast path for folded next-layer QKV projection in LightGlue block

Adds a new FP template path for the 112-token folded LightGlue block kernel. It reuses the already-loaded W2 fragments for the first weight slab, prefetches the remaining Q/K/V weight slabs into registers ahead of use, and computes the projections slab by slab with double-buffered weight loads. The goal is to hide global weight-load latency behind the MFMA work and cut redundant passes. It is on by default through a global switch, and debug hooks are added to choose the form and read raw outputs. The extra prefetch buffers raise register pressure, which could cause spills.

Result: no change. 8012, median of 6 (+0.4%).

```diff
diff --git a/airslam_amd/_lib.py b/airslam_amd/_lib.py
--- a/airslam_amd/_lib.py
+++ b/airslam_amd/_lib.py
@@ -69,7 +69,8 @@
     _fields_ = ([("prec", C.c_int), ("M", C.c_int)] + [(n, C.c_void_p) for n in ("attn", "x32", "xb", "wo", "bo", "w1", "b1", "gamma", "beta", "w2", "b2")]
                 + [(n, C.c_int) for n in ("relu", "tokens_per_wg", "mixed", "nqk_n")]
                 + [(n, C.c_void_p) for n in ("nqk_w", "nqk_b", "nv_w", "nv_b", "rot_cos", "rot_sin")]
-                + [("Np", C.c_int)] + [(n, C.c_void_p) for n in ("q", "k", "vt")] + [("rows_past", C.c_int * 5)])
+                + [("Np", C.c_int)] + [(n, C.c_void_p) for n in ("q", "k", "vt")] + [("rows_past", C.c_int * 5), ("fold_form", C.c_int), ("n_cu", C.c_int)]
+                + [(n, C.c_void_p) for n in ("raw_x32", "raw_xb", "raw_q", "raw_k", "raw_vt")])
 
 
 class DebugWgPrimsArgs(C.Structure):
@@ -316,6 +317,7 @@
     "airfe_debug_trace_buffer": (C.c_int, [C.c_void_p, C.c_int, C.c_void_p, C.c_size_t]),
     "airfe_debug_trace_slots": (C.c_int, [C.c_void_p]),
     "airfe_debug_conv_order": (C.c_int, [C.c_int, C.POINTER(C.c_int)]),
+    "airfe_debug_lg_fold_form": (C.c_int, [C.c_int, C.POINTER(C.c_int)]),
     "airfe_debug_wg_prims": (C.c_int, [C.c_void_p, C.POINTER(DebugWgPrimsArgs)]),
     "airfe_debug_trace_slot": (C.c_int, [C.c_void_p, C.c_int, C.c_char_p, C.c_int, C.POINTER(C.c_uint), C.POINTER(C.c_uint), C.POINTER(C.c_uint)]),
     "airfe_debug_trace_read": (C.c_int, [C.c_void_p, C.c_void_p, C.c_void_p, C.c_void_p]),
diff --git a/airslam_amd/api.py b/airslam_amd/api.py
--- a/airslam_amd/api.py
+++ b/airslam_amd/api.py
@@ -35,6 +35,13 @@
     return prev.value
 
 
+def lg_fold_form(form: int) -> int:
+    prev = C.c_int()
+    if _lib.lib().airfe_debug_lg_fold_form(int(form), C.byref(prev)) != 0:
+        raise AirfeError((_lib.lib().airfe_last_error(None) or b"airfe_debug_lg_fold_form failed").decode())
+    return prev.value
+
+
 class Context:
 
     def __init__(self, superpoint=None, lightglue=None, superglue=None, plnet_s1=None, tuning=None, **cfg):
@@ -45,6 +52,9 @@
         if tuning and "conv_order" in tuning:
             tuning = dict(tuning)
             conv_tile_order(int(tuning.pop("conv_order")))
+        if tuning and "lg_fold_form" in tuning:
+            tuning = dict(tuning)
+            lg_fold_form(int(tuning.pop("lg_fold_form")))
         if tuning:
             t = _lib.Tuning()
             self._l.airfe_default_tuning(C.byref(t))
@@ -663,7 +673,7 @@
         return q, k, vt
 
     def debug_lg_block(self, attn, x32, w1, b1, w2, b2, prec, gamma=None, beta=None, wo=None, bo=None, relu=False, tokens_per_wg=128, mixed=False,
-                       nqk=None, nv=None, rot=None, Np=0):
+                       nqk=None, nv=None, rot=None, Np=0, fold_form=0, n_cu=0, raw=False):
         f32 = lambda t: None if t is None else np.ascontiguousarray(t, np.float32)
         m = attn.shape[0]
         attn, w1, b1, w2, b2, gamma, beta, wo, bo = map(f32, (attn, w1, b1, w2, b2, gamma, beta, wo, bo))
@@ -671,9 +681,14 @@
         xb = np.empty_like(x32)
         ptr = lambda t: None if t is None else t.ctypes.data
         a = _lib.DebugLgBlockArgs(prec=prec, M=m, attn=ptr(attn), x32=ptr(x32), xb=ptr(xb), wo=ptr(wo), bo=ptr(bo), w1=ptr(w1), b1=ptr(b1), gamma=ptr(gamma),
-                                  beta=ptr(beta), w2=ptr(w2), b2=ptr(b2), relu=int(relu), tokens_per_wg=tokens_per_wg, mixed=int(mixed), Np=Np)
+                                  beta=ptr(beta), w2=ptr(w2), b2=ptr(b2), relu=int(relu), tokens_per_wg=tokens_per_wg, mixed=int(mixed), Np=Np, fold_form=fold_form, n_cu=n_cu)
         q = k = vt = None
         keep = []
+        rawd = None
+        if raw:
+            cap = m + 256
+            rawd = {"x32": np.empty((cap, 256), np.float32), "xb": np.empty((cap, 256), np.uint16)}
+            a.raw_x32, a.raw_xb = ptr(rawd["x32"]), ptr(rawd["xb"])
         if nqk is not None:
             (qw, qb), (vw, vb) = map(lambda p: (f32(p[0]), f32(p[1])), (nqk, nv))
             keep += [qw, qb, vw, vb]
@@ -683,12 +698,22 @@
             if qw.shape[0] == 512:
                 k = np.empty_like(q)
                 a.k = ptr(k)
+            if raw:
+                sg = -(-(m + 256) // Np)
+                rawd["q"], rawd["vt"] = np.empty((sg, 4, Np, 64), np.uint16), np.empty((sg, 4, 64, Np), np.uint16)
+                a.raw_q, a.raw_vt = ptr(rawd["q"]), ptr(rawd["vt"])
+                if k is not None:
+                    rawd["k"] = np.empty((sg, 4, Np, 64), np.uint16)
+                    a.raw_k = ptr(rawd["k"])
         if rot is not None:
             rc, rs = f32(rot[0]), f32(rot[1])
             keep += [rc, rs]
             a.rot_cos, a.rot_sin = ptr(rc), ptr(rs)
         self._chk(self._l.airfe_debug_lg_block(self._h, C.byref(a)), "airfe_debug_lg_block")
-        return {"x32": x32, "xb": xb, "q": q, "k": k, "vt": vt, "rows_past": list(a.rows_past)}
+        out = {"x32": x32, "xb": xb, "q": q, "k": k, "vt": vt, "rows_past": list(a.rows_past)}
+        if raw:
+            out["raw"] = rawd
+        return out
 
     def debug_ln_gelu(self, h, gamma, beta, prec):
         h = np.array(h, np.float32, copy=True)
diff --git a/airslam_amd/csrc/airfe_debug.hip b/airslam_amd/csrc/airfe_debug.hip
--- a/airslam_amd/csrc/airfe_debug.hip
+++ b/airslam_amd/csrc/airfe_debug.hip
@@ -260,6 +260,7 @@
   if (previous) *previous = before;
   return 0;
 } AIRFE_CATCH(nullptr)
+int airfe_debug_lg_fold_form(int form, int* previous) try { if (form < -1 || form > 1) return fail(nullptr, "debug_lg_fold_form: form must lie in -1 .. 1"); const int before = lg_fold_form_switch(form); if (previous) *previous = before; return 0; } AIRFE_CATCH(nullptr)
 
 int airfe_debug_linear(airfe_ctx* c, const airfe_debug_linear_args* a) try {
   AIRFE_ENTER(c);
@@ -359,7 +360,7 @@
 int airfe_debug_qkv(airfe_ctx* c, int prec, int M, int Np, const float* x, const float* wqk, const float* bqk, int nqk, const float* wv, const float* bv,
                     const float* rot_cos, const float* rot_sin, int pair, int gr_wgs, float* q, float* k, float* vt) try {
   AIRFE_ENTER(c);
-  if ((prec != 0 && prec != 1) || M < 1 || Np < 16 || Np % 16 || M % Np || (nqk != 256 && nqk != 512) || !x || !wqk || !bqk || !wv || !bv || !q || !vt ||
+  if ((prec != 0 && prec != 1) || M < 1 || Np < 16 || Np % (pair ? 4 : 16) || M % Np || (nqk != 256 && nqk != 512) || !x || !wqk || !bqk || !wv || !bv || !q || !vt ||
       (nqk == 512 && !k) || (!rot_cos) != (!rot_sin))
     return fail(c, "debug_qkv: bad argument");
   const int Mp = (M + 127) / 128 * 128, Sg = (Mp + Np - 1) / Np, S = M / Np;
@@ -398,16 +399,16 @@
   AIRFE_ENTER(c);
   if (!a || !a->attn || !a->x32 || !a->xb || !a->w1 || !a->b1 || !a->w2 || !a->b2 || (!a->relu && (!a->gamma || !a->beta)) || (!a->wo) != (!a->bo))
     return fail(c, "debug_lg_block: null argument");
-  const int prec = a->prec, M = a->M, T = a->tokens_per_wg, nq = a->nqk_n, Np = a->Np;
-  if ((prec != 0 && prec != 1) || M < 1 || (T != 32 && T != 64 && T != 112 && T != 128) || (nq != 0 && nq != 256 && nq != 512) || (a->relu && nq))
+  const int prec = a->prec, M = a->M, T = a->tokens_per_wg, nq = a->nqk_n, Np = a->Np, n_cu = a->n_cu > 0 ? a->n_cu : c->n_cu;
+  if ((prec != 0 && prec != 1) || M < 1 || (T != 32 && T != 64 && T != 112 && T != 128) || (nq != 0 && nq != 256 && nq != 512) || (a->relu && nq) || a->fold_form < 0 || a->fold_form > 2 || n_cu > c->n_cu)
     return fail(c, "debug_lg_block: bad argument");
   if (a->mixed) {
-    const int tiles = (M + 15) / 16, W = c->n_cu;
+    const int tiles = (M + 15) / 16, W = n_cu;
     if (a->wo || T != 112 || W <= 0 || tiles <= 7 * W || tiles > 13 * W) return fail(c, "debug_lg_block: the mixed split does not apply to this form");
   }
   if (nq && (!a->nqk_w || !a->nqk_b || !a->nv_w || !a->nv_b || !a->q || !a->vt || (nq == 512) != (a->rot_cos && a->rot_sin) || (nq == 512 && !a->k) || Np < 16 ||
-             Np % 16 || M % Np))
-    return fail(c, "debug_lg_block: the next projection needs its weights and outputs, rotary exactly when nqk_n = 512, and M = S * Np (Np a multiple of 16)");
+             Np % 4 || M % Np))
+    return fail(c, "debug_lg_block: the next projection needs its weights and outputs, rotary exactly when nqk_n = 512, and M = S * Np (Np a multiple of 4)");
   const int cap = M + 256;
   const int Sg = nq ? (cap + Np - 1) / Np : 0, S = nq ? M / Np : 0;
   const size_t helems = (size_t)Sg * 4 * Np * 64;
@@ -431,7 +432,7 @@
   g.gamma = dgb; g.beta = dgb ? dgb + 512 : nullptr;
   g.wo = a->wo ? (fr ? lo.wf : lo.w) : nullptr; g.bo = a->wo ? lo.b : nullptr;
   g.w1 = fr ? l1.wf : l1.w; g.b1 = l1.b; g.w2 = fr ? l2.wf : l2.w; g.b2 = l2.b;
-  g.M = M; g.tokens_per_wg = T; g.mixed = a->mixed; g.n_cu = c->n_cu; g.relu = a->relu;
+  g.M = M; g.tokens_per_wg = T; g.mixed = a->mixed; g.n_cu = n_cu; g.relu = a->relu; g.fold_form = a->fold_form - 1;
   if (nq) {
     g.nqk_w = fr ? lq.wf : lq.w; g.nqk_b = lq.b; g.nqk_n = nq; g.nv_w = fr ? lv.wf : lv.w; g.nv_b = lv.b; g.Np = Np; g.H = 4;
     if (nq == 512) { g.rot_cos = s.up(dbg_rows4(a->rot_cos, M, 32, cap)); g.rot_sin = s.up(dbg_rows4(a->rot_sin, M, 32, cap)); }
@@ -446,6 +447,7 @@
   const std::vector<uint16_t> xbo = s.get<uint16_t>(g.xb, (size_t)cap * 256);
   memcpy(a->x32, x32o.data(), (size_t)M * 256 * 4);
   dbg_back2(xbo, (size_t)M * 256, prec, a->xb);
+  if (a->raw_x32 && a->raw_xb) { memcpy(a->raw_x32, x32o.data(), x32o.size() * 4); memcpy(a->raw_xb, xbo.data(), xbo.size() * 2); }
   for (int i = 0; i < 5; ++i) a->rows_past[i] = 0;
   for (int r = M; r < cap; ++r)
     for (int f = 0; f < 256; ++f) {
@@ -454,11 +456,11 @@
       if (xbo[e] != xbh[e]) a->rows_past[1] = r - M + 1;
     }
   uint16_t* dev[3] = {g.q_out, g.k_out, g.vt_out};
-  float* host[3] = {a->q, a->k, a->vt};
+  float* host[3] = {a->q, a->k, a->vt}; uint16_t* raw[3] = {a->raw_q, a->raw_k, a->raw_vt};
   for (int j = 0; j < 3 && nq; ++j) {
     if (!dev[j]) continue;
     const std::vector<uint16_t> ho = s.get<uint16_t>(dev[j], helems);
-    dbg_back2(ho, (size_t)S * 4 * Np * 64, prec, host[j]);
+    dbg_back2(ho, (size_t)S * 4 * Np * 64, prec, host[j]); if (raw[j]) memcpy(raw[j], ho.data(), helems * 2);
     for (size_t e = (size_t)S * 4 * Np * 64; e < helems; ++e) {
       if (ho[e] == 0xFFFF) continue;
       const size_t sq = e / ((size_t)4 * Np * 64), w = e % ((size_t)Np * 64);
diff --git a/airslam_amd/csrc/kernels.h b/airslam_amd/csrc/kernels.h
--- a/airslam_amd/csrc/kernels.h
+++ b/airslam_amd/csrc/kernels.h
@@ -68,8 +68,12 @@
   const float *nqk_b = nullptr, *nv_b = nullptr, *rot_cos = nullptr, *rot_sin = nullptr;
   int nqk_n = 0, Np = 0, H = 4;
   uint16_t *q_out = nullptr, *k_out = nullptr, *vt_out = nullptr;
+  int fold_form = -1;
 };
 void launch_lg_blockf(int prec, const LgBlockFArgs& a, hipStream_t st);
+constexpr int LG_FOLD_FORM_DEFAULT = 1;
+int lg_fold_form_switch();
+int lg_fold_form_switch(int v);
 bool lg_blockf_frag_weights();
 
 struct ConvArgs {
diff --git a/airslam_amd/csrc/kernels_lgblockf.hip b/airslam_amd/csrc/kernels_lgblockf.hip
--- a/airslam_amd/csrc/kernels_lgblockf.hip
+++ b/airslam_amd/csrc/kernels_lgblockf.hip
@@ -294,6 +294,29 @@
 #endif
 }
 
+template <class P, int NT, int NMT, unsigned SWAPM>
+__device__ __forceinline__ void lf_slab(f32x4 (&acc)[NT][NMT], const typename P::vec8 (&w)[NT][2], int s, const char* brow, int pitch, int l15, int g) {
+#pragma unroll
+  for (int h = 0; h < 2; ++h) {
+    const int boff = (((s * 8 + h * 4 + g) ^ l15) << 4);
+#pragma unroll
+    for (int mb = 0; mb < NMT; mb += 4) {
+      typename P::vec8 bf[4];
+#pragma unroll
+      for (int j = 0; j < 4; ++j)
+        if (mb + j < NMT) bf[j] = lds_frag<P>(brow, boff + (mb + j) * 16 * pitch);
+#pragma unroll
+      for (int t = 0; t < NT; ++t)
+#pragma unroll
+        for (int j = 0; j < 4; ++j)
+          if (mb + j < NMT) {
+            if ((SWAPM >> t) & 1) acc[t][mb + j] = P::mfma(bf[j], w[t][h], acc[t][mb + j]);
+            else acc[t][mb + j] = P::mfma(w[t][h], bf[j], acc[t][mb + j]);
+          }
+    }
+  }
+}
+
 struct LfLane {
   int lane, wave, l15, g, wf, cb, tp, fo0, fo1;
 #ifdef LF_TIMING
@@ -302,7 +325,7 @@
   const char *wob, *w1b, *w2b;
 };
 
-template <class P, int NMT, bool RELU, int FOLD, bool FOLDO>
+template <class P, int NMT, bool RELU, int FOLD, bool FOLDO, int FP>
 __device__ __forceinline__ void lf_pass(const LgBlockFArgs& a, char* smem, const LfLane& L, int row0) {
   const int lane = L.lane, wave = L.wave, l15 = L.l15, g = L.g, wf = L.wf, cb = L.cb, tp = L.tp, fo0 = L.fo0, fo1 = L.fo1;
 #ifdef LF_TIMING
@@ -499,15 +522,56 @@
   LF_T(7)
 
   constexpr bool KEEP_X = FOLD != 0 && NMT < 8;
+  constexpr bool FAST = FP != 0 && KEEP_X && NMT > 4;
   [[maybe_unused]] uint4 xpk[KEEP_X ? NMT : 1];
+  [[maybe_unused]] typename P::vec8 vw[3][2][2];
+  [[maybe_unused]] typename P::vec8 pw[2][4][2];
+  [[maybe_unused]] float bt[2];
+  [[maybe_unused]] f32x4 bq[4];
+  [[maybe_unused]] const char *qbase = nullptr, *vbase = nullptr;
+  [[maybe_unused]] const unsigned fu0 = (unsigned)fo0, fu1 = (unsigned)fo1;
+  if constexpr (FOLD != 0) {
+    qbase = reinterpret_cast<const char*>(a.nqk_w) + lf_woff(256, cb, 2 * tp);
+    vbase = reinterpret_cast<const char*>(a.nv_w) + lf_woff(256, cb, 2 * tp);
+  }
   {
     f32x4 acc[2][NMT];
 #pragma unroll
     for (int u = 0; u < 2; ++u)
 #pragma unroll
       for (int m = 0; m < NMT; ++m) acc[u][m] = b22[u];
-    const char* nq = FOLD ? reinterpret_cast<const char*>(a.nqk_w) + lf_woff(256, cb, 2 * tp) : L.w2b;
+    const char* nq = !FOLD ? L.w2b : (FAST && FOLD == 2) ? vbase : qbase;
     lf_mma<P, 2, NMT, LF_TS512, (FOLD ? LF_TS256 : LF_TS512)>(acc, c2, L.w2b + fo0, L.w2b + fo1, 8, nq + fo0, nq + fo1, smem, 1024, l15, g);
+    if constexpr (FAST) {
+#pragma unroll
+      for (int u = 0; u < 2; ++u) bt[u] = a.nv_b[cb * 64 + slab_row_to_feature((2 * tp + u) * 16 + l15)];
+      if constexpr (FOLD == 2) {
+#pragma unroll
+        for (int s = 1; s < 4; ++s)
+#pragma unroll
+          for (int t = 0; t < 2; ++t) {
+            vw[s - 1][t][0] = lf_ldg<P>(vbase + t * LF_TS256 + s * LF_SS + fu0);
+            vw[s - 1][t][1] = lf_ldg<P>(vbase + t * LF_TS256 + s * LF_SS + fu1);
+          }
+      } else {
+#pragma unroll
+        for (int u = 0; u < 2; ++u) bq[u] = *reinterpret_cast<const f32x4*>(a.nqk_b + co + u * 4);
+#pragma unroll
+        for (int t = 0; t < 2; ++t) {
+          pw[0][t][0] = c2[t][0];
+          pw[0][t][1] = c2[t][1];
+          pw[0][2 + t][0] = lf_ldg<P>(vbase + t * LF_TS256 + fu0);
+          pw[0][2 + t][1] = lf_ldg<P>(vbase + t * LF_TS256 + fu1);
+        }
+#pragma unroll
+        for (int t = 0; t < 4; ++t) {
+          const char* wb = (t < 2 ? qbase : vbase) + (t & 1) * LF_TS256 + LF_SS;
+          pw[1][t][0] = lf_ldg<P>(wb + fu0);
+          pw[1][t][1] = lf_ldg<P>(wb + fu1);
+        }
+      }
+      __builtin_amdgcn_sched_barrier(0);
+    }
 #pragma unroll
     for (int m = 0; m < NMT; ++m) {
       const size_t row = (size_t)(row0 + m * 16 + l15);
@@ -537,8 +601,139 @@
     __syncthreads();
     LF_T(9)
     const int H = a.H, Np = a.Np;
+    if constexpr (FAST) {
+      const char* brow = smem + LF_R0 + l15 * 512;
+      int rowf = row0;
+      asm volatile("" : "+s"(rowf));
+      const int hh = cb, d = tp * 32 + g * 8;
+      auto store_v = [&](int u, int m, uint2 pk) {
+        const int cv = cb * 64 + slab_row_to_feature((2 * tp + u) * 16 + l15);
+        const int rw = rowf + m * 16 + g * 4;
+        const int sq = rw / Np, nn = rw - sq * Np;
+        *reinterpret_cast<uint2*>(a.vt_out + (((size_t)sq * H + (cv >> 6)) * 64 + (cv & 63)) * Np + nn) = pk;
+      };
+      auto store_qk = [&](uint16_t* ob, int m, const float* v) {
+        const int row = rowf + m * 16 + l15;
+        const int sq = row / Np, nn = row - sq * Np;
+        *reinterpret_cast<uint4*>(ob + (((size_t)sq * H + hh) * Np + nn) * 64 + d) = pack8<P>(v);
+      };
+      if constexpr (FOLD == 2) {
+        const char* kbase = reinterpret_cast<const char*>(a.nqk_w) + lf_woff(256, cb + 4, 2 * tp);
+        typename P::vec8 qw[2][4][2];
+        auto ldqk = [&](typename P::vec8 (&dst)[4][2], int s) {
+#pragma unroll
+          for (int t = 0; t < 4; ++t) {
+            const char* wb = (t < 2 ? qbase : kbase) + (t & 1) * LF_TS256 + s * LF_SS;
+            dst[t][0] = lf_ldg<P>(wb + fu0);
+            dst[t][1] = lf_ldg<P>(wb + fu1);
+          }
+        };
+        ldqk(qw[0], 0);
+        __builtin_amdgcn_sched_barrier(0);
+        uint2 vpk[2][NMT];
+        {
+          f32x4 acc[2][NMT];
+#pragma unroll
+          for (int u = 0; u < 2; ++u)
+#pragma unroll
+            for (int m = 0; m < NMT; ++m) acc[u][m] = f32x4{0.f, 0.f, 0.f, 0.f};
+          lf_slab<P, 2, NMT, 3u>(acc, c2, 0, brow, 512, l15, g);
+#pragma unroll
+          for (int s = 1; s < 4; ++s) lf_slab<P, 2, NMT, 3u>(acc, vw[s - 1], s, brow, 512, l15, g);
+#pragma unroll
+          for (int u = 0; u < 2; ++u)
+#pragma unroll
+            for (int m = 0; m < NMT; ++m) {
+              vpk[u][m] = pack4<P>(acc[u][m][0] + bt[u], acc[u][m][1] + bt[u], acc[u][m][2] + bt[u], acc[u][m][3] + bt[u]);
+              asm volatile("" : "+v"(vpk[u][m].x), "+v"(vpk[u][m].y));
+            }
+        }
+        __builtin_amdgcn_sched_barrier(0);
+        LF_T(10)
+        f32x4 acc[4][NMT];
+#pragma unroll
+        for (int t = 0; t < 4; ++t)
+#pragma unroll
+          for (int m = 0; m < NMT; ++m) acc[t][m] = f32x4{0.f, 0.f, 0.f, 0.f};
+        f32x4 cs[NMT], sn[NMT];
+        auto ldrot = [&](int m) {
+          const unsigned ro = (unsigned)(rowf + m * 16 + l15) * 32u + (unsigned)(tp * 16 + g * 4);
+          cs[m] = *reinterpret_cast<const f32x4*>(a.rot_cos + ro);
+          sn[m] = *reinterpret_cast<const f32x4*>(a.rot_sin + ro);
+        };
+#pragma unroll
+        for (int s = 0; s < 4; ++s) {
+          if (s < 3) {
+            ldqk(qw[(s + 1) & 1], s + 1);
+          } else {
+#pragma unroll
+            for (int u = 0; u < 4; ++u) bq[u] = *reinterpret_cast<const f32x4*>(a.nqk_b + (unsigned)((u >> 1) * 256 + d + hh * 64 + (u & 1) * 4));
+          }
+          __builtin_amdgcn_sched_barrier(0);
+          lf_slab<P, 4, NMT, 0u>(acc, qw[s & 1], s, brow, 512, l15, g);
+          __builtin_amdgcn_sched_barrier(0);
+        }
+#pragma unroll
+        for (int m = 0; m < NMT; ++m) ldrot(m);
+        __builtin_amdgcn_sched_barrier(0);
+#pragma unroll
+        for (int u = 0; u < 2; ++u)
+#pragma unroll
+          for (int m = 0; m < NMT; ++m) store_v(u, m, vpk[u][m]);
+#pragma unroll
+        for (int m = 0; m < NMT; ++m)
+#pragma unroll
+          for (int qu = 0; qu < 2; ++qu) {
+            float v[8];
+#pragma unroll
+            for (int e = 0; e < 4; ++e) {
+              v[e] = acc[2 * qu][m][e] + bq[2 * qu][e];
+              v[4 + e] = acc[2 * qu + 1][m][e] + bq[2 * qu + 1][e];
+            }
+            rotate_pairs(v, cs[m], sn[m]);
+            store_qk(qu ? a.k_out : a.q_out, m, v);
+          }
+        LF_T(11)
+      } else {
+        f32x4 acc[4][NMT];
+#pragma unroll
+        for (int t = 0; t < 4; ++t)
+#pragma unroll
+          for (int m = 0; m < NMT; ++m) acc[t][m] = f32x4{0.f, 0.f, 0.f, 0.f};
+#pragma unroll
+        for (int s = 0; s < 4; ++s) {
+          if (s == 1 || s == 2) {
+#pragma unroll
+            for (int t = 0; t < 4; ++t) {
+              const char* wb = (t < 2 ? qbase : vbase) + (t & 1) * LF_TS256 + (s + 1) * LF_SS;
+              pw[(s + 1) & 1][t][0] = lf_ldg<P>(wb + fu0);
+              pw[(s + 1) & 1][t][1] = lf_ldg<P>(wb + fu1);
+            }
+          }
+          __builtin_amdgcn_sched_barrier(0);
+          lf_slab<P, 4, NMT, 12u>(acc, pw[s & 1], s, brow, 512, l15, g);
+          __builtin_amdgcn_sched_barrier(0);
+        }
+        LF_T(10)
+#pragma unroll
+        for (int m = 0; m < NMT; ++m) {
+          float v[8];
+#pragma unroll
+          for (int e = 0; e < 4; ++e) {
+            v[e] = acc[0][m][e] + bq[0][e];
+            v[4 + e] = acc[1][m][e] + bq[1][e];
+          }
+          store_qk(a.q_out, m, v);
+        }
+#pragma unroll
+        for (int u = 0; u < 2; ++u)
+#pragma unroll
+          for (int m = 0; m < NMT; ++m)
+            store_v(u, m, pack4<P>(acc[2 + u][m][0] + bt[u], acc[2 + u][m][1] + bt[u], acc[2 + u][m][2] + bt[u], acc[2 + u][m][3] + bt[u]));
+        LF_T(11)
+      }
+    } else {
     constexpr int NQ = FOLD == 2 ? 2 : 1;
-    const char* vbase = reinterpret_cast<const char*>(a.nv_w) + lf_woff(256, cb, 2 * tp);
 #pragma unroll
     for (int qu = 0; qu < NQ; ++qu) {
       const int cbq = cb + 4 * qu;
@@ -599,6 +794,7 @@
       }
     }
     LF_T(11)
+    }
   }
 }
 
@@ -624,7 +820,7 @@
   L.w2b = reinterpret_cast<const char*>(a.w2) + lf_woff(512, L.cb, 2 * L.tp);
 }
 
-template <class P, int NMT, bool RELU, int FOLD, bool FOLDO>
+template <class P, int NMT, bool RELU, int FOLD, bool FOLDO, int FP>
 __global__ __launch_bounds__(512, 1) void lg_blockf_kernel(LgBlockFArgs a) {
   extern __shared__ __attribute__((aligned(16))) char smem[];
   LfLane L;
@@ -635,17 +831,17 @@
 #ifdef LF_TIMING
   L.tb = 0;
 #endif
-  lf_pass<P, NMT, RELU, FOLD, FOLDO>(a, smem, L, row0);
+  lf_pass<P, NMT, RELU, FOLD, FOLDO, FP>(a, smem, L, row0);
 #ifdef LF_TWICE
   __syncthreads();
   L.tb = 16;
   lf_stage_rows(a.attn, row0, NMT, FOLDO ? LF_R1 : LF_R0, L.wave, L.lane);
   if constexpr (FOLDO) lf_stage_rows(a.xb, row0, NMT, LF_R0, L.wave, L.lane);
-  lf_pass<P, NMT, RELU, FOLD, FOLDO>(a, smem, L, row0);
-#endif
-}
-
-template <class P, bool RELU, int FOLD>
+  lf_pass<P, NMT, RELU, FOLD, FOLDO, FP>(a, smem, L, row0);
+#endif
+}
+
+template <class P, bool RELU, int FOLD, int FP>
 __global__ __launch_bounds__(512, 1) void lg_blockf_mixed_kernel(LgBlockFArgs a, int n7) {
   extern __shared__ __attribute__((aligned(16))) char smem[];
   LfLane L;
@@ -657,22 +853,22 @@
     const int row0 = blockIdx.x * 112;
     lf_stage_rows(a.attn, row0, 7, LF_R1, L.wave, L.lane);
     lf_stage_rows(a.xb, row0, 7, LF_R0, L.wave, L.lane);
-    lf_pass<P, 7, RELU, FOLD, true>(a, smem, L, row0);
+    lf_pass<P, 7, RELU, FOLD, true, FP>(a, smem, L, row0);
   } else {
     const int row0 = n7 * 112 + ((int)blockIdx.x - n7) * 96;
     lf_stage_rows(a.attn, row0, 6, LF_R1, L.wave, L.lane);
     lf_stage_rows(a.xb, row0, 6, LF_R0, L.wave, L.lane);
-    lf_pass<P, 6, RELU, FOLD, true>(a, smem, L, row0);
-  }
-}
-
-template <class P, bool RELU, int FOLD>
+    lf_pass<P, 6, RELU, FOLD, true, FP>(a, smem, L, row0);
+  }
+}
+
+template <class P, bool RELU, int FOLD, int FP>
 static bool launch_mixed(const LgBlockFArgs& a, hipStream_t st) {
   const int tiles = (a.M + 15) / 16, W = a.n_cu;
   if (!a.mixed || a.wo || W <= 0 || tiles <= 7 * W || tiles > 13 * W) return false;
   const int n7 = W, n6 = (tiles - 7 * W + 5) / 6;
   static PerDeviceOnce attr_once;
-  auto kfn = lg_blockf_mixed_kernel<P, RELU, FOLD>;
+  auto kfn = lg_blockf_mixed_kernel<P, RELU, FOLD, FP>;
   if (auto once_token = attr_once.first()) {
     (void)hipFuncSetAttribute(reinterpret_cast<const void*>(kfn), hipFuncAttributeMaxDynamicSharedMemorySize, LF_LDS);
   }
@@ -680,20 +876,20 @@
   return true;
 }
 
-template <class P, int NMT, bool RELU, int FOLD, bool FOLDO>
+template <class P, int NMT, bool RELU, int FOLD, bool FOLDO, int FP>
 static void launch_fo(const LgBlockFArgs& a, hipStream_t st) {
   static PerDeviceOnce attr_once;
-  auto kfn = lg_blockf_kernel<P, NMT, RELU, FOLD, FOLDO>;
+  auto kfn = lg_blockf_kernel<P, NMT, RELU, FOLD, FOLDO, FP>;
   if (auto once_token = attr_once.first()) {
     (void)hipFuncSetAttribute(reinterpret_cast<const void*>(kfn), hipFuncAttributeMaxDynamicSharedMemorySize, LF_LDS);
   }
   hipLaunchKernelGGL(kfn, dim3((unsigned)((a.M + 16 * NMT - 1) / (16 * NMT))), dim3(512), LF_LDS, st, a);
 }
 
-template <class P, int NMT, bool RELU, int FOLD = 0>
+template <class P, int NMT, bool RELU, int FOLD = 0, int FP = 0>
 static void launch_f(const LgBlockFArgs& a, hipStream_t st) {
-  if (a.wo) launch_fo<P, NMT, RELU, FOLD, false>(a, st);
-  else launch_fo<P, NMT, RELU, FOLD, true>(a, st);
+  if (a.wo) launch_fo<P, NMT, RELU, FOLD, false, FP>(a, st);
+  else launch_fo<P, NMT, RELU, FOLD, true, FP>(a, st);
 }
 
 template <class P, bool RELU, int FOLD>
@@ -701,12 +897,25 @@
   switch (a.tokens_per_wg) {
     case 32: launch_f<P, 2, RELU, FOLD>(a, st); break;
     case 64: launch_f<P, 4, RELU, FOLD>(a, st); break;
-    case 112: if (!launch_mixed<P, RELU, FOLD>(a, st)) launch_f<P, 7, RELU, FOLD>(a, st); break;
+    case 112:
+      if constexpr (FOLD != 0) {
+        const int fp = a.fold_form < 0 ? lg_fold_form_switch() : a.fold_form;
+        if (fp != 0) {
+          if (!launch_mixed<P, RELU, FOLD, 1>(a, st)) launch_f<P, 7, RELU, FOLD, 1>(a, st);
+          break;
+        }
+      }
+      if (!launch_mixed<P, RELU, FOLD, 0>(a, st)) launch_f<P, 7, RELU, FOLD>(a, st);
+      break;
     default: launch_f<P, 8, RELU, FOLD>(a, st); break;
   }
 }
 
 bool lg_blockf_frag_weights() { return LF_FRAG != 0; }
+
+static std::atomic<int> g_fold_form{LG_FOLD_FORM_DEFAULT};
+int lg_fold_form_switch() { return g_fold_form.load(std::memory_order_relaxed); }
+int lg_fold_form_switch(int v) { return g_fold_form.exchange(v < 0 ? LG_FOLD_FORM_DEFAULT : (v != 0), std::memory_order_relaxed); }
 
 void launch_lg_blockf(int prec, const LgBlockFArgs& a, hipStream_t st) {
   if (a.relu) {
diff --git a/include/airfe_debug.h b/include/airfe_debug.h
--- a/include/airfe_debug.h
+++ b/include/airfe_debug.h
@@ -84,8 +84,13 @@
   int Np;
   float *q, *k, *vt;
   int rows_past[5];
+  int fold_form;
+  int n_cu;
+  float* raw_x32;
+  uint16_t *raw_xb, *raw_q, *raw_k, *raw_vt;
 } airfe_debug_lg_block_args;
 int airfe_debug_lg_block(airfe_ctx* ctx, airfe_debug_lg_block_args* a);
+int airfe_debug_lg_fold_form(int form, int* previous);
 int airfe_debug_ln_gelu(airfe_ctx* ctx, int prec, float* h, const float* gamma, const float* beta, int M);
 int airfe_debug_attention(airfe_ctx* ctx, const float* q, const float* k, const float* v, const int* lens, int S, int H, int n, int cross, float* out);
 typedef struct airfe_debug_attn_args {
```
